# OATML-Markslab/ProteinGym

Hardware: AMD Instinct MI355X
Metric: mutants scored/sec (ESM-1v 650M masked-marginal) (higher is better)
Workload: dtype f16x3 (fp32 operands split into 2 fp16 planes, 3 fp16 MFMAs per product, fp32 accumulate)

## Files before the change

### proteingym_amd/csrc/api_esm.hip

```cpp
#include "model.h"

namespace pgmi {

int create_esm(pgmi_model* m, const pgmi_config* cfg, const float* w, int64_t n_weights) {
    const size_t D = cfg->embed_dim, F = cfg->ffn_dim, V = cfg->vocab, dh = m->dh, Da = m->Da;
    BlobCursor c(m, w, n_weights);
    c.upload(&m->embed_tokens, V * D);
    if (cfg->arch == PGMI_ARCH_ESM1B) c.upload(&m->embed_positions, (size_t)(cfg->max_positions + 2) * D);
    if (cfg->emb_layer_norm_before) {
        c.upload(&m->lnb_w, D);
        c.upload(&m->lnb_b, D);
    }
    auto slot = [&](size_t col) -> size_t { return rotate_half_slot(col, dh); };
    const float qscale = 1.0f / sqrtf((float)dh);
    m->layers.resize(cfg->layers);
    std::vector<float> wq(3 * Da * D, 0.0f), bq(3 * Da, 0.0f), wo_r(D * Da, 0.0f);
    for (int l = 0; l < cfg->layers; ++l) {
        Layer& L = m->layers[l];
        c.upload(&L.ln1_w, D);
        c.upload(&L.ln1_b, D);
        pack_qkv_slots(c.take(3 * (D * D + D)), D, Da, slot, qscale, wq.data(), bq.data());
        c.linear(&L.wqkv, &L.wqkv16, wq.data(), wq.size(), D);
        c.upload(&L.bqkv, bq.data(), bq.size());
        pack_out_cols(c.take(D * D), D, Da, slot, wo_r.data());
        c.linear(&L.wo, &L.wo16, wo_r.data(), wo_r.size(), Da);
        c.upload(&L.bo, D);
        c.upload(&L.ln2_w, D);
        c.upload(&L.ln2_b, D);
        c.linear(&L.w1, &L.w116, F * D, D);
        c.upload(&L.b1, F);
        c.linear(&L.w2, &L.w216, D * F, F);
        c.upload(&L.b2, D);
    }
    c.upload(&m->lna_w, D);
    c.upload(&m->lna_b, D);
    c.linear(&m->hd_w, &m->hd16, D * D, D);
    c.upload(&m->hd_b, D);
    c.upload(&m->hln_w, D);
    c.upload(&m->hln_b, D);
    c.upload(&m->head_b, V);
    m->head_w = m->embed_tokens;
    return c.finish();
}

int ensure_rotary(pgmi_model* m, int T) {
    if ((!esm2_rotary(m->cfg.arch) && !esmc_blocks(m->cfg.arch)) || T <= m->rot_len) return PGMI_OK;
    return upload_rotate_half(m, std::max(T, 1026));
}

int upload_rotate_half(pgmi_model* m, int n) {
    const int rh = m->rot_halves;
    float inv[64];
    const int half = m->dh / 2;
    for (int i = 0; i < half; ++i) inv[i] = 1.0f / powf(10000.0f, (float)(2 * i) / (float)m->dh);
    return upload_rotary(m, n, rh, [&](int t, int g, int i) {
        const int j = (rh == 1) ? i : 32 * g + i;
        return j < half ? (float)t * inv[j] : 0.0f;
    });
}

int run_encoder(pgmi_model* m, int B, int T, const int32_t* keep, int n_keep, bool* compacted) {
    const pgmi_config& c = m->cfg;
    const int M = B * T, D = c.embed_dim, F = c.ffn_dim, N1 = m->fc1_cols, H = c.heads, Da = m->Da;
    hipStream_t s = m->stream;
    if (c.arch == PGMI_ARCH_ESM1B && T > c.max_positions) {
        set_error("Sequence length %d above maximum sequence length of %d", T, c.max_positions);
        return PGMI_EINVAL;
    }
    int rc = ensure_rotary(m, T);
    if (!rc) rc = reset_pad_keys(m, B, T);
    if (rc) return rc;
    {
        ProfScope p(m, PGMI_K_EMBED, 0, (double)M * D * 4);
        launch_seq_stats(m->tokens, B, T, m->embed_gather ? 0 : c.token_dropout, m->denom, m->pos_idx, m->kv_len, s, m->mask_id);
        if (c.arch == PGMI_ARCH_ESM3) { if ((rc = esm3_embed(m, B, T))) return rc; }
        else if (m->embed_gather) launch_gather_rows(m->embed_tokens, m->tokens, M, D, m->x, s);
        else launch_embed(m->tokens, m->denom, m->pos_idx, m->embed_tokens, m->embed_positions, c.token_dropout, M, T, D, m->x, s, m->mask_id);
        if (m->lnb_w) {
            launch_layernorm(m->x, m->lnb_w, m->lnb_b, M, D, 1e-5f, m->x, s);
            launch_zero_pad_rows(m->tokens, M, D, m->x, s);
        }
    }
    const double ln_bytes = 2.0 * M * D * 4;
    const int prec = c.precision;
    const int mode16 = (prec == PGMI_PREC_F16X3) ? 1 : 2;
    for (int l = 0; l < c.layers; ++l) {
        const Layer& L = m->layers[l];
        { ProfScope p(m, PGMI_K_LAYERNORM, 0, ln_bytes);
          if (prec == PGMI_PREC_FP32) launch_layernorm(m->x, L.ln1_w, L.ln1_b, M, D, 1e-5f, m->h, s);
          else launch_layernorm16(m->x, L.ln1_w, L.ln1_b, M, D, 1e-5f, m->h16, mode16, s); }
        const bool fused_qkv = prec != PGMI_PREC_FP32 && !L.q_ln;
        { ProfScope p(m, PGMI_K_GEMM_QKV, 2.0 * M * 3 * D * D, 0);
          if (fused_qkv) {
              GemmLaunch g = qkv_launch(m, L.wqkv16, L.bqkv, M, Da, D, T, m->Hs);
              g.bf = prec == PGMI_PREC_BF16;
              g.qkv.cos_t = m->rot_cos; g.qkv.sin_t = m->rot_sin; g.qkv.rotary = esm2_rotary(c.arch); g.qkv.rot_halves = m->rot_halves;
              rc = launch_gemm16(g);
          } else
              rc = linear(m, m->h, m->h16, L.wqkv, L.wqkv16, L.bqkv, nullptr, m->qkv, nullptr, M, 3 * Da, D, EPI_NONE);
          if (rc) return rc; }
        { ProfScope p(m, PGMI_K_ATTENTION, 4.0 * M * T * D, L.q_ln ? (double)M * D * 20 : 0);
          if (L.q_ln && (rc = launch_qkln_prep(m->qkv, L.q_ln, L.k_ln, 1e-5f, m->rot_cos, m->rot_sin, B, T, H, m->qk16, m->qk16_plane,
                                               m->vt16, m->vt16_plane, s)))
              return rc;
          const bool v2 = prec != PGMI_PREC_FP32;
          if (esm2_rotary(c.arch) && !v2) launch_rotary(m->qkv, m->rot_cos, m->rot_sin, M, T, m->Hs, s, m->rot_halves);
          if (v2) {
              AttLaunch a;
              a.qk16 = m->qk16, a.qk_plane = m->qk16_plane, a.vt16 = m->vt16, a.vt_plane = m->vt16_plane;
              a.B = B, a.T = T, a.H = H, a.head_dim = m->rot_halves * kHeadDim;
              a.kv_len = m->kv_len;
              a.out = prec == PGMI_PREC_F16X3 ? ATT_OUT_SPLIT : ATT_OUT_BF16;
              a.ctx16 = m->h16;
              a.stream = s;
              rc = launch_attention_f16x3_v2(a);
          } else {
              rc = launch_attention_f32(m->qkv, m->kv_len, B, T, H, m->h, s, m->rot_halves * kHeadDim);
          }
          if (rc) return rc; }
        if (keep && m->keep_rows && l == c.layers - 1 && !L.g_norm_w) {
            const int R = n_keep;
            ProfScope p(m, PGMI_K_KEPT_ROWS, 2.0 * R * D * (Da + N1 + F), 0);
            launch_gather_rows(m->x, keep, R, D, m->qkv, s);
            if (prec == PGMI_PREC_FP32) launch_gather_rows(m->h, keep, R, Da, m->g, s);
            else
                launch_gather_rows(reinterpret_cast<const float*>(m->h16), keep, R, prec == PGMI_PREC_F16X3 ? Da : Da / 2,
                                   reinterpret_cast<float*>(m->g16), s);
            rc = linear(m, m->g, m->g16, L.wo, L.wo16, L.bo, m->qkv, m->x, nullptr, R, D, Da, EPI_NONE);
            if (rc) return rc;
            if (prec == PGMI_PREC_FP32) launch_layernorm(m->x, L.ln2_w, L.ln2_b, R, D, 1e-5f, m->h, s);
            else launch_layernorm16(m->x, L.ln2_w, L.ln2_b, R, D, 1e-5f, m->h16, mode16, s);
            rc = linear(m, m->h, m->h16, L.w1, L.w116, L.b1, nullptr,
                        prec == PGMI_PREC_FP32 ? m->g : nullptr, prec == PGMI_PREC_FP32 ? nullptr : m->g16,
                        R, N1, D, m->fc1_epi);
            if (rc) return rc;
            rc = linear(m, m->g, m->g16, L.w2, L.w216, L.b2, m->x, m->x, nullptr, R, D, F, EPI_NONE);
            if (rc) return rc;
            if (compacted) *compacted = true;
            break;
        }
        { ProfScope p(m, PGMI_K_GEMM_OUT, 2.0 * M * D * D, 0);
          rc = linear(m, m->h, m->h16, L.wo, L.wo16, L.bo, m->x, m->x, nullptr, M, D, Da, EPI_NONE);
          if (rc) return rc; }
        if (L.g_norm_w && m->e3_framed && (rc = geom_branch(m, L, B, T))) return rc;
        { ProfScope p(m, PGMI_K_LAYERNORM, 0, ln_bytes);
          if (prec == PGMI_PREC_FP32) launch_layernorm(m->x, L.ln2_w, L.ln2_b, M, D, 1e-5f, m->h, s);
          else launch_layernorm16(m->x, L.ln2_w, L.ln2_b, M, D, 1e-5f, m->h16, mode16, s); }
        { ProfScope p(m, PGMI_K_GEMM_FC1, 2.0 * M * N1 * D, 0);
          rc = linear(m, m->h, m->h16, L.w1, L.w116, L.b1, nullptr,
                      prec == PGMI_PREC_FP32 ? m->g : nullptr, prec == PGMI_PREC_FP32 ? nullptr : m->g16,
                      M, N1, D, m->fc1_epi);
          if (rc) return rc; }
        { ProfScope p(m, PGMI_K_GEMM_FC2, 2.0 * M * F * D, 0);
          rc = linear(m, m->g, m->g16, L.w2, L.w216, L.b2, m->x, m->x, nullptr, M, D, F, EPI_NONE);
          if (rc) return rc; }
    }
    PGMI_HIP(hipGetLastError());
    return PGMI_OK;
}

int run_head(pgmi_model* m, int R, const int32_t* row_idx) {
    const pgmi_config& c = m->cfg;
    ProfScope p(m, PGMI_K_HEAD, 2.0 * R * c.embed_dim * (c.embed_dim + c.vocab), 0);
    int rc = head_hidden(m, R, row_idx);
    if (rc) return rc;
    launch_vocab_logsoftmax(m->g, m->head_w, m->head_b, R, c.embed_dim, c.vocab, m->lp, m->nonfinite, m->stream);
    PGMI_HIP(hipGetLastError());
    return PGMI_OK;
}

int head_hidden(pgmi_model* m, int R, const int32_t* row_idx) {
    const pgmi_config& c = m->cfg;
    const int D = c.embed_dim;
    hipStream_t s = m->stream;
    const int prec = c.precision;
    const float* src = m->x;
    if (row_idx) {
        launch_gather_rows(m->x, row_idx, R, D, m->h, s);
        src = m->h;
    }
    if (prec == PGMI_PREC_FP32) launch_layernorm(src, m->lna_w, m->lna_b, R, D, 1e-5f, m->h, s);
    else launch_layernorm16(src, m->lna_w, m->lna_b, R, D, 1e-5f, m->h16, prec == PGMI_PREC_F16X3 ? 1 : 2, s);
    int rc = linear(m, m->h, m->h16, m->hd_w, m->hd16, m->hd_b, nullptr, m->g, nullptr, R, D, D, EPI_GELU);
    if (rc) return rc;
    launch_layernorm(m->g, m->hln_w, m->hln_b, R, D, 1e-5f, m->g, s);
    return PGMI_OK;
}


int run_rows(pgmi_model* m, int B, int T, int R, const int32_t* row_idx) {
    bool compacted = false;
    int rc = run_encoder(m, B, T, row_idx, R, &compacted);
    if (rc) return rc;
    return run_head(m, R, compacted ? nullptr : row_idx);
}

}

extern "C" {

int pgmi_token_logprobs(pgmi_model* m, const int32_t* tokens, int B, int T, float* out) {
    if (!m || !tokens || !out || B <= 0 || T <= 0) { set_error("bad argument"); return PGMI_EINVAL; }
    if (m->cfg.arch == PGMI_ARCH_SAPROT) { set_error("SaProt models are scored with pgmi_saprot_token_logprobs / pgmi_saprot_group_logprobs"); return PGMI_EINVAL; }
    if (T + 31 > m->max_rows) { set_error("T=%d exceeds workspace rows %d", T, m->max_rows); return PGMI_EINVAL; }
    int rc = check_tokens(tokens, B, T);
    if (rc) return rc;
    PGMI_HIP(hipSetDevice(m->device));
    const int V = m->cfg.vocab;
    rc = for_each_chunk(m, B, T, [&](int b0, int bc) {
        PGMI_HIP(hipMemcpyAsync(m->tokens, tokens + (size_t)b0 * T, (size_t)bc * T * 4, hipMemcpyHostToDevice, m->stream));
        int rc = run_rows(m, bc, T, bc * T, nullptr);
        if (rc) return rc;
        PGMI_HIP(hipMemcpyAsync(out + (size_t)b0 * T * V, m->lp, (size_t)bc * T * V * 4, hipMemcpyDeviceToHost, m->stream));
        return PGMI_OK;
    });
    return rc ? rc : check_nonfinite(m);
}

int pgmi_masked_logprobs(pgmi_model* m, const int32_t* tokens, const int32_t* mask_pos, int B, int T, float* out) {
    if (!m || !tokens || !mask_pos || !out || B <= 0 || T <= 0) { set_error("bad argument"); return PGMI_EINVAL; }
    if (m->cfg.arch == PGMI_ARCH_SAPROT) { set_error("SaProt models are scored with pgmi_saprot_token_logprobs / pgmi_saprot_group_logprobs"); return PGMI_EINVAL; }
    if (esmc_blocks(m->cfg.arch) && T + 31 > m->max_rows) { set_error("T=%d exceeds workspace rows %d", T, m->max_rows); return PGMI_EINVAL; }
    if (T > m->max_rows) { set_error("T=%d exceeds workspace rows %d", T, m->max_rows); return PGMI_EINVAL; }
    int rc = check_tokens(tokens, B, T);
    if (rc) return rc;
    for (int b = 0; b < B; ++b)
        if (mask_pos[b] < 0 || mask_pos[b] >= T) { set_error("mask_pos[%d]=%d out of range", b, mask_pos[b]); return PGMI_EINVAL; }
    PGMI_HIP(hipSetDevice(m->device));
    const int V = m->cfg.vocab;
    std::vector<int32_t> ridx;
    rc = for_each_chunk(m, B, T, [&](int b0, int bc) {
        ridx.resize(bc);
        for (int b = 0; b < bc; ++b) ridx[b] = b * T + mask_pos[b0 + b];
        PGMI_HIP(hipMemcpyAsync(m->tokens, tokens + (size_t)b0 * T, (size_t)bc * T * 4, hipMemcpyHostToDevice, m->stream));
        PGMI_HIP(hipMemcpyAsync(m->aux_i, mask_pos + b0, (size_t)bc * 4, hipMemcpyHostToDevice, m->stream));
        PGMI_HIP(hipMemcpyAsync(m->row_idx, ridx.data(), (size_t)bc * 4, hipMemcpyHostToDevice, m->stream));
        launch_apply_mask(m->tokens, m->aux_i, bc, T, m->stream);
        int rc = run_rows(m, bc, T, bc, m->row_idx);
        if (rc) return rc;
        PGMI_HIP(hipMemcpyAsync(out + (size_t)b0 * V, m->lp, (size_t)bc * V * 4, hipMemcpyDeviceToHost, m->stream));
        return PGMI_OK;
    });
    return rc ? rc : check_nonfinite(m);
}

int pgmi_assay_create(pgmi_model* m, const int32_t* wt_tokens, int n_tok, const int32_t* positions, int P,
                      int window, const int32_t* sub_pos, const int32_t* sub_wt, const int32_t* sub_mt,
                      const int64_t* mut_off, int64_t n_mut, pgmi_assay** out) {
    if (!out) { set_error("null out"); return PGMI_EINVAL; }
    *out = nullptr;
    if (!m || !wt_tokens || n_tok <= 0 || P < 0 || (P > 0 && !positions) || window <= 0 || n_mut < 0) { set_error("bad argument"); return PGMI_EINVAL; }
    if (esmc_blocks(m->cfg.arch)) { set_error("ESM C / ESM3 assays run through pgmi_masked_logprobs (their window rule is not pgmi_optimal_window)"); return PGMI_EINVAL; }
    if (m->cfg.arch == PGMI_ARCH_SAPROT) { set_error("SaProt assays run through pgmi_saprot_group_logprobs (position sets, no window)"); return PGMI_EINVAL; }
    for (int i = 0; i < n_tok; ++i)
        if (wt_tokens[i] < 0 || wt_tokens[i] >= PGMI_VOCAB || wt_tokens[i] == PGMI_TOK_PAD) { set_error("wt token %d invalid at %d", wt_tokens[i], i); return PGMI_EINVAL; }
    const int T = std::min(n_tok, window);
    if (T > m->max_rows) { set_error("T=%d exceeds workspace rows %d", T, m->max_rows); return PGMI_EINVAL; }
    std::vector<int32_t> ws(P), mr(P);
    for (int i = 0; i < P; ++i) {
        if (positions[i] < 0 || positions[i] >= n_tok) { set_error("position %d out of range", positions[i]); return PGMI_EINVAL; }
        int s, e;
        pgmi_optimal_window(positions[i], n_tok, window, &s, &e);
        if (e - s != T) { set_error("internal: window length %d != %d", e - s, T); return PGMI_EINVAL; }
        ws[i] = s;
        mr[i] = positions[i] - s;
    }
    const int64_t n_sub = n_mut ? mut_off[n_mut] : 0;
    for (int64_t k = 0; k < n_sub; ++k)
        if (sub_pos[k] < 0 || sub_pos[k] >= n_tok || sub_wt[k] < 0 || sub_wt[k] >= PGMI_VOCAB || sub_mt[k] < 0 || sub_mt[k] >= PGMI_VOCAB) {
            set_error("substitution %lld out of range", (long long)k);
            return PGMI_EINVAL;
        }
    PGMI_HIP(hipSetDevice(m->device));
    pgmi_assay* a = new pgmi_assay();
    a->m = m; a->n_tok = n_tok; a->P = P; a->T = T; a->n_mut = n_mut; a->n_sub = n_sub;
    int rc = dev_upload(a->allocs, &a->wt, wt_tokens, (size_t)n_tok);
    if (!rc) rc = dev_upload(a->allocs, &a->positions, positions, (size_t)P);
    if (!rc) rc = dev_upload(a->allocs, &a->win_start, ws.data(), (size_t)P);
    if (!rc) rc = dev_upload(a->allocs, &a->mask_rel, mr.data(), (size_t)P);
    if (!rc) rc = dev_upload(a->allocs, &a->sub_pos, sub_pos, (size_t)n_sub);
    if (!rc) rc = dev_upload(a->allocs, &a->sub_wt, sub_wt, (size_t)n_sub);
    if (!rc) rc = dev_upload(a->allocs, &a->sub_mt, sub_mt, (size_t)n_sub);
    if (!rc) rc = dev_upload(a->allocs, &a->mut_off, mut_off, (size_t)(n_mut + 1));
    if (!rc) rc = dev_alloc(a->allocs, &a->table, (size_t)n_tok * PGMI_VOCAB);
    if (!rc) rc = dev_alloc(a->allocs, &a->scores, (size_t)n_mut);
    if (rc) { pgmi_assay_destroy(a); return rc; }
    m->assays.push_back(a);
    *out = a;
    return PGMI_OK;
}

void pgmi_assay_destroy(pgmi_assay* a) {
    if (!a) return;
    if (a->m) {
        hipSetDevice(a->m->device);
        hipStreamSynchronize(a->m->stream);
        auto& v = a->m->assays;
        v.erase(std::remove(v.begin(), v.end(), a), v.end());
    }
    for (void* p : a->allocs) hipFree(p);
    delete a;
}

int pgmi_assay_run(pgmi_model* m, pgmi_assay* a, double* scores_host, float* table_host, double* scores_dev) {
    if (!m || !a || a->m != m) { set_error("bad model/assay handle (assay belongs to another or a destroyed model)"); return PGMI_EINVAL; }
    PGMI_HIP(hipSetDevice(m->device));
    hipStream_t s = m->stream;
    const int T = a->T, V = m->cfg.vocab;
    const int per = rows_per_chunk(m, T);
    launch_fill_f32(a->table, (int64_t)a->n_tok * V, NAN, s);
    for (int p0 = 0; p0 < a->P; p0 += per) {
        const int bc = std::min(per, a->P - p0);
        launch_make_masked_windows(a->wt, a->win_start + p0, a->mask_rel + p0, bc, T, m->tokens, s);
        launch_row_index(a->mask_rel + p0, bc, T, m->row_idx, s);
        int rc = run_rows(m, bc, T, bc, m->row_idx);
        if (rc) return rc;
        launch_scatter_rows(m->lp, a->positions + p0, bc, V, a->table, s);
    }
    {
        ProfScope p(m, PGMI_K_SCORE, 0, (double)a->n_sub * 20);
        launch_score_mutants(a->table, V, a->sub_pos, a->sub_wt, a->sub_mt, a->mut_off, a->n_mut, a->scores, s);
    }
    PGMI_HIP(hipGetLastError());
    if (scores_dev && a->n_mut) PGMI_HIP(hipMemcpyAsync(scores_dev, a->scores, (size_t)a->n_mut * 8, hipMemcpyDeviceToDevice, s));
    if (scores_host && a->n_mut) PGMI_HIP(hipMemcpyAsync(scores_host, a->scores, (size_t)a->n_mut * 8, hipMemcpyDeviceToHost, s));
    if (table_host) PGMI_HIP(hipMemcpyAsync(table_host, a->table, (size_t)a->n_tok * V * 4, hipMemcpyDeviceToHost, s));
    PGMI_HIP(hipStreamSynchronize(s));
    return check_nonfinite(m);
}

int pgmi_pppl_create(pgmi_model* m, const uint8_t* tokens, const int64_t* seq_off, int64_t n_seq, pgmi_pppl** out) {
    if (!out) { set_error("null out"); return PGMI_EINVAL; }
    *out = nullptr;
    if (!m || !tokens || !seq_off || n_seq <= 0 || n_seq > 0x7fffffff) { set_error("bad argument"); return PGMI_EINVAL; }
    if (m->cfg.arch != PGMI_ARCH_ESM1B && m->cfg.arch != PGMI_ARCH_ESM2) { set_error("pseudo-ppl needs an ESM-1b/1v/ESM2 model"); return PGMI_EINVAL; }
    if (seq_off[0] != 0) { set_error("seq_off[0] must be 0"); return PGMI_EINVAL; }
    for (int64_t n = 0; n < n_seq; ++n) {
        const int64_t len = seq_off[n + 1] - seq_off[n];
        if (len < 2 || len > (1 << 24)) { set_error("sequence %lld has %lld tokens", (long long)n, (long long)len); return PGMI_EINVAL; }
        const uint8_t* t = tokens + seq_off[n];
        for (int64_t i = 0; i < len; ++i)
            if (t[i] >= PGMI_VOCAB || t[i] == PGMI_TOK_PAD) { set_error("token id %d invalid at sequence %lld, position %lld", (int)t[i], (long long)n, (long long)i); return PGMI_EINVAL; }
    }
    PGMI_HIP(hipSetDevice(m->device));
    pgmi_pppl* q = new pgmi_pppl();
    q->m = m;
    q->N = n_seq;
    q->off.assign(seq_off, seq_off + n_seq + 1);
    int rc = dev_upload(q->allocs, &q->tok8, tokens, (size_t)seq_off[n_seq]);
    if (!rc) rc = dev_upload(q->allocs, &q->off_dev, seq_off, (size_t)n_seq + 1);
    if (rc) { for (void* p : q->allocs) hipFree(p); delete q; return rc; }
    m->pppls.push_back(q);
    *out = q;
    return PGMI_OK;
}

void pgmi_pppl_destroy(pgmi_pppl* q) {
    if (!q) return;
    if (q->m) {
        hipSetDevice(q->m->device);
        hipStreamSynchronize(q->m->stream);
        auto& v = q->m->pppls;
        v.erase(std::remove(v.begin(), v.end(), q), v.end());
    }
    for (void* p : q->allocs) hipFree(p);
    delete q;
}

int64_t pgmi_pppl_rows(const pgmi_pppl* q, int64_t first, int64_t count) {
    if (!q || first < 0 || count < 0 || first + count > q->N) return -1;
    int64_t r = 0;
    for (int64_t n = first; n < first + count; ++n) r += std::max<int64_t>(0, q->off[n + 1] - q->off[n] - 4);
    return r;
}

int pgmi_pppl_run(pgmi_model* m, pgmi_pppl* q, int64_t first, int64_t count, double* scores_host, float* terms_host,
                  double* scores_dev) {
    if (!m || !q || q->m != m) { set_error("bad model/library handle (library belongs to another or a destroyed model)"); return PGMI_EINVAL; }
    if (first < 0 || count <= 0 || first + count > q->N) { set_error("sequence range [%lld, %lld) outside the library of %lld", (long long)first, (long long)(first + count), (long long)q->N); return PGMI_EINVAL; }
    PGMI_HIP(hipSetDevice(m->device));
    hipStream_t s = m->stream;
    const int J = (int)count, V = m->cfg.vocab;
    std::vector<int32_t> sid(J);
    for (int j = 0; j < J; ++j) sid[j] = (int32_t)(first + j);
    auto len_of = [&](int32_t n) { return q->off[n + 1] - q->off[n]; };
    std::stable_sort(sid.begin(), sid.end(), [&](int32_t a, int32_t b) { return len_of(a) > len_of(b); });
    std::vector<int64_t> rp((size_t)J + 1);
    rp[0] = 0;
    for (int j = 0; j < J; ++j) rp[j + 1] = rp[j] + std::max<int64_t>(0, len_of(sid[j]) - 4);
    const int64_t R = rp[J];
    const int64_t Tmax = len_of(sid[0]);
    if (R > 0 && Tmax + 31 > m->max_rows) { set_error("T=%lld exceeds workspace rows %d", (long long)Tmax, m->max_rows); return PGMI_EINVAL; }
    if (R > 0 && m->cfg.arch == PGMI_ARCH_ESM1B && Tmax > m->cfg.max_positions) {
        set_error("Sequence length %lld above maximum sequence length of %d", (long long)Tmax, m->cfg.max_positions);
        return PGMI_EINVAL;
    }
    std::vector<void*> pool;
    auto cleanup = [&]() { for (void* p : pool) hipFree(p); };
    int32_t* d_sid = nullptr;
    int64_t* d_rp = nullptr;
    float* d_terms = nullptr;
    double* d_out = nullptr;
    int rc = dev_upload(pool, &d_sid, sid.data(), (size_t)J);
    if (!rc) rc = dev_upload(pool, &d_rp, rp.data(), (size_t)J + 1);
    if (!rc) rc = dev_alloc(pool, &d_terms, (size_t)R);
    if (!rc) rc = dev_alloc(pool, &d_out, (size_t)J);
    if (rc) { cleanup(); return rc; }
    q->last_rows = R; q->last_chunks = 0; q->last_tokens = 0; q->last_padded = 0;
    int j0 = 0;
    for (int64_t g0 = 0; g0 < R;) {
        while (rp[j0 + 1] <= g0) ++j0;
        const int T = (int)len_of(sid[j0]);
        const int bc = (int)std::min<int64_t>(rows_per_chunk(m, T), R - g0);
        launch_make_pppl_rows(q->tok8, q->off_dev, d_sid, d_rp, J, g0, bc, T, m->tokens, m->row_idx, m->aux_i, s);
        rc = run_rows(m, bc, T, bc, m->row_idx);
        if (rc) { hipStreamSynchronize(s); cleanup(); return rc; }
        launch_pppl_pick(m->lp, m->aux_i, bc, V, d_terms + g0, s);
        q->last_chunks += 1;
        q->last_padded += (int64_t)bc * T;
        g0 += bc;
        if ((q->last_chunks & 63) == 0 && g0 < R && (rc = check_nonfinite(m)) != PGMI_OK) { cleanup(); return rc; }
    }
    for (int j = 0; j < J; ++j) q->last_tokens += (rp[j + 1] - rp[j]) * len_of(sid[j]);
    {
        ProfScope p(m, PGMI_K_SCORE, 0, (double)R * 4);
        launch_pppl_sum(d_terms, d_rp, d_sid, J, first, d_out, s);
    }
    hipError_t e = hipGetLastError();
    if (e == hipSuccess && scores_dev) e = hipMemcpyAsync(scores_dev, d_out, (size_t)J * 8, hipMemcpyDeviceToDevice, s);
    if (e == hipSuccess && scores_host) e = hipMemcpyAsync(scores_host, d_out, (size_t)J * 8, hipMemcpyDeviceToHost, s);
    std::vector<float> sorted_terms;
    if (e == hipSuccess && terms_host && R > 0) {
        sorted_terms.resize((size_t)R);
        e = hipMemcpyAsync(sorted_terms.data(), d_terms, (size_t)R * 4, hipMemcpyDeviceToHost, s);
    }
    if (e == hipSuccess) e = hipStreamSynchronize(s);
    cleanup();
    if (e != hipSuccess) { set_error("pseudo-ppl run failed: %s", hipGetErrorString(e)); return PGMI_EHIP; }
    if (terms_host && R > 0) {
        std::vector<int64_t> dst((size_t)J + 1, 0);
        for (int k = 0; k < J; ++k) dst[k + 1] = dst[k] + std::max<int64_t>(0, len_of((int32_t)(first + k)) - 4);
        for (int j = 0; j < J; ++j)
            std::copy(sorted_terms.begin() + rp[j], sorted_terms.begin() + rp[j + 1], terms_host + dst[sid[j] - first]);
    }
    return check_nonfinite(m);
}

int pgmi_pppl_stats(const pgmi_pppl* q, int64_t* rows, int64_t* chunks, int64_t* tokens, int64_t* padded_tokens) {
    if (!q) { set_error("null library"); return PGMI_EINVAL; }
    if (rows) *rows = q->last_rows;
    if (chunks) *chunks = q->last_chunks;
    if (tokens) *tokens = q->last_tokens;
    if (padded_tokens) *padded_tokens = q->last_padded;
    return PGMI_OK;
}

}
```

### proteingym_amd/csrc/api_model.hip

```cpp
#include "model.h"

namespace pgmi {

static thread_local char g_err[1024] = "";
void set_error(const char* fmt, ...) {
    va_list ap;
    va_start(ap, fmt);
    vsnprintf(g_err, sizeof(g_err), fmt, ap);
    va_end(ap);
}

int prof_drain(pgmi_model* m) {
    if (m->events_used == 0) return PGMI_OK;
    PGMI_HIP(hipStreamSynchronize(m->stream));
    for (size_t i = 0; i < m->events_used; ++i) {
        float ms = 0.f;
        PGMI_HIP(hipEventElapsedTime(&ms, m->events[i].start, m->events[i].stop));
        m->prof_ms[m->events[i].cls] += ms;
    }
    m->events_used = 0;
    return PGMI_OK;
}

int check_cfg(const pgmi_config* c) {
    if (!c) { set_error("null config"); return PGMI_EINVAL; }
    if (c->abi_version != PGMI_ABI_VERSION) { set_error("ABI version mismatch: got %d, library is %d", c->abi_version, PGMI_ABI_VERSION); return PGMI_EINVAL; }
    if (c->arch != PGMI_ARCH_ESM1B && c->arch != PGMI_ARCH_ESM2 && c->arch != PGMI_ARCH_TRANCEPTION && c->arch != PGMI_ARCH_MSA &&
        c->arch != PGMI_ARCH_PROGEN2 && c->arch != PGMI_ARCH_GPT && c->arch != PGMI_ARCH_ESMC && c->arch != PGMI_ARCH_SAPROT &&
        c->arch != PGMI_ARCH_POET && c->arch != PGMI_ARCH_PROGEN3 && c->arch != PGMI_ARCH_ESM3 && c->arch != PGMI_ARCH_ESMIF1) { set_error("unknown arch %d", c->arch); return PGMI_EINVAL; }
    if (c->layers <= 0 || c->embed_dim <= 0 || c->heads <= 0 || c->ffn_dim <= 0) { set_error("non-positive model dimension"); return PGMI_EINVAL; }
    if (c->arch == PGMI_ARCH_ESMIF1) return if1_check(c, c->embed_dim);
    if (esmc_blocks(c->arch)) {
        if (c->precision != PGMI_PREC_F16X3) { set_error("ESM C is available in precision f16x3 only"); return PGMI_EINVAL; }
        if (c->embed_dim % 32 || c->embed_dim != c->heads * kHeadDim) { set_error("ESM C needs head_dim 64 and d %% 32 == 0 (embed_dim %d, heads %d)", c->embed_dim, c->heads); return PGMI_EINVAL; }
        if (c->embed_dim > 2048) { set_error("ESM C: embed_dim %d above the 2048 this build supports", c->embed_dim); return PGMI_EINVAL; }
        if (c->ffn_dim % 32) { set_error("ESM C: the SwiGLU hidden width %d must be a multiple of 32", c->ffn_dim); return PGMI_EINVAL; }
        if (c->vocab != PGMI_ESMC_VOCAB) { set_error("ESM C vocab must be %d", PGMI_ESMC_VOCAB); return PGMI_EINVAL; }
        return PGMI_OK;
    }
    {
        const int dh = c->embed_dim / c->heads;
        const bool pg2 = c->arch == PGMI_ARCH_PROGEN2;
        const bool esm_layout = c->arch == PGMI_ARCH_ESM1B || c->arch == PGMI_ARCH_ESM2 || c->arch == PGMI_ARCH_GPT || c->arch == PGMI_ARCH_SAPROT;
        const bool pg3 = c->arch == PGMI_ARCH_PROGEN3;
        if (pg3 && (c->embed_dim % c->heads || (dh != 64 && dh != 80 && dh != 96 && dh != 128 && dh != 256))) {
            set_error("unsupported head_dim %d (embed_dim %d / heads %d): ProGen3 runs head dims 64, 80, 96, 128 and 256", dh, c->embed_dim, c->heads);
            return PGMI_EINVAL;
        }
        const bool poet = c->arch == PGMI_ARCH_POET;
        if (poet && c->embed_dim % c->heads == 0 && dh > kHeadDim) {
            set_error("unsupported head_dim %d (embed_dim %d / heads %d): PoET's prefix attention runs even head dims up to 64", dh, c->embed_dim, c->heads);
            return PGMI_EINVAL;
        }
        const bool ok = c->embed_dim % c->heads == 0 &&
                        (dh == kHeadDim || (dh < kHeadDim && dh % 2 == 0 && (esm_layout || poet)) || (dh == 2 * kHeadDim && esm_layout) ||
                         (pg2 && dh % 2 == 0 && dh <= 4 * kHeadDim) || pg3);
        if (pg2 && !ok && c->embed_dim % c->heads == 0 && dh > 4 * kHeadDim) {
            set_error("unsupported head_dim %d (embed_dim %d / heads %d): ProGen2 runs even head dims up to 256", dh, c->embed_dim, c->heads);
            return PGMI_EINVAL;
        }
        if (!ok) { set_error("unsupported head_dim %d (embed_dim %d / heads %d): this build supports head_dim 64, even head dims below 64 and head_dim 128 (ESM)", dh, c->embed_dim, c->heads); return PGMI_EINVAL; }
    }
    if (c->embed_dim % 32 || c->ffn_dim % 32) { set_error("embed_dim and ffn_dim must be multiples of 32"); return PGMI_EINVAL; }
    if (c->arch == PGMI_ARCH_TRANCEPTION) {
        if (c->vocab != 25) { set_error("Tranception vocab must be 25"); return PGMI_EINVAL; }
        if (c->heads % 4) { set_error("Invalid number of heads. Tranception requires the number of heads to be a multiple of 4."); return PGMI_EINVAL; }
        if (c->precision != PGMI_PREC_F16X3) { set_error("Tranception is available in precision f16x3 only"); return PGMI_EINVAL; }
        if (c->max_positions <= 0) { set_error("Tranception needs max_positions = n_ctx"); return PGMI_EINVAL; }
    } else if (c->arch == PGMI_ARCH_PROGEN2) {
        if (c->vocab != PGMI_PG2_VOCAB) { set_error("ProGen2 vocab must be %d", PGMI_PG2_VOCAB); return PGMI_EINVAL; }
        if (c->heads % 8) { set_error("ProGen2 needs the number of heads to be a multiple of 8 (mp_num = 8), got %d", c->heads); return PGMI_EINVAL; }
        if (c->precision != PGMI_PREC_F16X3) { set_error("ProGen2 is available in precision f16x3 only"); return PGMI_EINVAL; }
        if (c->max_positions <= 0) { set_error("ProGen2 needs max_positions = n_positions"); return PGMI_EINVAL; }
    } else if (c->arch == PGMI_ARCH_GPT) {
        if (c->vocab < 2) { set_error("causal decoder vocab must be at least 2, got %d", c->vocab); return PGMI_EINVAL; }
        if (c->precision != PGMI_PREC_F16X3) { set_error("the causal decoder (RITA / ProtGPT2) is available in precision f16x3 only"); return PGMI_EINVAL; }
        if (c->max_positions <= 0) { set_error("the causal decoder needs max_positions = n_positions / max_seq_len"); return PGMI_EINVAL; }
    } else if (c->arch == PGMI_ARCH_SAPROT) {
        if (c->vocab != PGMI_SAPROT_VOCAB) { set_error("SaProt vocab must be %d (5 specials + 21 x 21 residue tokens)", PGMI_SAPROT_VOCAB); return PGMI_EINVAL; }
        if (c->max_positions != 0) { set_error("SaProt has rotary positions: max_positions must be 0"); return PGMI_EINVAL; }
    } else if (c->arch == PGMI_ARCH_POET) {
        if (c->vocab <= PGMI_POET_TOK_MASK || c->vocab > kWave) { set_error("PoET vocab must be in [%d, 64], got %d", PGMI_POET_TOK_MASK + 1, c->vocab); return PGMI_EINVAL; }
        if (c->precision != PGMI_PREC_F16X3) { set_error("PoET is available in precision f16x3 only"); return PGMI_EINVAL; }
        if (c->max_positions < 0) { set_error("PoET: max_positions is the largest prompt in tokens (0: no prompt)"); return PGMI_EINVAL; }
    } else if (c->arch == PGMI_ARCH_PROGEN3) {
        if (c->vocab <= kWave) { set_error("ProGen3 vocab must be above 64 (the wide LM head), got %d", c->vocab); return PGMI_EINVAL; }
        if (c->precision != PGMI_PREC_F16X3) { set_error("ProGen3 is available in precision f16x3 only"); return PGMI_EINVAL; }
        if (c->max_positions <= 0) { set_error("ProGen3 needs max_positions = the rotary table's rows"); return PGMI_EINVAL; }
    } else if (c->vocab != PGMI_VOCAB) { set_error("vocab must be %d", PGMI_VOCAB); return PGMI_EINVAL; }
    if (c->arch == PGMI_ARCH_ESM1B && c->max_positions <= 0) { set_error("ESM-1b arch needs max_positions"); return PGMI_EINVAL; }
    if (c->arch == PGMI_ARCH_MSA) {
        if (c->max_positions <= 0) { set_error("MSA Transformer needs max_positions"); return PGMI_EINVAL; }
        if (c->embed_dim != c->heads * kHeadDim) { set_error("MSA Transformer: head_dim must be 64"); return PGMI_EINVAL; }
        if (c->precision != PGMI_PREC_F16X3) { set_error("MSA Transformer is available in precision f16x3 only"); return PGMI_EINVAL; }
    }
    if (c->precision != PGMI_PREC_FP32 && c->precision != PGMI_PREC_F16X3 && c->precision != PGMI_PREC_BF16) { set_error("unknown precision %d", c->precision); return PGMI_EINVAL; }
    if (c->precision == PGMI_PREC_BF16 && (c->embed_dim % 64 || c->ffn_dim % 64)) { set_error("precision bf16 needs embed_dim and ffn_dim to be multiples of 64"); return PGMI_EINVAL; }
    return PGMI_OK;
}

int check_tokens(const int32_t* tokens, int B, int T, int n_ids) {
    for (int b = 0; b < B; ++b) {
        const int32_t* t = tokens + (size_t)b * T;
        bool seen_pad = false;
        if (t[0] == PGMI_TOK_PAD) { set_error("sequence %d is empty (all <pad>)", b); return PGMI_EINVAL; }
        for (int i = 0; i < T; ++i) {
            if (t[i] < 0 || t[i] >= n_ids) { set_error("token id %d out of range at [%d,%d]", t[i], b, i); return PGMI_EINVAL; }
            if (t[i] == PGMI_TOK_PAD) seen_pad = true;
            else if (seen_pad) { set_error("interior <pad> at [%d,%d]: only trailing padding is supported", b, i); return PGMI_EINVAL; }
        }
    }
    return PGMI_OK;
}

int check_vocab(const int32_t* tokens, int B, int T, int V) {
    for (int b = 0; b < B; ++b)
        for (int t = 0; t < T; ++t) {
            const int tk = tokens[(size_t)b * T + t];
            if (tk < 0 || tk >= V) { set_error("token id %d out of range at [%d,%d]", tk, b, t); return PGMI_EINVAL; }
        }
    return PGMI_OK;
}

int env_int(const char* name, int dflt) {
    const char* v = getenv(name);
    return v ? atoi(v) : dflt;
}

int make_w16(std::vector<void*>& pool, const float* host, size_t n, size_t K, int precision, hipStream_t s, W16* out) {
    float mx = 0.f;
    for (size_t i = 0; i < n; ++i) mx = std::max(mx, fabsf(host[i]));
    float scale = 1.0f;
    const int planes = (precision == PGMI_PREC_F16X3) ? 2 : 1;
    if (precision == PGMI_PREC_F16X3 && mx > 0.f && std::isfinite(mx)) scale = exp2f(floorf(log2f(16384.0f / mx)));
    float* tmp = nullptr;
    hipError_t e = hipMalloc(reinterpret_cast<void**>(&tmp), n * sizeof(float));
    if (e != hipSuccess) { set_error("hipMalloc failed: %s", hipGetErrorString(e)); return PGMI_ENOMEM; }
    int rc = dev_alloc(pool, &out->p, n * planes);
    if (rc) { hipFree(tmp); return rc; }
    e = hipMemcpy(tmp, host, n * sizeof(float), hipMemcpyHostToDevice);
    if (e == hipSuccess) {
        launch_split16(tmp, (int64_t)n, scale, precision == PGMI_PREC_BF16 ? 1 : 0, (int)K, out->p, s);
        e = hipStreamSynchronize(s);
    }
    hipFree(tmp);
    if (e != hipSuccess) { set_error("weight split failed: %s", hipGetErrorString(e)); return PGMI_EHIP; }
    out->out_scale = 1.0f / scale;
    return PGMI_OK;
}

int linear(pgmi_model* m, const float* in32, const unsigned short* in16, const float* W32, const W16& w16, const float* bias,
           const float* residual, float* out32, unsigned short* out16, int M, int N, int K, int epi) {
    if (m->cfg.precision == PGMI_PREC_FP32)
        return launch_gemm_f32(in32, W32, bias, residual, out32, M, N, K, epi, m->stream);
    GemmLaunch g;
    g.A = in16; g.W = w16.p; g.out_scale = w16.out_scale;
    g.bias = bias; g.residual = residual;
    g.out32 = out32; g.out16 = out16;
    g.M = M; g.N = N; g.K = K;
    g.epilogue = epi; g.bf = m->cfg.precision == PGMI_PREC_BF16; g.variant = m->gemm_variant; g.stream = m->stream;
    return launch_gemm16(g);
}

GemmLaunch qkv_launch(pgmi_model* m, const W16& w16, const float* bias, int M, int Da, int K, int T, int H) {
    GemmLaunch g;
    g.A = m->h16; g.W = w16.p; g.out_scale = w16.out_scale;
    g.bias = bias;
    g.out16 = m->qk16;
    g.M = M; g.N = 3 * Da; g.K = K;
    g.variant = m->gemm_variant; g.stream = m->stream;
    g.qkv.vt16 = m->vt16; g.qkv.vt_plane = m->vt16_plane; g.qkv.qk_plane = m->qk16_plane;
    g.qkv.T = T; g.qkv.H = H;
    return g;
}

PrefixAttLaunch prefix_launch(pgmi_model* m, const SegPlan& pl) {
    PrefixAttLaunch a;
    a.seg_off = pl.d_seg_off; a.ent_seg = pl.d_ent_seg; a.ent_tile = pl.d_ent_tile;
    a.n_seg = pl.n_seg(); a.n_ent = pl.n_ent(); a.H = m->cfg.heads;
    a.q16 = m->qk16; a.q_plane = (size_t)m->max_rows * m->Da;
    a.out = ATT_OUT_SPLIT; a.ctx16 = m->h16; a.stream = m->stream;
    return a;
}

int alloc_prefix_cache(pgmi_model* m) {
    PrefixCache& c = m->pfx;
    c.pitch = ((size_t)m->cfg.max_positions + 31) / 32 * 32;
    c.plane = (size_t)m->Da * c.pitch;
    c.cap = (size_t)m->max_rows;
    int rc = PGMI_OK;
    if (c.pitch) {
        const size_t n = (size_t)m->cfg.layers * 4 * c.plane;
        rc = dev_alloc(m->allocs, &c.planes, n);
        if (!rc) PGMI_HIP(hipMemset(c.planes, 0, n * sizeof(unsigned short)));
    }
    if (!rc) rc = dev_alloc(m->allocs, &c.meta, PrefixCache::meta_ints(c.cap));
    if (!rc) rc = dev_alloc(m->allocs, &m->gpt_sum, c.cap);
    return rc;
}

int check_nonfinite(pgmi_model* m) {
    if (m->cfg.precision == PGMI_PREC_FP32) return PGMI_OK;
    int32_t flag = 0;
    PGMI_HIP(hipMemcpyAsync(&flag, m->nonfinite, 4, hipMemcpyDeviceToHost, m->stream));
    PGMI_HIP(hipStreamSynchronize(m->stream));
    if (flag) {
        PGMI_HIP(hipMemsetAsync(m->nonfinite, 0, 4, m->stream));
        set_error("non-finite log-probabilities: an activation left the fp16/bf16 range in precision mode %d; "
                  "re-run with precision fp32", m->cfg.precision);
        return PGMI_EOVERFLOW;
    }
    return PGMI_OK;
}

int reset_pad_keys(pgmi_model* m, int B, int T) {
    if (!m->vt16 || (B == m->last_B && T == m->last_T)) return PGMI_OK;
    PGMI_HIP(hipMemsetAsync(m->vt16, 0, m->vt16_plane * 2 * sizeof(unsigned short), m->stream));
    m->last_B = B;
    m->last_T = T;
    return PGMI_OK;
}

}

extern "C" {

int pgmi_abi_version(void) { return PGMI_ABI_VERSION; }

const char* pgmi_last_error(void) { return g_err; }

int pgmi_device_count(void) {
    int n = 0;
    if (hipGetDeviceCount(&n) != hipSuccess) return 0;
    return n;
}

int64_t pgmi_weight_count(const pgmi_config* c) {
    if (!c || c->layers <= 0 || c->embed_dim <= 0 || c->ffn_dim <= 0) return -1;
    const int64_t D = c->embed_dim, F = c->ffn_dim, V = c->vocab;
    if (c->arch == PGMI_ARCH_TRANCEPTION) {
        const int64_t conv = 3 * ((64 * 3 + 64) + (64 * 5 + 64) + (64 * 7 + 64));
        return V * D + (int64_t)c->layers * (2 * D + (D * 3 * D + 3 * D) + conv + (D * D + D) + 2 * D + (D * F + F) + (F * D + D)) + 2 * D + V * D;
    }
    if (c->arch == PGMI_ARCH_PROGEN2)
        return V * D + (int64_t)c->layers * (2 * D + 3 * D * D + D * D + (F * D + F) + (D * F + D)) + 2 * D + V * D + V;
    if (c->arch == PGMI_ARCH_GPT) return -1;
    if (c->arch == PGMI_ARCH_POET) return -1;
    if (c->arch == PGMI_ARCH_PROGEN3) return -1;
    if (c->arch == PGMI_ARCH_ESM3) return -1;
    if (c->arch == PGMI_ARCH_ESMIF1) return -1;
    if (c->arch == PGMI_ARCH_ESMC) return esmc_weight_count(c);
    if (c->arch == PGMI_ARCH_MSA) {
        const int64_t attn = 2 * D + 4 * (D * D + D);
        return V * D + (int64_t)(c->max_positions + 2) * D + 1024 * D + 2 * D +
               (int64_t)c->layers * (2 * attn + 2 * D + (F * D + F) + (D * F + D)) + 2 * D + (D * D + D) + 2 * D + V;
    }
    int64_t n = V * D;
    if (c->arch == PGMI_ARCH_ESM1B) n += (int64_t)(c->max_positions + 2) * D;
    if (c->emb_layer_norm_before) n += 2 * D;
    n += (int64_t)c->layers * (2 * D + 4 * (D * D + D) + 2 * D + (F * D + F) + (D * F + D));
    n += 2 * D + (D * D + D) + 2 * D + V;
    return n;
}

int pgmi_model_create(const pgmi_config* cfg, const float* w, int64_t n_weights, int device, pgmi_model** out) {
    if (cfg && cfg->arch == PGMI_ARCH_PROGEN2) {
        if (out) *out = nullptr;
        set_error("ProGen2 models are created with pgmi_pg2_model_create (it takes rotary_dim)");
        return PGMI_EINVAL;
    }
    if (cfg && cfg->arch == PGMI_ARCH_GPT) {
        if (out) *out = nullptr;
        set_error("causal decoder models are created with pgmi_gpt_model_create (it takes pos_kind)");
        return PGMI_EINVAL;
    }
    if (cfg && cfg->arch == PGMI_ARCH_SAPROT) {
        if (out) *out = nullptr;
        set_error("SaProt models are created with pgmi_saprot_model_create (it takes the tokenizer's <mask> id)");
        return PGMI_EINVAL;
    }
    if (cfg && cfg->arch == PGMI_ARCH_POET) {
        if (out) *out = nullptr;
        set_error("PoET models are created with pgmi_poet_model_create (it takes final_norm)");
        return PGMI_EINVAL;
    }
    if (cfg && cfg->arch == PGMI_ARCH_PROGEN3) {
        if (out) *out = nullptr;
        set_error("ProGen3 models are created with pgmi_pg3_model_create (it takes pgmi_pg3_params)");
        return PGMI_EINVAL;
    }
    if (cfg && cfg->arch == PGMI_ARCH_ESM3) {
        if (out) *out = nullptr;
        set_error("ESM3 models are created with pgmi_esm3_model_create (it takes v_heads)");
        return PGMI_EINVAL;
    }
    if (cfg && cfg->arch == PGMI_ARCH_ESMIF1) {
        if (out) *out = nullptr;
        set_error("ESM-IF1 decoders are created with pgmi_esmif1_model_create (it takes the encoder width)");
        return PGMI_EINVAL;
    }
    return model_create(cfg, w, n_weights, device, out, 0);
}

}

namespace pgmi {

static int alloc_workspace(pgmi_model* m) {
    const pgmi_config& c = m->cfg;
    const size_t R = m->max_rows, D = c.embed_dim, F = c.ffn_dim, V = c.vocab, Da = m->Da;
    const size_t Dw = std::max(D, Da);
    const bool f32mode = c.precision == PGMI_PREC_FP32;
    int rc = PGMI_OK;
    auto alloc = [&](auto** p, size_t n) { if (!rc) rc = dev_alloc(m->allocs, p, n); };
    alloc(&m->x, R * D);
    alloc(&m->h, R * Dw);
    alloc(&m->qkv, R * 3 * Da);
    alloc(&m->g, R * (f32mode ? std::max(F, D) : D));
    if (!f32mode) {
        const size_t planes = c.precision == PGMI_PREC_F16X3 ? 2 : 1;
        m->h16_plane = R * Dw;
        m->g16_plane = R * F;
        alloc(&m->h16, m->h16_plane * planes);
        alloc(&m->g16, m->g16_plane * planes);
    }
    alloc(&m->nonfinite, (size_t)1);
    if (!f32mode) {
        m->qk16_plane = R * 2 * Da;
        m->vt16_plane = R * Da;
        alloc(&m->qk16, m->qk16_plane * 2);
        alloc(&m->vt16, m->vt16_plane * 2);
    }
    if (c.arch == PGMI_ARCH_MSA) {
        alloc(&m->xt, R * D);
        alloc(&m->msa_kv_len, (size_t)2048);
    }
    alloc(&m->lp, ((c.arch == PGMI_ARCH_GPT || c.arch == PGMI_ARCH_PROGEN3) && V > kWave ? (size_t)m->gpt_head_rows : R) * V);
    alloc(&m->denom, R);
    alloc(&m->tokens, R);
    alloc(&m->pos_idx, R);
    alloc(&m->kv_len, R);
    alloc(&m->row_idx, R);
    alloc(&m->aux_i, R);
    if (rc) return rc;
    PGMI_HIP(hipMemset(m->nonfinite, 0, 4));
    if (m->vt16) PGMI_HIP(hipMemset(m->vt16, 0, m->vt16_plane * 2 * sizeof(unsigned short)));
    return PGMI_OK;
}

int model_create(const pgmi_config* cfg, const float* w, int64_t n_weights, int device, pgmi_model** out, int arch_arg,
                 const pgmi_pg3_params* pg3) {
    if (!out) { set_error("null out"); return PGMI_EINVAL; }
    *out = nullptr;
    int rc = check_cfg(cfg);
    if (rc) return rc;
    if (cfg->arch == PGMI_ARCH_PROGEN3 && (rc = pg3_check(cfg, pg3))) return rc;
    if (cfg->arch == PGMI_ARCH_ESM3 && (rc = esm3_check(cfg, arch_arg))) return rc;
    if (cfg->arch == PGMI_ARCH_ESMIF1 && (rc = if1_check(cfg, arch_arg))) return rc;
    const int64_t need = cfg->arch == PGMI_ARCH_GPT ? gpt_weight_count(cfg, arch_arg)
                         : cfg->arch == PGMI_ARCH_PROGEN3 ? pg3_weight_count(cfg, pg3)
                         : cfg->arch == PGMI_ARCH_POET ? poet_weight_count(cfg, arch_arg)
                         : cfg->arch == PGMI_ARCH_ESM3 ? esm3_weight_count(cfg, arch_arg)
                         : cfg->arch == PGMI_ARCH_ESMIF1 ? if1_weight_count(cfg, arch_arg) : pgmi_weight_count(cfg);
    if (need < 0) { set_error("causal decoder pos_kind %d: must be PGMI_GPT_POS_ROTARY or PGMI_GPT_POS_LEARNED", arch_arg); return PGMI_EINVAL; }
    if (!w || n_weights != need) {
        set_error("weight blob has %lld elements, config needs %lld", (long long)n_weights, (long long)need);
        return PGMI_EINVAL;
    }
    const int ndev = pgmi_device_count();
    if (ndev <= 0) { set_error("no HIP device visible (libpgmi has no CPU fallback)"); return PGMI_ENODEV; }
    if (device < 0 || device >= ndev) { set_error("device %d out of range (%d visible)", device, ndev); return PGMI_EINVAL; }
    PGMI_HIP(hipSetDevice(device));
    pgmi_model* m = new pgmi_model();
    m->cfg = *cfg;
    m->device = device;
    if (hipStreamCreateWithFlags(&m->stream, hipStreamNonBlocking) != hipSuccess) { set_error("hipStreamCreate failed"); delete m; return PGMI_EHIP; }
    m->dh = cfg->embed_dim / cfg->heads;
    m->rot_halves = m->dh > 2 * kHeadDim ? 4 : m->dh > kHeadDim ? 2 : 1;
    m->Hs = cfg->heads * m->rot_halves;
    m->Da = m->Hs * kHeadDim;
    m->ln_eps = cfg->ln_eps > 0.f ? cfg->ln_eps : 1e-5f;
    m->max_rows = std::max(cfg->max_rows > 0 ? cfg->max_rows : 98304, 2048);
    const size_t V = cfg->vocab;
    const std::vector<float> zeros(std::max({3 * (size_t)m->Da, (V + 63) / 64 * 64, (size_t)cfg->embed_dim, V, (size_t)cfg->heads}), 0.0f);
    rc = dev_upload(m->allocs, &m->zeros, zeros.data(), zeros.size());
    m->fc1_cols = cfg->ffn_dim;
    if (!rc) switch (cfg->arch) {
        case PGMI_ARCH_TRANCEPTION: rc = create_tranception(m, cfg, w, n_weights); break;
        case PGMI_ARCH_MSA: rc = create_msa(m, cfg, w, n_weights); break;
        case PGMI_ARCH_PROGEN2: rc = create_progen2(m, cfg, w, n_weights, arch_arg); break;
        case PGMI_ARCH_GPT: rc = create_gpt(m, cfg, w, n_weights, arch_arg); break;
        case PGMI_ARCH_ESMC: rc = create_esmc(m, cfg, w, n_weights); break;
        case PGMI_ARCH_SAPROT: rc = create_saprot(m, cfg, w, n_weights, arch_arg); break;
        case PGMI_ARCH_POET: rc = create_poet(m, cfg, w, n_weights, arch_arg); break;
        case PGMI_ARCH_PROGEN3: rc = create_progen3(m, cfg, w, n_weights, pg3); break;
        case PGMI_ARCH_ESM3: rc = create_esm3(m, cfg, w, n_weights, arch_arg); break;
        case PGMI_ARCH_ESMIF1: rc = create_esmif1(m, cfg, w, n_weights, arch_arg); break;
        default: rc = create_esm(m, cfg, w, n_weights);
    }
    if (!rc) rc = alloc_workspace(m);
    if (rc) { pgmi_model_destroy(m); return rc; }
    m->keep_rows = env_int("PGMI_KEEP_ROWS", 1);
    gemm_options_from_env();
    m->gemm_variant = env_int("PGMI_GEMM_VARIANT", 0);
    *out = m;
    return PGMI_OK;
}

}

extern "C" {

void pgmi_model_destroy(pgmi_model* m) {
    if (!m) return;
    hipSetDevice(m->device);
    if (m->stream) hipStreamSynchronize(m->stream);
    for (pgmi_assay* a : m->assays) {
        for (void* p : a->allocs) hipFree(p);
        a->allocs.clear();
        a->m = nullptr;
    }
    m->assays.clear();
    for (pgmi_pppl* q : m->pppls) {
        for (void* p : q->allocs) hipFree(p);
        q->allocs.clear();
        q->m = nullptr;
    }
    m->pppls.clear();
    for (auto& e : m->events) { hipEventDestroy(e.start); hipEventDestroy(e.stop); }
    if (m->moe.counts_host) hipHostFree(m->moe.counts_host);
    for (void* p : m->allocs) hipFree(p);
    if (m->stream) hipStreamDestroy(m->stream);
    delete m;
}

int pgmi_model_device(const pgmi_model* m) { return m ? m->device : -1; }

int pgmi_set_option(const char* name, int64_t value) {
    if (!name) { set_error("null option name"); return PGMI_EINVAL; }
    int rc = gemm_set_option(name, (long long)value);
    if (rc) rc = att_set_option(name, (long long)value);
    if (rc) rc = eve_set_option(name, (long long)value);
    if (rc) rc = mpnn_set_option(name, (long long)value);
    if (rc) rc = unirep_set_option(name, (long long)value);
    if (rc) rc = s2f_set_option(name, (long long)value);
    if (rc) set_error("unknown option '%s' (gemm_half_tail, gemm_max_rows, att_xcd_local, att_v3, eve_max_rows, eve_fixed_sample, eve_prior_batch, mpnn_max_rows, unirep_max_rows, s2f_max_rows)", name);
    return rc;
}

int pgmi_synchronize(pgmi_model* m) {
    if (!m) { set_error("null model"); return PGMI_EINVAL; }
    PGMI_HIP(hipStreamSynchronize(m->stream));
    return PGMI_OK;
}

int pgmi_profile_enable(pgmi_model* m, int on) {
    if (!m) { set_error("null model"); return PGMI_EINVAL; }
    int rc = prof_drain(m);
    m->prof = on != 0;
    return rc;
}

int pgmi_profile_reset(pgmi_model* m) {
    if (!m) { set_error("null model"); return PGMI_EINVAL; }
    int rc = prof_drain(m);
    for (int i = 0; i < PGMI_K_COUNT; ++i) { m->prof_ms[i] = 0; m->prof_n[i] = 0; m->prof_flops[i] = 0; m->prof_bytes[i] = 0; }
    return rc;
}

int pgmi_profile_get(pgmi_model* m, int k, double* ms, int64_t* launches, double* flops, double* bytes) {
    if (!m || k < 0 || k >= PGMI_K_COUNT) { set_error("bad argument"); return PGMI_EINVAL; }
    int rc = prof_drain(m);
    if (rc) return rc;
    if (ms) *ms = m->prof_ms[k];
    if (launches) *launches = m->prof_n[k];
    if (flops) *flops = m->prof_flops[k];
    if (bytes) *bytes = m->prof_bytes[k];
    return PGMI_OK;
}

}
```

### proteingym_amd/csrc/attention_f16.hip

```cpp
#include <stdlib.h>
#include <string.h>
#include <algorithm>

#include "attention_f16_common.h"

namespace pgmi {

template <int WPB, int OUT, int NSTG, int DH = 64, bool RAG = false, int DO = DH>
__global__ __launch_bounds__(WPB * 64) void attention_f16x3_v2_kernel(
    const unsigned short* __restrict__ qk16, size_t qk_plane, const unsigned short* __restrict__ vt16,
    size_t vt_plane, const int32_t* __restrict__ kv_len, const float* __restrict__ slopes, int T, int H,
    int Tp, float* __restrict__ ctx, unsigned short* __restrict__ ctx16, RagMap rag, int dense_nblk, int nseq) {
    constexpr float defer_thr = kAttDefer;
    constexpr int NT = WPB * 64;
    constexpr int KCPR = DH / 8;
    constexpr int KCH = AKT * KCPR, VCH = DO * 4;
    constexpr int NSL = DH / DO;
    static_assert(NSL == 1 || (OUT == ATT_OUT_SPLIT && !RAG), "sliced context: split-plane output of dense launches only");
    constexpr int STG_CH = 2 * KCH + 2 * VCH;
    constexpr int NWI = STG_CH / 64;
    static_assert(NWI % WPB == 0, "the wave-instructions of a stage divide evenly over the waves");
    constexpr int NDMA = NWI / WPB;
    constexpr int NS = DH / 16, ND = DO / 32;
    extern __shared__ __attribute__((aligned(16))) u32x4 lds[];

    int b, h, qblk_dense, hs;
    if (RAG) {
        b = rag.ent_seq[blockIdx.x];
        hs = blockIdx.y;
        qblk_dense = 0;
    } else if (dense_nblk > 0) {
        const int pair = xcd_local_pair(dense_nblk, qblk_dense);
        if (pair >= nseq * H * NSL) return;
        b = pair / (H * NSL);
        hs = pair - b * (H * NSL);
    } else {
        b = blockIdx.z;
        hs = blockIdx.y;
        qblk_dense = blockIdx.x;
    }
    h = hs / NSL;
    const int d0 = (hs - h * NSL) * DO;
    const int tid = threadIdx.x, lane = tid & 63;
    const int wave = __builtin_amdgcn_readfirstlane(tid >> 6);
    const int r = lane & 31, kh = lane >> 5;
    const int D = H * DH;
    const int Tk = (!RAG && kv_len) ? kv_len[b] : T;
    const int p0 = RAG ? rag.seq_p[b] : 0, a0 = p0 & ~(AKT - 1), kt0 = a0 / AKT;
    const int qblk = RAG ? rag.ent_j[blockIdx.x] : qblk_dense;
    const int row0 = RAG ? rag.seq_q[b] : b * T, rrow0 = RAG ? rag.seq_q[rag.seq_root[b]] : 0;
    const int orow0 = RAG ? rag.seq_off[b] - p0 : b * T;
    const int Tpo = RAG ? (T - a0 + 31) / 32 * 32 : Tp;
    const int q0 = a0 + (qblk * WPB + wave) * 32;
    const bool active = q0 < T;

    constexpr bool q_lds = NSTG >= 3;
    u32x4 qh[NS], ql[NS];
    if (!q_lds) {
        const int qrow = min(q0 + r, T - 1);
        const unsigned short* qp = qk16 + ((size_t)row0 + (qrow - a0)) * (2 * D) + h * DH + kh * 8;
#pragma unroll
        for (int s = 0; s < NS; ++s) {
            qh[s] = *reinterpret_cast<const u32x4*>(qp + s * 16);
            ql[s] = *reinterpret_cast<const u32x4*>(qp + qk_plane + s * 16);
        }
    }

    const size_t seq_halfs = (size_t)T * (2 * D), vt_halfs = (size_t)DH * Tp;
    const unsigned long long qk_bytes = std::min<unsigned long long>(0xFFFFFFFFull, (unsigned long long)qk_plane * 2ull + seq_halfs * 2ull);
    const unsigned long long vt_bytes = std::min<unsigned long long>(0xFFFFFFFFull, (unsigned long long)vt_plane * 2ull + vt_halfs * 2ull);
    const __amdgpu_buffer_rsrc_t rsQK = operand_rsrc(qk16 + (size_t)row0 * (2 * D), qk_bytes);
    const __amdgpu_buffer_rsrc_t rsVT = operand_rsrc(vt16 + (RAG ? (size_t)rag.seq_vt[b] + (size_t)h * DH * Tpo : ((size_t)b * H + h) * vt_halfs), vt_bytes);
    const __amdgpu_buffer_rsrc_t rsQKr = operand_rsrc(qk16 + (size_t)rrow0 * (2 * D), qk_bytes);
    const __amdgpu_buffer_rsrc_t rsVTr = operand_rsrc(vt16 + (RAG ? (size_t)rag.seq_vt[rag.seq_root[b]] + (size_t)h * DH * Tp : (size_t)0), vt_bytes);
    const bool causal = slopes != nullptr;
    const int last_q = min(T, a0 + (qblk * WPB + WPB) * 32);
    const int nkt = causal ? (min(Tk, last_q) + AKT - 1) / AKT : (Tk + AKT - 1) / AKT;
    int voff[NDMA], voff_last[NDMA], voff_root[NDMA], sbase[NDMA], sstep[NDMA], slot0[NDMA];
    bool is_k[NDMA];
#pragma unroll
    for (int i = 0; i < NDMA; ++i) {
        int wi = wave + WPB * i;
        if (wi >= NWI) wi -= NWI;
        slot0[i] = wi * 64;
        is_k[i] = wi < 2 * KCH / 64;
        if (is_k[i]) {
            const int p = wi / (KCH / 64), key = ((wi % (KCH / 64)) * 64 + lane) / KCPR;
            const int c = (lane % KCPR) ^ k_swizzle<DH>(key);
            voff[i] = voff_root[i] = key * (2 * D) * 2 + c * 16;
            voff_last[i] = min(key, T - 1 - (nkt - 1) * AKT) * (2 * D) * 2 + c * 16;
            sbase[i] = (int)((unsigned int)p * (unsigned int)qk_plane * 2u + (unsigned int)(D + h * DH) * 2u);
            sstep[i] = AKT * (2 * D) * 2;
        } else {
            const int wv = wi - 2 * KCH / 64, p = wv / (VCH / 64), g = (wv % (VCH / 64)) * 64 + lane;
            const int d = g >> 2, c = (g & 3) ^ ((d >> 2) & 3);
            voff[i] = voff_last[i] = (d0 + d) * Tpo * 2 + c * 16;
            voff_root[i] = (d0 + d) * Tp * 2 + c * 16;
            sbase[i] = (int)((unsigned int)p * (unsigned int)vt_plane * 2u);
            sstep[i] = (AKT / 8) * 16;
        }
    }
    auto issue_tile = [&](int kt, int buf) {
        u32x4* base = lds + buf * STG_CH;
        const bool from_root = RAG && kt < kt0;
#pragma unroll
        for (int i = 0; i < NDMA; ++i) {
            const int vo = from_root ? voff_root[i] : ((kt == nkt - 1) ? voff_last[i] : voff[i]);
            const int so = sbase[i] + (from_root ? kt : kt - kt0) * sstep[i];
            if (is_k[i]) __builtin_amdgcn_raw_ptr_buffer_load_lds(from_root ? rsQKr : rsQK, (__attribute__((address_space(3))) void*)(base + slot0[i]), 16, vo, so, 0, 0);
            else __builtin_amdgcn_raw_ptr_buffer_load_lds(from_root ? rsVTr : rsVT, (__attribute__((address_space(3))) void*)(base + slot0[i]), 16, vo, so, 0, 0);
        }
    };

    constexpr float kLog2e = 1.4426950408889634f;
    const float slope2 = causal ? slopes[h] * kLog2e : 0.0f;
    if (q_lds) {
        issue_tile(0, 0);
        u32x4* qbase = lds + STG_CH + wave * (2 * KCH);
        if (active) {
            constexpr int NQ = 2 * KCH / 64;
#pragma unroll
            for (int i = 0; i < NQ; ++i) {
                const int f = i * 64 + lane, pq = f / KCH, row = (f % KCH) / KCPR;
                const int c = (f % KCPR) ^ k_swizzle<DH>(row);
                const int vo = (int)(((unsigned int)(min(q0 + row, T - 1) - a0) * (unsigned int)(2 * D) + (unsigned int)(h * DH)) * 2u + (unsigned int)c * 16u);
                const int so = (int)((unsigned int)pq * (unsigned int)qk_plane * 2u);
                __builtin_amdgcn_raw_ptr_buffer_load_lds(rsQK, (__attribute__((address_space(3))) void*)(qbase + i * 64), 16, vo, so, 0, 0);
            }
        }
        asm volatile("s_waitcnt vmcnt(0)" ::: "memory");
        if (active) {
#pragma unroll
            for (int s = 0; s < NS; ++s) {
                const int ci = r * KCPR + ((2 * s + kh) ^ k_swizzle<DH>(r));
                qh[s] = qbase[ci];
                ql[s] = qbase[KCH + ci];
            }
        }
        asm volatile("s_waitcnt lgkmcnt(0)" ::: "memory");
        __builtin_amdgcn_s_barrier();
        asm volatile("" ::: "memory");
#pragma unroll
        for (int t = 1; t < NSTG - 1; ++t)
            if (t < nkt) issue_tile(t, t);
    } else {
#pragma unroll
        for (int t = 0; t < NSTG - 1; ++t)
            if (t < nkt) issue_tile(t, t);
    }

    f32x16 om[ND], oc[ND];
#pragma unroll
    for (int dt = 0; dt < ND; ++dt)
#pragma unroll
        for (int v = 0; v < 16; ++v) { om[dt][v] = 0.f; oc[dt][v] = 0.f; }
    float m_run = -INFINITY, l_run = 0.f;
    constexpr float kInvLo = 1.0f / kLoScale;

    const f32x16 zero16 = {0.f, 0.f, 0.f, 0.f, 0.f, 0.f, 0.f, 0.f, 0.f, 0.f, 0.f, 0.f, 0.f, 0.f, 0.f, 0.f};
    auto wanted = [&](int kt) -> bool { return active && !(causal && kt * AKT > q0 + 31); };
    auto scores = [&](int buf, f32x16& sm, f32x16& sc) {
        const u32x4* Kb = lds + buf * STG_CH;
#pragma unroll
        for (int s = 0; s < NS; ++s) {
            const int ci = r * KCPR + ((2 * s + kh) ^ k_swizzle<DH>(r));
            const u32x4 kfh = Kb[ci], kfl = Kb[KCH + ci];
            sc = mfma_h(kfh, ql[s], s == 0 ? zero16 : sc);
            sc = mfma_h(kfl, qh[s], sc);
            sm = mfma_h(kfh, qh[s], s == 0 ? zero16 : sm);
        }
    };
    auto wait_tile = [&](int younger) {
        if (younger >= 2) asm volatile("s_waitcnt vmcnt(%0)" ::"n"(2 * NDMA) : "memory");
        else if (younger == 1) asm volatile("s_waitcnt vmcnt(%0)" ::"n"(NDMA) : "memory");
        else asm volatile("s_waitcnt vmcnt(0)" ::: "memory");
    };
    int cur = 0;
    for (int kt = 0; kt < nkt; ++kt) {
        wait_tile(min(NSTG - 2, nkt - 1 - kt));
        __builtin_amdgcn_s_barrier();
        asm volatile("" ::: "memory");
        if (kt + NSTG - 1 < nkt) issue_tile(kt + NSTG - 1, (cur == 0) ? NSTG - 1 : cur - 1);
        if (wanted(kt)) {
            const u32x4* Vb = lds + cur * STG_CH + 2 * KCH;
            f32x16 sm, sc;
            scores(cur, sm, sc);
            float st[16];
            if (causal) {
                const float kb = (float)(kt * AKT + 4 * kh);
#pragma unroll
                for (int v = 0; v < 16; ++v)
                    st[v] = fmaf(slope2, kb + (float)((v & 3) + 8 * (v >> 2)), fmaf(sc[v], kInvLo, sm[v]));
                if (kt * AKT + AKT - 1 > q0) {
#pragma unroll
                    for (int v = 0; v < 16; ++v) {
                        const int key = kt * AKT + (v & 3) + 8 * (v >> 2) + 4 * kh;
                        if (key > q0 + r) st[v] = -INFINITY;
                    }
                }
            } else {
#pragma unroll
                for (int v = 0; v < 16; ++v) st[v] = fmaf(sc[v], kInvLo, sm[v]);
            }
            if (kt * AKT + AKT > Tk) {
#pragma unroll
                for (int v = 0; v < 16; ++v) {
                    const int key = kt * AKT + (v & 3) + 8 * (v >> 2) + 4 * kh;
                    if (key >= Tk) st[v] = -INFINITY;
                }
            }
            float mloc = st[0];
#pragma unroll
            for (int v = 1; v < 16; ++v) mloc = fmaxf(mloc, st[v]);
            {
                const unsigned int mu = __builtin_bit_cast(unsigned int, mloc);
                const auto sw = __builtin_amdgcn_permlane32_swap(mu, mu, false, false);
                const unsigned int s0 = sw[0], s1 = sw[1];
                mloc = fmaxf(__builtin_bit_cast(float, s0), __builtin_bit_cast(float, s1));
            }
            const float m_new = fmaxf(m_run, mloc);
            if (!__all(m_new <= m_run + defer_thr)) {
                const bool moved = m_new > m_run + defer_thr;
                const float alpha = moved ? __builtin_amdgcn_exp2f(m_run - m_new) : 1.0f;
                l_run *= alpha;
#pragma unroll
                for (int dt = 0; dt < ND; ++dt)
#pragma unroll
                    for (int v = 0; v < 16; ++v) { om[dt][v] *= alpha; oc[dt][v] *= alpha; }
                if (moved) m_run = m_new;
            }
            const float mb = m_run - 10.0f;
            typedef float f32x2 __attribute__((ext_vector_type(2)));
#pragma unroll
            for (int v = 0; v < 16; v += 2) {
                const f32x2 dlt = f32x2{st[v], st[v + 1]} - f32x2{mb, mb};
                st[v] = __builtin_amdgcn_exp2f(dlt[0]);
                st[v + 1] = __builtin_amdgcn_exp2f(dlt[1]);
            }
            l_run += ((st[0] + st[1]) + (st[2] + st[3])) + ((st[4] + st[5]) + (st[6] + st[7])) +
                     (((st[8] + st[9]) + (st[10] + st[11])) + ((st[12] + st[13]) + (st[14] + st[15])));
#pragma unroll
            for (int m = 0; m < 2; ++m) {
                u32x4 ph, pl;
#pragma unroll
                for (int e = 0; e < 4; ++e) {
                    const u32x2 p = split_p(st[8 * m + 2 * e], st[8 * m + 2 * e + 1]);
                    ph[e] = p[0];
                    pl[e] = p[1];
                }
#pragma unroll
                for (int dt = 0; dt < ND; ++dt) {
                    const int ci = v_chunk(dt * 32 + r, m, kh);
                    const u32x4 vfh = Vb[ci], vfl = Vb[VCH + ci];
                    oc[dt] = mfma_h(vfh, pl, oc[dt]);
                    oc[dt] = mfma_h(vfl, ph, oc[dt]);
                    om[dt] = mfma_h(vfh, ph, om[dt]);
                }
            }
        }
        cur = (cur == NSTG - 1) ? 0 : cur + 1;
    }

    if (active) {
        const float l_tot = l_run + __shfl_xor(l_run, 32);
        const float inv = 1.0f / l_tot;
        const bool row_ok = q0 + r < T && q0 + r >= p0;
        const size_t orow = (size_t)(orow0 + max(min(q0 + r, T - 1), p0));
        if (OUT == ATT_OUT_BF16) store_ctx_bf16<ND>(om, oc, inv, kInvLo, row_ok, ctx16 + orow * (size_t)D + (size_t)h * DH, kh);
        else if (OUT == ATT_OUT_SPLIT) store_ctx_split<ND>(om, oc, inv, kInvLo, row_ok, ctx16 + orow * (size_t)(2 * D) + (size_t)((h * DH + d0) / 32) * 64, kh);
        else if (row_ok) store_ctx_f32<ND>(om, oc, inv, kInvLo, ctx + (size_t)(orow0 + q0 + r) * D + (size_t)h * DH + 4 * kh);
    }
}


using Att16v2Kernel = decltype(&attention_f16x3_v2_kernel<4, ATT_OUT_F32, 3, 64, false, 64>);
struct Att16v2Inst { int wpb, out, head_dim; bool rag; Att16v2Kernel fn; size_t lds_bytes; };
template <int WPB, int OUT, int NSTG, int DH, bool RAG = false, int DO = DH>
static constexpr Att16v2Inst att16v2_inst() {
    return {WPB, OUT, DH, RAG, attention_f16x3_v2_kernel<WPB, OUT, NSTG, DH, RAG, DO>, (size_t)NSTG * (8 * DH + 8 * DO) * 16};
}
static const Att16v2Inst kAtt16v2[] = {
    att16v2_inst<1, ATT_OUT_F32, 3, 64>(),   att16v2_inst<2, ATT_OUT_F32, 3, 64>(),   att16v2_inst<4, ATT_OUT_F32, 3, 64>(),
    att16v2_inst<1, ATT_OUT_SPLIT, 3, 64>(), att16v2_inst<2, ATT_OUT_SPLIT, 3, 64>(), att16v2_inst<4, ATT_OUT_SPLIT, 3, 64>(),
    att16v2_inst<1, ATT_OUT_BF16, 3, 64>(),  att16v2_inst<2, ATT_OUT_BF16, 3, 64>(),  att16v2_inst<4, ATT_OUT_BF16, 3, 64>(),
    att16v2_inst<1, ATT_OUT_SPLIT, 3, 64, true>(), att16v2_inst<2, ATT_OUT_SPLIT, 3, 64, true>(), att16v2_inst<4, ATT_OUT_SPLIT, 3, 64, true>(),
    att16v2_inst<4, ATT_OUT_F32, 3, 128>(),  att16v2_inst<4, ATT_OUT_SPLIT, 3, 128>(), att16v2_inst<4, ATT_OUT_BF16, 3, 128>(),
    att16v2_inst<4, ATT_OUT_SPLIT, 2, 256, false, 128>(),
};

static int launch_att16v2(const AttLaunch& a, int wpb, dim3 grid, const RagMap* rag, int dense_nblk) {
    for (const Att16v2Inst& k : kAtt16v2) {
        if (k.wpb != wpb || k.out != a.out || k.head_dim != a.head_dim || k.rag != (rag != nullptr)) continue;
        if (k.lds_bytes > 65536) {
            hipError_t e = hipFuncSetAttribute(reinterpret_cast<const void*>(k.fn), hipFuncAttributeMaxDynamicSharedMemorySize, (int)k.lds_bytes);
            if (e != hipSuccess) { set_error("hipFuncSetAttribute: %s", hipGetErrorString(e)); return PGMI_EHIP; }
        }
        hipLaunchKernelGGL(k.fn, grid, dim3(wpb * 64), k.lds_bytes, a.stream, a.qk16, a.qk_plane, a.vt16, a.vt_plane, a.kv_len, a.slopes,
                           a.T, a.H, (a.T + 31) / 32 * 32, a.ctx, a.ctx16, rag ? *rag : RagMap{}, dense_nblk, a.B);
        PGMI_HIP(hipGetLastError());
        return PGMI_OK;
    }
    set_error("attention_f16x3_v2: no kernel for %d waves, output %d, head_dim %d%s", wpb, (int)a.out, a.head_dim, rag ? ", ragged" : "");
    return PGMI_EINVAL;
}

static int g_att_xcd_local = -1;
int att_set_option(const char* name, long long value) {
    if (!strcmp(name, "att_xcd_local")) { g_att_xcd_local = (int)value; return PGMI_OK; }
    if (!strcmp(name, "att_v3")) { att_v3_set_option((int)value); return PGMI_OK; }
    return PGMI_EINVAL;
}
static dim3 dense_grid(int nblk, int H, int B, int* dense_nblk) {
    if (g_att_xcd_local == 0 || (g_att_xcd_local < 0 && nblk < 2)) { *dense_nblk = 0; return dim3(nblk, H, B); }
    *dense_nblk = nblk;
    const long long pairs = (long long)H * B, groups = (pairs + 7) / 8;
    return dim3((unsigned)(groups * 8 * nblk), 1, 1);
}

int att16_waves_per_block(int T) {
    const int n32 = (T + 31) / 32, nblk = (n32 + 3) / 4;
    const int wpb = (n32 + nblk - 1) / nblk;
    return wpb == 3 ? 4 : wpb;
}

static int check_operand_range(const char* who, const AttLaunch& a) {
    const unsigned long long Tp = (unsigned long long)(a.T + 31) / 32 * 32;
    const unsigned long long seq_bytes = (unsigned long long)a.T * 2ull * (unsigned long long)a.H * (unsigned long long)a.head_dim * 2ull;
    const unsigned long long vt_bytes = (unsigned long long)a.head_dim * Tp * 2ull;
    if ((unsigned long long)a.qk_plane * 2ull + seq_bytes >= (1ull << 32) || (unsigned long long)a.vt_plane * 2ull + vt_bytes >= (1ull << 32)) {
        set_error("%s: operand planes of %zu / %zu halfs exceed the 32-bit offset range of the K / V^T DMA "
                  "(plane stride + one sequence must stay below 4 GiB: create the model with a smaller max_rows)", who, a.qk_plane, a.vt_plane);
        return PGMI_EINVAL;
    }
    return PGMI_OK;
}

int launch_attention_f16x3_v2(const AttLaunch& a) {
    const int B = a.B, T = a.T, H = a.H, head_dim = a.head_dim;
    if (B <= 0 || T <= 0 || H <= 0 || a.out < ATT_OUT_F32 || a.out > ATT_OUT_BF16 || (head_dim != 64 && head_dim != 128 && head_dim != 256)) {
        set_error("attention_f16x3_v2: bad arguments B=%d T=%d H=%d out=%d head_dim=%d", B, T, H, (int)a.out, head_dim);
        return PGMI_EINVAL;
    }
    const int n32 = (T + 31) / 32, Tp = n32 * 32;
    int rc = check_operand_range("attention_f16x3_v2", a);
    if (rc) return rc;
    int dn = 0;
    if (head_dim == 256) {
        if (a.qkv || a.conv || !a.slopes || a.out != ATT_OUT_SPLIT) { set_error("attention_f16x3_v2: head_dim 256 is the causal, fused-QKV, split-plane-output flavour only"); return PGMI_EINVAL; }
        const dim3 grid = dense_grid((n32 + 3) / 4, 2 * H, B, &dn);
        return launch_att16v2(a, 4, grid, nullptr, dn);
    }
    if (head_dim == 128) {
        if (a.qkv || a.conv) { set_error("attention_f16x3_v2: head_dim 128 needs operands from the fused QKV projection"); return PGMI_EINVAL; }
        const dim3 grid = dense_grid((n32 + 3) / 4, H, B, &dn);
        return launch_att16v2(a, 4, grid, nullptr, dn);
    }
    if (a.qkv && a.conv && a.rotary) { set_error("attention_f16x3_v2: depth-wise convolution and rotary together are not a model this library knows"); return PGMI_EINVAL; }
    if (a.qkv && a.conv && H % 4) { set_error("attention_f16x3_v2: the depth-wise convolution has four head groups, H = %d is not a multiple of 4", H); return PGMI_EINVAL; }
    if (a.qkv && a.conv)
        launch_qkv_prep_conv(dim3(n32, H, B), a.stream, a.qkv, a.conv, T, H, Tp, a.qk16, a.qk_plane, a.vt16, a.vt_plane, nullptr);
    else if (a.qkv)
        launch_qkv_prep(dim3(n32, H, B), a.stream, a.qkv, a.cos_t, a.sin_t, a.rotary, T, H, Tp, a.qk16, a.qk_plane, a.vt16, a.vt_plane);
    const int wpb = att16_waves_per_block(T);
    const dim3 grid = dense_grid((n32 + wpb - 1) / wpb, H, B, &dn);
    return att_v3_serves(a) ? launch_att16v3(a, wpb, grid, dn) : launch_att16v2(a, wpb, grid, nullptr, dn);
}

int launch_attention_tr_ragged(const AttLaunch& a, const AttRagged& rg) {
    const int T = a.T, H = a.H;
    if (T <= 0 || H <= 0 || !a.qkv || !a.conv || !a.slopes || a.head_dim != 64 || a.out != ATT_OUT_SPLIT || rg.n_tiles <= 0 || rg.n_blocks <= 0) {
        set_error("attention_tr_ragged: bad arguments T=%d H=%d tiles=%d blocks=%d", T, H, rg.n_tiles, rg.n_blocks);
        return PGMI_EINVAL;
    }
    const int rc = check_operand_range("attention_tr_ragged", a);
    if (rc) return rc;
    const RagMap tiles{rg.seq_off, rg.seq_p, rg.seq_q, rg.seq_root, rg.seq_vt, rg.tile_seq, rg.tile_j};
    launch_qkv_prep_conv(dim3(rg.n_tiles, H, 1), a.stream, a.qkv, a.conv, T, H, (T + 31) / 32 * 32, a.qk16, a.qk_plane, a.vt16, a.vt_plane, &tiles);
    const RagMap rag{rg.seq_off, rg.seq_p, rg.seq_q, rg.seq_root, rg.seq_vt, rg.blk_seq, rg.blk_j};
    return launch_att16v2(a, att16_waves_per_block(T), dim3(rg.n_blocks, H, 1), &rag, 0);
}

}
```

### proteingym_amd/csrc/attention_f16_v3.hip

```cpp
#include <stdlib.h>
#include <string.h>
#include <algorithm>

#include "attention_f16_common.h"

namespace pgmi {

template <int WPB, int OUT>
__global__ __launch_bounds__(WPB * 64, 2) void attention_f16x3_v3_kernel(
    const unsigned short* __restrict__ qk16, size_t qk_plane, const unsigned short* __restrict__ vt16, size_t vt_plane,
    const int32_t* __restrict__ kv_len, int T, int H, int Tp, float* __restrict__ ctx, unsigned short* __restrict__ ctx16,
    int dense_nblk, int nseq) {
    constexpr float defer_thr = kAttDefer;
    constexpr int DH = 64, NSTG = 3, KCPR = 8, KCH = AKT * KCPR, VCH = DH * 4, STG_CH = 2 * KCH + 2 * VCH;
    constexpr int NWI = STG_CH / 64, NDMA = (NWI + WPB - 1) / WPB, NS = 4, ND = 2;
    extern __shared__ __attribute__((aligned(16))) u32x4 lds[];
    int b, h, qblk;
    if (dense_nblk > 0) {
        const int pair = xcd_local_pair(dense_nblk, qblk);
        if (pair >= nseq * H) return;
        b = pair / H;
        h = pair - b * H;
    } else {
        b = blockIdx.z;
        h = blockIdx.y;
        qblk = blockIdx.x;
    }
    const int tid = threadIdx.x, lane = tid & 63;
    const int wave = __builtin_amdgcn_readfirstlane(tid >> 6);
    const int r = lane & 31, kh = lane >> 5;
    const int D = H * DH;
    const int Tk = kv_len ? kv_len[b] : T;
    const int q0 = (qblk * WPB + wave) * 32;
    const bool active = q0 < T;
    const int nkt = (Tk + AKT - 1) / AKT;
    const size_t seq_halfs = (size_t)T * (2 * D), vt_halfs = (size_t)DH * Tp;
    const unsigned long long qk_bytes = std::min<unsigned long long>(0xFFFFFFFFull, (unsigned long long)qk_plane * 2ull + seq_halfs * 2ull);
    const unsigned long long vt_bytes = std::min<unsigned long long>(0xFFFFFFFFull, (unsigned long long)vt_plane * 2ull + vt_halfs * 2ull);
    const __amdgpu_buffer_rsrc_t rsQK = operand_rsrc(qk16 + (size_t)b * seq_halfs, qk_bytes);
    const __amdgpu_buffer_rsrc_t rsVT = operand_rsrc(vt16 + ((size_t)b * H + h) * vt_halfs, vt_bytes);

    static_assert(WPB == 1 || WPB == 2 || WPB == 4, "the DMA map needs WPB to divide 8");
    constexpr int NK = 8 / WPB;
    int kvoff[NK], krow[NK], vvoff[NDMA - NK];
#pragma unroll
    for (int i = 0; i < NK; ++i) {
        const int q4 = (wave + WPB * i) & 3;
        const int key = q4 * 8 + (lane >> 3);
        krow[i] = key;
        kvoff[i] = ((lane & 7) ^ k_swizzle<DH>(key)) * 16;
    }
#pragma unroll
    for (int i = 0; i < NDMA - NK; ++i) {
        const int q4 = (wave + WPB * (i + NK)) & 3;
        const int g = q4 * 64 + lane, d = g >> 2, c = (g & 3) ^ ((d >> 2) & 3);
        vvoff[i] = d * Tp * 2 + c * 16;
    }
    auto issue_piece = [&](int i, int m, int stage, bool on) {
        u32x4* base = lds + stage * STG_CH;
        const int kk = min(m, nkt - 1), vv = min(max(m - 2, 0), nkt - 1);
        if (i < NK) {
            const int wi = wave + WPB * i, p = (WPB * i) >> 2;
            const int kr = krow[i < NK ? i : 0], ko = kvoff[i < NK ? i : 0];
            const int vo = on ? min(kk * AKT + kr, T - 1) * (2 * D) * 2 + ko : -16;
            const int so = (int)((unsigned int)p * (unsigned int)qk_plane * 2u + (unsigned int)(D + h * DH) * 2u);
            __builtin_amdgcn_raw_ptr_buffer_load_lds(rsQK, (__attribute__((address_space(3))) void*)(base + wi * 64), 16, vo, so, 0, 0);
        } else {
            const int wi = wave + WPB * i, p = (WPB * i - 8) >> 2;
            const int so = (int)((unsigned int)p * (unsigned int)vt_plane * 2u) + vv * ((AKT / 8) * 16);
            const int vv0 = vvoff[i >= NK ? i - NK : 0];
            const int vo = on ? vv0 : -16;
            __builtin_amdgcn_raw_ptr_buffer_load_lds(rsVT, (__attribute__((address_space(3))) void*)(base + wi * 64), 16, vo, so, 0, 0);
        }
    };
    auto issue_bundle = [&](int m, int stage, bool on) {
#pragma unroll
        for (int i = 0; i < NDMA; ++i) issue_piece(i, m, stage, on);
    };
    const int last_bundle = nkt + 1;

    issue_bundle(0, 0, true);
    u32x4 qh[NS], ql[NS];
    {
        u32x4* qbase = lds + STG_CH + wave * (2 * KCH);
        if (active) {
            constexpr int NQ = 2 * KCH / 64;
#pragma unroll
            for (int i = 0; i < NQ; ++i) {
                const int f = i * 64 + lane, pq = f / KCH, row = (f % KCH) / KCPR;
                const int c = (f % KCPR) ^ k_swizzle<DH>(row);
                const int vo = (int)(((unsigned int)min(q0 + row, T - 1) * (unsigned int)(2 * D) + (unsigned int)(h * DH)) * 2u + (unsigned int)c * 16u);
                const int so = (int)((unsigned int)pq * (unsigned int)qk_plane * 2u);
                __builtin_amdgcn_raw_ptr_buffer_load_lds(rsQK, (__attribute__((address_space(3))) void*)(qbase + i * 64), 16, vo, so, 0, 0);
            }
        }
        asm volatile("s_waitcnt vmcnt(0)" ::: "memory");
        if (active) {
#pragma unroll
            for (int s = 0; s < NS; ++s) {
                const int ci = r * KCPR + ((2 * s + kh) ^ k_swizzle<DH>(r));
                qh[s] = qbase[ci];
                ql[s] = qbase[KCH + ci];
            }
        }
        asm volatile("s_waitcnt lgkmcnt(0)" ::: "memory");
        __builtin_amdgcn_s_barrier();
        asm volatile("" ::: "memory");
    }
    issue_bundle(1, 1, true);
    issue_bundle(2, 2, true);

    f32x16 om[ND], oc[ND], sm, sc;
#pragma unroll
    for (int dt = 0; dt < ND; ++dt)
#pragma unroll
        for (int v = 0; v < 16; ++v) { om[dt][v] = 0.f; oc[dt][v] = 0.f; }
#pragma unroll
    for (int v = 0; v < 16; ++v) { sm[v] = 0.f; sc[v] = 0.f; }
    u32x4 ph[2], pl[2];
#pragma unroll
    for (int m = 0; m < 2; ++m)
#pragma unroll
        for (int e = 0; e < 4; ++e) { ph[m][e] = 0u; pl[m][e] = 0u; }
    float m_run = -INFINITY, l_run = 0.f;
    constexpr float kInvLo = 1.0f / kLoScale;
    const f32x16 zero16 = {0.f, 0.f, 0.f, 0.f, 0.f, 0.f, 0.f, 0.f, 0.f, 0.f, 0.f, 0.f, 0.f, 0.f, 0.f, 0.f};
    typedef float f32x2 __attribute__((ext_vector_type(2)));
    typedef _Float16 h4 __attribute__((ext_vector_type(4)));

    auto vfrag = [&](const u32x4* Vb, int m, u32x4 (&fh)[ND], u32x4 (&fl)[ND]) {
#pragma unroll
        for (int dt = 0; dt < ND; ++dt) {
            const int ci = v_chunk(dt * 32 + r, m, kh);
            fh[dt] = Vb[ci];
            fl[dt] = Vb[VCH + ci];
        }
    };
    auto kfrag = [&](const u32x4* Kb, int s, u32x4& kh_, u32x4& kl_) {
        const int ci = r * KCPR + ((2 * s + kh) ^ k_swizzle<DH>(r));
        kh_ = Kb[ci];
        kl_ = Kb[KCH + ci];
    };
    auto pv = [&](int m, const u32x4 (&fh)[ND], const u32x4 (&fl)[ND]) {
#pragma unroll
        for (int dt = 0; dt < ND; ++dt) {
            oc[dt] = mfma_h(fh[dt], pl[m], oc[dt]);
            oc[dt] = mfma_h(fl[dt], ph[m], oc[dt]);
            om[dt] = mfma_h(fh[dt], ph[m], om[dt]);
        }
    };
    auto split_pm = [&](const float (&st)[16], int m, int e) {
        const u32x2 p = split_p(st[8 * m + 2 * e], st[8 * m + 2 * e + 1]);
        ph[m][e] = p[0];
        pl[m][e] = p[1];
    };
    bool pend = false;
    float pend_alpha = 1.0f;
    auto apply_pending = [&]() {
        if (pend) {
#pragma unroll
            for (int dt = 0; dt < ND; ++dt)
#pragma unroll
                for (int v = 0; v < 16; ++v) { om[dt][v] *= pend_alpha; oc[dt][v] *= pend_alpha; }
        }
    };
    auto step = [&](auto MKc, int kt, const u32x4* stage, int dma_stage) {
        constexpr bool MK = decltype(MKc)::value;
        apply_pending();
        const u32x4* Kb = stage;
        const u32x4* Vb = stage + 2 * KCH;
        u32x4 va_h[ND], va_l[ND], vb_h[ND], vb_l[ND];
        u32x4 k0h, k0l, k1h, k1l;
        float st[16];
#define PGMI_SLOT() __builtin_amdgcn_sched_barrier(0)
        vfrag(Vb, 0, va_h, va_l);
        vfrag(Vb, 1, vb_h, vb_l);
#pragma unroll
        for (int v = 0; v < 16; ++v) st[v] = fmaf(sc[v], kInvLo, sm[v]);
        if constexpr (MK) {
#pragma unroll
            for (int v = 0; v < 16; ++v) {
                const int key = kt * AKT + (v & 3) + 8 * (v >> 2) + 4 * kh;
                if (key >= Tk) st[v] = -INFINITY;
            }
        }
        float ma = st[0];
#pragma unroll
        for (int v = 1; v < 8; ++v) ma = fmaxf(ma, st[v]);
        PGMI_SLOT();
        oc[0] = mfma_h(va_h[0], pl[0], oc[0]);
        float mloc = st[8];
#pragma unroll
        for (int v = 9; v < 16; ++v) mloc = fmaxf(mloc, st[v]);
        mloc = fmaxf(mloc, ma);
        PGMI_SLOT();
        oc[0] = mfma_h(va_l[0], ph[0], oc[0]);
        {
            const unsigned int mu = __builtin_bit_cast(unsigned int, mloc);
            const auto sw = __builtin_amdgcn_permlane32_swap(mu, mu, false, false);
            const unsigned int s0 = sw[0], s1 = sw[1];
            mloc = fmaxf(__builtin_bit_cast(float, s0), __builtin_bit_cast(float, s1));
        }
        const float m_new = fmaxf(m_run, mloc);
        PGMI_SLOT();
        om[0] = mfma_h(va_h[0], ph[0], om[0]);
        const bool moved = m_new > m_run + defer_thr;
        pend = !__all(m_new <= m_run + defer_thr);
        pend_alpha = moved ? __builtin_amdgcn_exp2f(m_run - m_new) : 1.0f;
        l_run *= pend_alpha;
        asm volatile("" : "+v"(l_run));
        m_run = moved ? m_new : m_run;
        const float mb = m_run - 10.0f;
        PGMI_SLOT();
        auto exp_pairs = [&](int v0) {
#pragma unroll
            for (int v = v0; v < v0 + 4; v += 2) {
                const f32x2 dlt = f32x2{st[v], st[v + 1]} - f32x2{mb, mb};
                st[v] = __builtin_amdgcn_exp2f(dlt[0]);
                st[v + 1] = __builtin_amdgcn_exp2f(dlt[1]);
            }
        };
        oc[1] = mfma_h(va_h[1], pl[0], oc[1]);
        exp_pairs(0);
        PGMI_SLOT();
        oc[1] = mfma_h(va_l[1], ph[0], oc[1]);
        exp_pairs(4);
        PGMI_SLOT();
        om[1] = mfma_h(va_h[1], ph[0], om[1]);
        exp_pairs(8);
        PGMI_SLOT();
        oc[0] = mfma_h(vb_h[0], pl[1], oc[0]);
        exp_pairs(12);
        PGMI_SLOT();
        oc[0] = mfma_h(vb_l[0], ph[1], oc[0]);
        const float sa = ((st[0] + st[1]) + (st[2] + st[3])) + ((st[4] + st[5]) + (st[6] + st[7]));
        PGMI_SLOT();
        om[0] = mfma_h(vb_h[0], ph[1], om[0]);
        kfrag(Kb, 0, k0h, k0l);
        l_run += sa + (((st[8] + st[9]) + (st[10] + st[11])) + ((st[12] + st[13]) + (st[14] + st[15])));
        PGMI_SLOT();
        oc[1] = mfma_h(vb_h[1], pl[1], oc[1]);
        split_pm(st, 0, 0);
        PGMI_SLOT();
        oc[1] = mfma_h(vb_l[1], ph[1], oc[1]);
        split_pm(st, 0, 1);
        PGMI_SLOT();
        om[1] = mfma_h(vb_h[1], ph[1], om[1]);
        kfrag(Kb, 1, k1h, k1l);
        split_pm(st, 0, 2);
        PGMI_SLOT();
        sc = mfma_h(k0h, ql[0], zero16);
        split_pm(st, 0, 3);
        PGMI_SLOT();
        sc = mfma_h(k0l, qh[0], sc);
        split_pm(st, 1, 0);
        PGMI_SLOT();
        sm = mfma_h(k0h, qh[0], zero16);
        kfrag(Kb, 2, k0h, k0l);
        split_pm(st, 1, 1);
        PGMI_SLOT();
        sc = mfma_h(k1h, ql[1], sc);
        split_pm(st, 1, 2);
        PGMI_SLOT();
        sc = mfma_h(k1l, qh[1], sc);
        split_pm(st, 1, 3);
        PGMI_SLOT();
        sm = mfma_h(k1h, qh[1], sm);
        kfrag(Kb, 3, k1h, k1l);
        PGMI_SLOT();
        const bool dma_on = kt + 3 <= last_bundle;
        auto dma_slot = [&](int j) {
#pragma unroll
            for (int i = j; i < NDMA; i += 6) issue_piece(i, kt + 3, dma_stage, dma_on);
        };
        sc = mfma_h(k0h, ql[2], sc);
        dma_slot(0);
        PGMI_SLOT();
        sc = mfma_h(k0l, qh[2], sc);
        dma_slot(1);
        PGMI_SLOT();
        sm = mfma_h(k0h, qh[2], sm);
        dma_slot(2);
        PGMI_SLOT();
        sc = mfma_h(k1h, ql[3], sc);
        dma_slot(3);
        PGMI_SLOT();
        sc = mfma_h(k1l, qh[3], sc);
        dma_slot(4);
        PGMI_SLOT();
        sm = mfma_h(k1h, qh[3], sm);
        dma_slot(5);
#undef PGMI_SLOT
    };
    auto closing_pv = [&](const u32x4* stage) {
        apply_pending();
        const u32x4* Vb = stage + 2 * KCH;
        u32x4 va_h[ND], va_l[ND], vb_h[ND], vb_l[ND];
        vfrag(Vb, 0, va_h, va_l);
        vfrag(Vb, 1, vb_h, vb_l);
        pv(0, va_h, va_l);
        pv(1, vb_h, vb_l);
    };
    using T1 = std::integral_constant<bool, true>;
    using T0 = std::integral_constant<bool, false>;

    if (active && nkt > 0) {
#pragma unroll
        for (int s = 0; s < NS; ++s) {
            const int ci = r * KCPR + ((2 * s + kh) ^ k_swizzle<DH>(r));
            const u32x4 kfh = lds[ci], kfl = lds[KCH + ci];
            sc = mfma_h(kfh, ql[s], s == 0 ? zero16 : sc);
            sc = mfma_h(kfl, qh[s], sc);
            sm = mfma_h(kfh, qh[s], s == 0 ? zero16 : sm);
        }
    }
    auto wait_bundle = [&](int younger) {
        if (younger >= 1) asm volatile("s_waitcnt vmcnt(%0)" ::"n"(NDMA) : "memory");
        else asm volatile("s_waitcnt vmcnt(0)" ::: "memory");
    };
    int cur = 1;
    auto step_head = [&](int kt) {
        wait_bundle(1);
        __builtin_amdgcn_s_barrier();
        asm volatile("" ::: "memory");
    };
    auto idle_dma = [&](int kt) {
        issue_bundle(kt + 3, cur == 0 ? NSTG - 1 : cur - 1, kt + 3 <= last_bundle);
    };
    for (int kt = 0; kt < nkt - 1; ++kt) {
        step_head(kt);
        if (active) step(T0{}, kt, lds + cur * STG_CH, cur == 0 ? NSTG - 1 : cur - 1);
        else idle_dma(kt);
        cur = (cur == NSTG - 1) ? 0 : cur + 1;
    }
    step_head(nkt - 1);
    if (active) step(T1{}, nkt - 1, lds + cur * STG_CH, cur == 0 ? NSTG - 1 : cur - 1);
    else idle_dma(nkt - 1);
    cur = (cur == NSTG - 1) ? 0 : cur + 1;
    asm volatile("s_waitcnt vmcnt(0)" ::: "memory");
    __builtin_amdgcn_s_barrier();
    asm volatile("" ::: "memory");
    if (active) closing_pv(lds + cur * STG_CH);

    if (active) {
        const float l_tot = l_run + __shfl_xor(l_run, 32);
        const float inv = 1.0f / l_tot;
        const bool row_ok = q0 + r < T;
        const size_t orow = (size_t)(b * T + min(q0 + r, T - 1));
        if (OUT == ATT_OUT_BF16) store_ctx_bf16<ND>(om, oc, inv, kInvLo, row_ok, ctx16 + orow * (size_t)D + (size_t)h * DH, kh);
        else if (OUT == ATT_OUT_SPLIT) store_ctx_split<ND>(om, oc, inv, kInvLo, row_ok, ctx16 + orow * (size_t)(2 * D) + (size_t)(ND * h) * 64, kh);
        else if (row_ok) store_ctx_f32<ND>(om, oc, inv, kInvLo, ctx + (size_t)(b * T + q0 + r) * D + (size_t)h * DH + 4 * kh);
    }
}

static int g_att_v3 = -1;
void att_v3_set_option(int value) { g_att_v3 = value; }
bool att_v3_serves(const AttLaunch& a) {
    if (g_att_v3 == 0 || a.conv || a.slopes || a.head_dim != 64) return false;
    return g_att_v3 > 0 || (a.T + 31) / 32 >= 7;
}

using Att16v3Kernel = decltype(&attention_f16x3_v3_kernel<4, ATT_OUT_F32>);
struct Att16v3Inst { int wpb, out; Att16v3Kernel fn; };
template <int WPB, int OUT>
static constexpr Att16v3Inst att16v3_inst() { return {WPB, OUT, attention_f16x3_v3_kernel<WPB, OUT>}; }
static const Att16v3Inst kAtt16v3[] = {
    att16v3_inst<1, ATT_OUT_F32>(),   att16v3_inst<2, ATT_OUT_F32>(),   att16v3_inst<4, ATT_OUT_F32>(),
    att16v3_inst<1, ATT_OUT_SPLIT>(), att16v3_inst<2, ATT_OUT_SPLIT>(), att16v3_inst<4, ATT_OUT_SPLIT>(),
    att16v3_inst<1, ATT_OUT_BF16>(),  att16v3_inst<2, ATT_OUT_BF16>(),  att16v3_inst<4, ATT_OUT_BF16>(),
};

int launch_att16v3(const AttLaunch& a, int wpb, dim3 grid, int dense_nblk) {
    constexpr size_t lds_bytes = (size_t)3 * (2 * AKT * 8 + 2 * 64 * 4) * 16;
    for (const Att16v3Inst& k : kAtt16v3) {
        if (k.wpb != wpb || k.out != a.out) continue;
        hipLaunchKernelGGL(k.fn, grid, dim3(wpb * 64), lds_bytes, a.stream, a.qk16, a.qk_plane, a.vt16, a.vt_plane, a.kv_len, a.T, a.H, (a.T + 31) / 32 * 32,
                           a.ctx, a.ctx16, dense_nblk, a.B);
        PGMI_HIP(hipGetLastError());
        return PGMI_OK;
    }
    set_error("attention_f16x3_v3: no kernel for %d waves, output %d", wpb, (int)a.out);
    return PGMI_EINVAL;
}

}
```

### proteingym_amd/csrc/common.h

```cpp
#pragma once
#include <hip/hip_runtime.h>
#include <stdint.h>
#include <stddef.h>

#include "../../include/pgmi.h"

namespace pgmi {

void set_error(const char* fmt, ...);

#define PGMI_HIP(expr)                                                                   \
    do {                                                                                 \
        hipError_t _e = (expr);                                                          \
        if (_e != hipSuccess) {                                                          \
            pgmi::set_error("%s failed: %s (%s:%d)", #expr, hipGetErrorString(_e),       \
                            __FILE__, __LINE__);                                         \
            return PGMI_EHIP;                                                            \
        }                                                                                \
    } while (0)

typedef float f32x4 __attribute__((ext_vector_type(4)));
typedef float f32x16 __attribute__((ext_vector_type(16)));

constexpr int kWave = 64;
constexpr int kHeadDim = 64;

enum Epilogue { EPI_NONE = 0, EPI_GELU = 1, EPI_SQRELU = 2, EPI_GELU_TANH = 3,
                EPI_SWIGLU = 4,
                EPI_RELU = 5 };

constexpr float kLoScale = 2048.0f;
constexpr float kQLog2e = 1.4426950408889634f;

__host__ __device__ __forceinline__ size_t ki_off(size_t row, int k, int K) {
    return row * (size_t)(2 * K) + (size_t)(k >> 5) * 64 + (size_t)(k & 31);
}
#if defined(__HIPCC__)
__device__ __forceinline__ void split_act(float x, _Float16& hi, _Float16& lo) {
    hi = (fabsf(x) < 6.103515625e-05f) ? (_Float16)0.0f : (_Float16)x;
    lo = (_Float16)((x - (float)hi) * kLoScale);
}
typedef _Float16 f16x4 __attribute__((ext_vector_type(4)));
__device__ __forceinline__ void split_act4(f32x4 x, f16x4& hi, f16x4& lo) {
    f32x4 xz, lo32;
#pragma unroll
    for (int e = 0; e < 4; ++e) xz[e] = (fabsf(x[e]) < 6.103515625e-05f) ? 0.0f : x[e];
    hi = __builtin_convertvector(xz, f16x4);
    const f32x4 xs = x * f32x4{kLoScale, kLoScale, kLoScale, kLoScale};
#pragma unroll
    for (int e = 0; e < 4; ++e) lo32[e] = __builtin_fmaf((float)hi[e], -kLoScale, xs[e]);
    lo = __builtin_convertvector(lo32, f16x4);
}
__device__ __forceinline__ void split_act4_prod(f32x4 a, f32x4 b, f16x4& hi, f16x4& lo) {
    const f32x4 x = a * b;
    f32x4 xz, lo32;
#pragma unroll
    for (int e = 0; e < 4; ++e) xz[e] = (fabsf(x[e]) < 6.103515625e-05f) ? 0.0f : x[e];
    hi = __builtin_convertvector(xz, f16x4);
#pragma unroll
    for (int e = 0; e < 4; ++e) lo32[e] = __builtin_fmaf(a[e], b[e], -(float)hi[e]);
    lo = __builtin_convertvector(lo32 * f32x4{kLoScale, kLoScale, kLoScale, kLoScale}, f16x4);
}
__device__ __forceinline__ void store_split4(f32x4 o, unsigned short* y16, size_t row, int c, int lane, int D) {
    typedef _Float16 h4 __attribute__((ext_vector_type(4)));
    typedef unsigned int u32x2 __attribute__((ext_vector_type(2)));
    typedef unsigned int u32x4 __attribute__((ext_vector_type(4)));
    h4 hi, lo;
#pragma unroll
    for (int k = 0; k < 4; ++k) {
        _Float16 a, b;
        split_act(o[k], a, b);
        hi[k] = a;
        lo[k] = b;
    }
    const u32x2 H = __builtin_bit_cast(u32x2, hi), L = __builtin_bit_cast(u32x2, lo);
    const bool odd = lane & 1;
    const unsigned int s0 = odd ? H[0] : L[0], s1 = odd ? H[1] : L[1];
    const unsigned int r0 = __shfl_xor(s0, 1), r1 = __shfl_xor(s1, 1);
    const u32x4 out = odd ? u32x4{r0, r1, L[0], L[1]} : u32x4{H[0], H[1], r0, r1};
    *reinterpret_cast<u32x4*>(y16 + ki_off(row, 4 * (c & ~1), D) + (odd ? 32 : 0)) = out;
}
#endif

void launch_make_masked_windows(const int32_t* wt, const int32_t* win_start, const int32_t* mask_rel,
                                int B, int T, int32_t* tokens_out, hipStream_t s);
void launch_apply_mask(int32_t* tokens, const int32_t* mask_pos, int B, int T, hipStream_t s);
void launch_seq_stats(const int32_t* tokens, int B, int T, int token_dropout, float* scale,
                      int32_t* pos_idx, int32_t* kv_len, hipStream_t s, int mask_id = PGMI_TOK_MASK);
void launch_zero_pad_rows(const int32_t* tokens, int rows, int D, float* x, hipStream_t s);
void launch_embed(const int32_t* tokens, const float* scale, const int32_t* pos_idx,
                  const float* embed_tokens, const float* embed_positions, int token_dropout,
                  int rows, int T, int D, float* x, hipStream_t s, int mask_id = PGMI_TOK_MASK);
void launch_layernorm(const float* x, const float* w, const float* b, int rows, int D, float eps,
                      float* y, hipStream_t s);
void launch_gather_rows(const float* x, const int32_t* row_idx, int n, int D, float* y, hipStream_t s);
void launch_strided_index(int first, int stride, int n, int32_t* idx, hipStream_t s);
void launch_vocab_logsoftmax(const float* h, const float* E, const float* bias, int rows, int D,
                             int V, float* out, int32_t* nonfinite, hipStream_t s);
void launch_layernorm16(const float* x, const float* w, const float* b, int rows, int D, float eps,
                        unsigned short* y16, int mode, hipStream_t s);
int launch_rmsnorm16(const float* x, const float* w, int rows, int D, float eps, unsigned short* y16, hipStream_t s);
void launch_scatter_rows(const float* src, const int32_t* dst_row, int n, int V, float* table,
                         hipStream_t s);
void launch_row_index(const int32_t* mask_rel, int B, int T, int32_t* out, hipStream_t s);
void launch_fill_f32(float* p, int64_t n, float v, hipStream_t s);
void launch_seq_loglik(const float* lp, const int32_t* tokens, const int32_t* lens, int B, int T, int V,
                       const float* prior, const int32_t* a0, const int32_t* row0, const int32_t* n,
                       const int32_t* flip, float alpha, const float* eve, float beta, int eve_fallback, float* out, hipStream_t s);
void launch_seq_loglik_ragged(const float* lp, const int32_t* tokens, const int32_t* seq_off, const int32_t* seq_p,
                              const int32_t* seq_root, int B, int T, int V, const float* prior, const int32_t* a0,
                              const int32_t* row0, const int32_t* n, const int32_t* flip, float alpha, const float* eve, float beta,
                              int eve_fallback, float* out, hipStream_t s);
void launch_pg2_seq_loglik(const float* lp, const int32_t* col, const int32_t* n_kept, int B, int T, int V, float* out, hipStream_t s);
void launch_embed_learned(const int32_t* tokens, const float* E, const float* P, int rows, int T, int D, float* x, hipStream_t s);
void launch_embed_scaled_pos(const int32_t* tokens, const int32_t* pos, const float* E, const float* P, float scale, int rows, int D,
                             float* x, hipStream_t s);
void launch_wide_logsoftmax(const float* logits, int ldl, int rows, int V, const int32_t* tgt, float* out, int32_t* nonfinite,
                            hipStream_t s);
void launch_seq_sum(const float* terms, const int32_t* off, int B, double* out, hipStream_t s);
void launch_score_mutants(const float* table, int V, const int32_t* sub_pos, const int32_t* sub_wt,
                          const int32_t* sub_mt, const int64_t* mut_off, int64_t n_mut,
                          double* scores, hipStream_t s);
void launch_rotary(float* qkv, const float* cos_t, const float* sin_t, int rows, int T, int H,
                   hipStream_t s, int rot_halves = 1);
void launch_make_pppl_rows(const uint8_t* tok8, const int64_t* seq_off, const int32_t* sid, const int64_t* rp, int J,
                           int64_t g0, int bc, int T, int32_t* tokens, int32_t* row_idx, int32_t* target, hipStream_t s);
void launch_pppl_pick(const float* lp, const int32_t* target, int bc, int V, float* terms, hipStream_t s);
void launch_pppl_sum(const float* terms, const int64_t* rp, const int32_t* sid, int J, int64_t first, double* out, hipStream_t s);
void launch_saprot_rows(const int32_t* wt, const int32_t* set_off, const int32_t* set_pos, int s0, int bc, int T, int first, int groups,
                        int width, int32_t* tokens, int32_t* keep, hipStream_t s);
int launch_group_logsoftmax(const float* h, const float* E, const float* bias, int rows, int D, int V, int first, int groups, int width,
                            float* full, float* group, int32_t* nonfinite, hipStream_t s);
int group_logsoftmax_check(int D, int V, int first, int groups, int width);

struct MoeRoute {
    const float* gate = nullptr;
    int E = 0, top_k = 0;
    const int32_t* tokens = nullptr;
    int pad_id = 0;
    int32_t* ids = nullptr;
    float* wts = nullptr;
};
int launch_rmsnorm_route(const float* x, const float* w, int rows, int D, float eps, unsigned short* y16, const MoeRoute& r, hipStream_t s);
int moe_perm_blocks(int n_entries);
void launch_moe_permute(const int32_t* ids, int n_entries, int E, int tile, int32_t* blk_cnt, int32_t* blk_base, int32_t* counts_seg,
                        int32_t* slot, hipStream_t s);
void launch_moe_gather(const unsigned short* h16, const int32_t* slot, int n_entries, int top_k, int D, unsigned short* a16, hipStream_t s);
void launch_moe_combine(const float* y, const int32_t* slot, const float* wts, int rows, int top_k, int D, float* x, hipStream_t s);
void launch_silu_split(const float* t, int rows, int F, unsigned short* g16, hipStream_t s);

enum EveTensor { PGMI_EVE_T_Z = 0, PGMI_EVE_T_KEEP = 1, PGMI_EVE_T_W = 16, PGMI_EVE_T_B = 32, PGMI_EVE_T_WOUT = 48, PGMI_EVE_T_BOUT = 49,
                 PGMI_EVE_T_CONV = 50, PGMI_EVE_T_SPARSITY = 51, PGMI_EVE_T_TEMP = 52 };
void launch_eve_gather(const uint8_t* res, const float* W0t, const float* b, int rows, int L, int ld, int act, float* out, hipStream_t s);
void launch_eve_act(float* x, int rows, int n, int ld, int act, uint32_t keep24, float scale, uint64_t seed, uint32_t sample, int tensor,
                    int64_t row_base, const uint8_t* inj, int64_t inj_row0, hipStream_t s);
void launch_eve_latent(const float* mulv, int ldz, int64_t mulv_row0, int rows, int z, int ld, uint32_t keep24, float scale, uint64_t seed,
                       uint32_t sample, int64_t row_base, const float* inj_eps, const uint8_t* inj_keep, int64_t inj_row0, float* h,
                       hipStream_t s);
void launch_eve_sample(const float* mean, const float* sd, int64_t n, int K, int Kp, uint64_t seed, uint32_t sample, int tensor,
                       const float* inj, float* out, hipStream_t s);
void launch_eve_sample_final(const float* w_mean, const float* w_sd, const float* c_mean, const float* c_sd, const float* s_mean,
                             const float* s_sd, int L, int H, int Hp, int C, int Ht, bool conv, uint64_t seed, uint32_t sample,
                             const float* inj_w, const float* inj_c, const float* inj_s, float* out, hipStream_t s);
void launch_eve_elbo(const float* logits, const uint8_t* res, const float* mulv, int ldz, int z, const float* temp, int rows, int L,
                     int64_t loc0, float* elbo, float* bce, float* kld, double* acc, int first, hipStream_t s);
void launch_eve_fill_normal(uint64_t seed, uint32_t sample, int tensor, uint64_t e0, int64_t n, float* out, hipStream_t s);
void launch_eve_fill_keep(uint64_t seed, uint32_t sample, int tensor, uint64_t e0, int64_t n, uint32_t keep24, uint8_t* out, hipStream_t s);
constexpr int EVE_PRIOR_S = 4;
struct EvePriorPtrs { const float* p[EVE_PRIOR_S] = {nullptr, nullptr, nullptr, nullptr}; };
void launch_eve_prior_latent(const float* mulv, int z, int ld, uint64_t seed, uint32_t sample, const EvePriorPtrs& inj, int S, float* h,
                             hipStream_t s);
void launch_eve_prior_hidden(const float* w_mean, const float* w_sd, const float* b_mean, const float* b_sd, int N, int K, uint64_t seed,
                             uint32_t sample, int tw, int tb, const EvePriorPtrs& inj_w, const EvePriorPtrs& inj_b, int S, const float* x,
                             int ldx, int act, float* y, int ldy, hipStream_t s);
int eve_prior_blocks(int L, int H);
int eve_prior_kmax(int H);
int eve_prior_max_samples(int C, bool conv);
void launch_eve_prior_final(const float* w_mean, const float* w_sd, const float* c_mean, const float* c_sd, const float* s_mean,
                            const float* s_sd, int L, int H, int C, int Ht, bool conv, uint64_t seed, uint32_t sample,
                            const EvePriorPtrs& inj_w, const EvePriorPtrs& inj_c, const EvePriorPtrs& inj_s, int S, const float* h, int ldh,
                            float* partial, hipStream_t s);
void launch_eve_prior_finish(const float* partial, int S, const float* b_mean, const float* b_sd, const float* t_mean, const float* t_sd,
                             uint64_t seed, uint32_t sample, const EvePriorPtrs& inj_b, const EvePriorPtrs& inj_t, int L, int H, int sample0,
                             double* acc, hipStream_t s);
int eve_set_option(const char* name, long long value);

void launch_mpnn_graph(const float* X, const float* mask, int L, int K, int32_t* E_idx, float* D_nb, hipStream_t s);
void launch_mpnn_edge_feat(const float* X, const int32_t* ridx, const int32_t* chain, const int32_t* E_idx, const float* D_nb,
                           const float* Wpos, const float* bpos, const float* Wt, const float* ln_w, const float* ln_b, int L, int K, float* E,
                           hipStream_t s);
void launch_mpnn_concat(const float* hV, const float* hE, const int32_t* E_idx, int L, int K, float* out, hipStream_t s);
void launch_mpnn_edge_sum(const float* msg, const float* mask, const int32_t* E_idx, int L, int K, float* out, hipStream_t s);
void launch_mpnn_add_ln(const float* a, int64_t a_rows, const float* b, const float* bias, float kb, float div, const float* ln_w,
                        const float* ln_b, const float* rowmask, int L, int64_t rows, float* out, hipStream_t s);
int launch_mpnn_dec_edge(const float* Ep, const float* T, const float* Penc, const float* AP, int64_t ap_bstride, const float* W2,
                         const float* b2, const int32_t* E_idx, const float* mask, const uint8_t* S, const int32_t* rank, int B, int L, int K,
                         float* out, hipStream_t s);
void launch_mpnn_head(const float* h, const float* W, const float* bias, const uint8_t* S, int64_t rows, float* lp, float* nll,
                      hipStream_t s);
void launch_mpnn_score(const float* nll, const float* mask, int B, int L, double* out, hipStream_t s);
int mpnn_set_option(const char* name, long long value);

struct S2fMsgWeights {
    const float *wv0, *wsv0, *bsv0;
    const float *wh1, *ws1, *bs1, *wv1, *wsv1, *bsv1;
    const float *wh2, *ws2, *bs2, *wv2, *wsv2, *bsv2;
    int ldw;
};
int launch_s2f_message(const float* P, const float* VT, const float* Es, const float* ev, const float* whe, const float* Wnt,
                       const S2fMsgWeights& w, const int32_t* src, const int32_t* off, int L, int64_t nodes, float* ds, float* dv, hipStream_t s);
int launch_s2f_gvp_mid(const float* spre, const float* vh, const float* wv, const float* gpre, const float* nwh, int so,
                       int vo, int h, int h2, int relu, int lda, int64_t rows, float* outA, float* outV, hipStream_t s);
int launch_s2f_node_ln(const float* rs, const float* rv, const float* ds, const float* dv, const float* lnw, const float* lnb, const float* wh, int h, int vn, int lda, int64_t rows, float* os, float* ov,
                       float* outA, float* outV, hipStream_t s);
void launch_s2f_head(const float* x, const float* W, const float* bias, const float* seq, const float* plddt, float thr, int L, int64_t rows,
                     float* lp, hipStream_t s);
void launch_s2f_pick_logits(const float* lp, const int32_t* cols, int L, int T, int V, int64_t rows, float* out, hipStream_t s);
int s2f_set_option(const char* name, long long value);

void launch_mlstm_m(const float* g1, const float* Tmx, const int32_t* tok, int tok_stride, int rows, int Hp, unsigned short* m16,
                    float* m32, hipStream_t s);
struct MlstmGate {
    const float* z = nullptr;
    const float* Tx = nullptr;
    const int32_t* tok = nullptr;
    int tok_stride = 0;
    float* c = nullptr;
    unsigned short* h16 = nullptr;
    float* h32 = nullptr;
    float* hwin = nullptr;
    float* z_out = nullptr;
    int rows = 0, Hp = 0;
};
void launch_mlstm_gate(const MlstmGate& a, hipStream_t s);
void launch_mlstm_init(const float* ctab, const uint32_t* htab, const float* tlp, const int32_t* tgt, const int32_t* join, int rows,
                       int Hp, int Lc, float* c, uint32_t* h, float* terms, hipStream_t s);
void launch_mlstm_head(const float* hwin, size_t slot_stride, int W, const float* Wd, const float* bd, const int32_t* tgt,
                       const int32_t* join, int Lc, int t0, int nw, int rows, int Hp, float* terms, float* lp, hipStream_t s);
void launch_mlstm_score(const float* terms, const int32_t* tgt, int rows, int Lc, double* out, hipStream_t s);
int unirep_set_option(const char* name, long long value);

int launch_dilated_conv16(const unsigned short* A16, const unsigned short* W16, float out_scale, const float* bias, const int32_t* seg_off,
                          int n_seg, int64_t M, int C, int taps, int dilation, float* out32, hipStream_t s);
int launch_dilated_conv32(const float* x, const float* W, const float* bias, const int32_t* seg_off, int n_seg, int64_t M, int C, int taps,
                          int dilation, float* col, float* out32, hipStream_t s);
int launch_ln_gelu16(const float* x, const float* w, const float* b, int rows, int D, float eps, unsigned short* y16, hipStream_t s);
int launch_ln_gelu32(const float* x, const float* w, const float* b, int rows, int D, float eps, float* y, hipStream_t s);

void launch_msa_window_tokens(const int32_t* full, int R, int Tfull, int start, int Tw, int mask_col, int32_t* out, hipStream_t s);
void launch_add_row_embedding(float* x, const float* pe, int R, int C, int D, hipStream_t s);
void launch_permute_rows(const float* src, float* dst, int A, int B, int D, hipStream_t s);
void launch_tied_prep_qk(const float* qkv, int64_t M, int D, unsigned short* q16, unsigned short* k16, hipStream_t s);
void launch_pack_vt16(const float* qkv, int R, int C, int Kp, int H, unsigned short* Vt, hipStream_t s);
int launch_tied_softmax16(const float* part, int H, int S, int C, int Kp, float scale, unsigned short* P, hipStream_t s);
float tied_w_scale();
struct TiedRowLaunch {
    const float* qkv = nullptr;
    int R = 0, C = 0, H = 0;
    int S = 0;
    unsigned short* qctx16 = nullptr;
    unsigned short* k16 = nullptr;
    float* part = nullptr;
    float* p = nullptr;
    float* vt = nullptr;
    hipStream_t stream = nullptr;
};
int tied_row_kp(int C);
int tied_row_splits(int R, int C, int H);
int tied_row_check(int R, int C, int H, int S);
int launch_tied_row_attention(const TiedRowLaunch& t);

int launch_gemm_f32(const float* A, const float* W, const float* bias, const float* residual,
                    float* C, int M, int N, int K, int epilogue, hipStream_t s);

void gemm_options_from_env();
int gemm_set_option(const char* name, long long value);
struct GemmLaunch {
    const unsigned short* A = nullptr;
    const unsigned short* W = nullptr;
    float out_scale = 1.0f;
    const float* bias = nullptr;
    const float* residual = nullptr;
    float* out32 = nullptr;
    unsigned short* out16 = nullptr;
    int M = 0, N = 0, K = 0;
    int epilogue = EPI_NONE;
    bool bf = false;
    int variant = 0;
    hipStream_t stream = nullptr;
    struct Qkv {
        unsigned short* vt16 = nullptr;
        size_t vt_plane = 0, qk_plane = 0;
        const float* cos_t = nullptr;
        const float* sin_t = nullptr;
        int rotary = 0, T = 0, H = 0, rot_halves = 1;
    } qkv;
};
int launch_gemm16(const GemmLaunch& g);
struct XMap;
int launch_gemm16_ex(const unsigned short* A, const unsigned short* W, float* Cf, unsigned short* Ch, int M, int N, int K,
                     float out_scale, XMap xm, int nbatch, hipStream_t s);
void launch_split16(const float* x, int64_t n, float scale, int mode, int K, unsigned short* out, hipStream_t s);

int launch_qkln_prep(const float* qkv, const float* q_w, const float* k_w, float eps, const float* cos_t, const float* sin_t, int B,
                     int T, int H, unsigned short* qk16, size_t qk_plane, unsigned short* vt16, size_t vt_plane, hipStream_t s);

struct GeomAttLaunch {
    const float* proj = nullptr;
    int pitch = 0;
    const float *rot = nullptr, *trans = nullptr;
    const int32_t* mask = nullptr;
    bool per_row_frames = false;
    const float *w_rot = nullptr, *w_dist = nullptr;
    int B = 0, S = 0, H = 0;
    float* out = nullptr;
    int opitch = 0;
    hipStream_t stream = nullptr;
};
int launch_geom_attention(const GeomAttLaunch& g);
int geom_key_tile(int S);
void launch_esm3_embed(const int32_t* tokens, const int32_t* stok, const int32_t* plddt, const float* seq_embed, const float* struct_embed,
                       const float* cst, int rows, int T, int D, float* x, hipStream_t s);

int launch_attention_f32(const float* qkv, const int32_t* kv_len, int B, int T, int H, float* ctx, hipStream_t s,
                         int head_dim = 64);

enum AttOut {
    ATT_OUT_F32 = 0,
    ATT_OUT_SPLIT = 1,
    ATT_OUT_BF16 = 2
};
struct AttLaunch {
    unsigned short* qk16 = nullptr;
    size_t qk_plane = 0;
    unsigned short* vt16 = nullptr;
    size_t vt_plane = 0;
    int B = 1, T = 0, H = 0;
    int head_dim = 64;
    const int32_t* kv_len = nullptr;
    const float* slopes = nullptr;
    AttOut out = ATT_OUT_F32;
    float* ctx = nullptr;
    unsigned short* ctx16 = nullptr;
    hipStream_t stream = nullptr;
    const float* qkv = nullptr;
    const float* conv = nullptr;
    const float* cos_t = nullptr;
    const float* sin_t = nullptr;
    int rotary = 0;
};
int launch_attention_f16x3_v2(const AttLaunch& a);

struct AttRagged {
    const int32_t* seq_off;
    const int32_t* seq_p;
    const int32_t* seq_q;
    const int32_t* seq_root;
    const uint32_t* seq_vt;
    const int32_t* tile_seq;
    const int32_t* tile_j;
    const int32_t* blk_seq;
    const int32_t* blk_j;
    int n_tiles, n_blocks;
};
struct PrefixAttLaunch {
    const float* qkv = nullptr;
    const int32_t* pos = nullptr;
    const float* cos_t = nullptr;
    const float* sin_t = nullptr;
    const int32_t* seg_off = nullptr;
    const int32_t* ent_seg = nullptr;
    const int32_t* ent_tile = nullptr;
    int n_seg = 0, n_ent = 0, H = 0;
    unsigned short* q16 = nullptr;
    size_t q_plane = 0;
    unsigned short* k16 = nullptr;
    unsigned short* vt16 = nullptr;
    size_t pitch = 0;
    const unsigned short* pk16 = nullptr;
    const unsigned short* pvt16 = nullptr;
    size_t ppitch = 0;
    int P = 0;
    AttOut out = ATT_OUT_SPLIT;
    float* ctx = nullptr;
    unsigned short* ctx16 = nullptr;
    hipStream_t stream = nullptr;
};
int launch_prefix_prep(const PrefixAttLaunch& p);
int launch_prefix_attention(const PrefixAttLaunch& p);
int launch_cross_q_prep(const float* q, size_t rows, int H, unsigned short* q16, size_t q_plane, hipStream_t s);
int launch_cross_attention(const PrefixAttLaunch& p);

int att16_waves_per_block(int T);
int att_set_option(const char* name, long long value);
int launch_attention_tr_ragged(const AttLaunch& a, const AttRagged& rg);

}
```

### proteingym_amd/csrc/elementwise.hip

```cpp
#include "common.h"

namespace pgmi {

__device__ __forceinline__ float wave_sum(float v) {
#pragma unroll
    for (int o = 32; o > 0; o >>= 1) v += __shfl_xor(v, o);
    return v;
}
__device__ __forceinline__ float wave_max(float v) {
#pragma unroll
    for (int o = 32; o > 0; o >>= 1) v = fmaxf(v, __shfl_xor(v, o));
    return v;
}
__device__ __forceinline__ double wave_sum_d(double v) {
#pragma unroll
    for (int o = 32; o > 0; o >>= 1) v += __shfl_xor(v, o);
    return v;
}
__device__ __forceinline__ int wave_sum_i(int v) {
#pragma unroll
    for (int o = 32; o > 0; o >>= 1) v += __shfl_xor(v, o);
    return v;
}

__global__ void make_masked_windows_kernel(const int32_t* __restrict__ wt,
                                           const int32_t* __restrict__ win_start,
                                           const int32_t* __restrict__ mask_rel, int B, int T,
                                           int32_t* __restrict__ out) {
    const int64_t i = (int64_t)blockIdx.x * blockDim.x + threadIdx.x;
    if (i >= (int64_t)B * T) return;
    const int b = (int)(i / T), t = (int)(i % T);
    out[i] = (t == mask_rel[b]) ? PGMI_TOK_MASK : wt[win_start[b] + t];
}
void launch_make_masked_windows(const int32_t* wt, const int32_t* win_start, const int32_t* mask_rel,
                                int B, int T, int32_t* out, hipStream_t s) {
    const int64_t n = (int64_t)B * T;
    hipLaunchKernelGGL(make_masked_windows_kernel, dim3((unsigned)((n + 255) / 256)), dim3(256), 0, s,
                       wt, win_start, mask_rel, B, T, out);
}

__global__ void apply_mask_kernel(int32_t* tokens, const int32_t* __restrict__ mask_pos, int B, int T) {
    const int b = blockIdx.x * blockDim.x + threadIdx.x;
    if (b < B) tokens[(int64_t)b * T + mask_pos[b]] = PGMI_TOK_MASK;
}
void launch_apply_mask(int32_t* tokens, const int32_t* mask_pos, int B, int T, hipStream_t s) {
    hipLaunchKernelGGL(apply_mask_kernel, dim3((B + 255) / 256), dim3(256), 0, s, tokens, mask_pos, B, T);
}

__global__ void seq_stats_kernel(const int32_t* __restrict__ tokens, int B, int T, int token_dropout, int mask_id,
                                 float* __restrict__ denom, int32_t* __restrict__ pos_idx,
                                 int32_t* __restrict__ kv_len) {
    const int b = blockIdx.x * (blockDim.x >> 6) + (threadIdx.x >> 6);
    const int lane = threadIdx.x & 63;
    if (b >= B) return;
    const int32_t* tk = tokens + (int64_t)b * T;
    int running = 0, n_mask = 0, last_valid = -1;
    for (int t0 = 0; t0 < T; t0 += 64) {
        const int t = t0 + lane;
        const int tok = (t < T) ? tk[t] : PGMI_TOK_PAD;
        const int valid = (t < T) && (tok != PGMI_TOK_PAD);
        const unsigned long long bal = __ballot(valid);
        const unsigned long long below = bal & ((lane == 63) ? ~0ull : ((1ull << (lane + 1)) - 1ull));
        const int incl = __popcll(below);
        if (t < T) pos_idx[(int64_t)b * T + t] = valid ? (running + incl + PGMI_TOK_PAD) : PGMI_TOK_PAD;
        running += __popcll(bal);
        n_mask += __popcll(__ballot((t < T) && tok == mask_id));
        if (bal) last_valid = t0 + 63 - __clzll(bal);
    }
    if (lane == 0) {
        float d = 1.0f;
        if (token_dropout) d = 1.0f - (float)n_mask / (float)running;
        denom[b] = d;
        kv_len[b] = last_valid + 1;
    }
}
void launch_seq_stats(const int32_t* tokens, int B, int T, int token_dropout, float* denom,
                      int32_t* pos_idx, int32_t* kv_len, hipStream_t s, int mask_id) {
    hipLaunchKernelGGL(seq_stats_kernel, dim3((B + 3) / 4), dim3(256), 0, s, tokens, B, T, token_dropout, mask_id,
                       denom, pos_idx, kv_len);
}

__global__ void embed_kernel(const int32_t* __restrict__ tokens, const float* __restrict__ denom,
                             const int32_t* __restrict__ pos_idx, const float* __restrict__ E,
                             const float* __restrict__ P, int token_dropout, int mask_id, int rows, int T, int D,
                             float* __restrict__ x) {
    const int row = blockIdx.x * (blockDim.x >> 6) + (threadIdx.x >> 6);
    const int lane = threadIdx.x & 63;
    if (row >= rows) return;
    const int tok = tokens[row];
    const int b = row / T;
    const float dn = denom[b];
    const f32x4* e = reinterpret_cast<const f32x4*>(E + (size_t)tok * D);
    const f32x4* p = P ? reinterpret_cast<const f32x4*>(P + (size_t)pos_idx[row] * D) : nullptr;
    f32x4* xo = reinterpret_cast<f32x4*>(x + (size_t)row * D);
    const bool is_pad = tok == PGMI_TOK_PAD;
    const bool zero_emb = token_dropout && tok == mask_id;
    for (int i = lane; i < D / 4; i += 64) {
        f32x4 v = zero_emb ? f32x4{0.f, 0.f, 0.f, 0.f} : e[i];
        if (token_dropout) {
#pragma unroll
            for (int c = 0; c < 4; ++c) v[c] = (v[c] * 0.88f) / dn;
        }
        if (p) {
            const f32x4 pv = p[i];
#pragma unroll
            for (int c = 0; c < 4; ++c) v[c] += pv[c];
        }
        if (is_pad) v = f32x4{0.f, 0.f, 0.f, 0.f};
        xo[i] = v;
    }
}
void launch_embed(const int32_t* tokens, const float* denom, const int32_t* pos_idx, const float* E,
                  const float* P, int token_dropout, int rows, int T, int D, float* x, hipStream_t s, int mask_id) {
    hipLaunchKernelGGL(embed_kernel, dim3((rows + 3) / 4), dim3(256), 0, s, tokens, denom, pos_idx, E, P,
                       token_dropout, mask_id, rows, T, D, x);
}

__global__ void zero_pad_rows_kernel(const int32_t* __restrict__ tokens, int rows, int D, float* __restrict__ x) {
    const int row = blockIdx.x * 4 + (threadIdx.x >> 6);
    const int lane = threadIdx.x & 63;
    if (row >= rows || tokens[row] != PGMI_TOK_PAD) return;
    for (int i = lane; i < D; i += 64) x[(size_t)row * D + i] = 0.f;
}
void launch_zero_pad_rows(const int32_t* tokens, int rows, int D, float* x, hipStream_t s) {
    hipLaunchKernelGGL(zero_pad_rows_kernel, dim3((rows + 3) / 4), dim3(256), 0, s, tokens, rows, D, x);
}

template <int NV, int OUTMODE>
__global__ __launch_bounds__(256) void layernorm_kernel(const float* x,
                                                        const float* __restrict__ w,
                                                        const float* __restrict__ bsh, int rows, int D,
                                                        float eps, float* y, unsigned short* y16) {
    const int row = blockIdx.x * 4 + (threadIdx.x >> 6);
    const int lane = threadIdx.x & 63;
    if (row >= rows) return;
    const int nv = D >> 2;
    const f32x4* xr = reinterpret_cast<const f32x4*>(x + (size_t)row * D);
    f32x4 v[NV];
    float s = 0.f;
#pragma unroll
    for (int i = 0; i < NV; ++i) {
        const int c = lane + 64 * i;
        v[i] = (c < nv) ? xr[c] : f32x4{0.f, 0.f, 0.f, 0.f};
        s += (v[i][0] + v[i][1]) + (v[i][2] + v[i][3]);
    }
    const float mean = wave_sum(s) / (float)D;
    float q = 0.f;
#pragma unroll
    for (int i = 0; i < NV; ++i) {
        const int c = lane + 64 * i;
        if (c < nv) {
#pragma unroll
            for (int k = 0; k < 4; ++k) {
                const float d = v[i][k] - mean;
                q += d * d;
            }
        }
    }
    const float rstd = 1.0f / sqrtf(wave_sum(q) / (float)D + eps);
    const f32x4* wr = reinterpret_cast<const f32x4*>(w);
    const f32x4* br = reinterpret_cast<const f32x4*>(bsh);
#pragma unroll
    for (int i = 0; i < NV; ++i) {
        const int c = lane + 64 * i;
        if (c < nv) {
            const f32x4 wv = wr[c], bv = br[c];
            f32x4 o;
#pragma unroll
            for (int k = 0; k < 4; ++k) o[k] = (v[i][k] - mean) * rstd * wv[k] + bv[k];
            if constexpr (OUTMODE == 0) {
                reinterpret_cast<f32x4*>(y + (size_t)row * D)[c] = o;
            } else if constexpr (OUTMODE == 1) {
                typedef _Float16 h4 __attribute__((ext_vector_type(4)));
                h4 hi, lo;
#pragma unroll
                for (int k = 0; k < 4; ++k) {
                    _Float16 a, b2;
                    split_act(o[k], a, b2);
                    hi[k] = a;
                    lo[k] = b2;
                }
                typedef unsigned int u32x2 __attribute__((ext_vector_type(2)));
                typedef unsigned int u32x4 __attribute__((ext_vector_type(4)));
                const u32x2 H = __builtin_bit_cast(u32x2, hi), L = __builtin_bit_cast(u32x2, lo);
                const bool odd = lane & 1;
                const unsigned int s0 = odd ? H[0] : L[0], s1 = odd ? H[1] : L[1];
                const unsigned int r0 = __shfl_xor(s0, 1), r1 = __shfl_xor(s1, 1);
                const u32x4 out = odd ? u32x4{r0, r1, L[0], L[1]} : u32x4{H[0], H[1], r0, r1};
                unsigned short* dst = y16 + ki_off((size_t)row, 4 * (c & ~1), D) + (odd ? 32 : 0);
                *reinterpret_cast<u32x4*>(dst) = out;
            } else {
                typedef unsigned int u32x2 __attribute__((ext_vector_type(2)));
                unsigned short b[4];
#pragma unroll
                for (int k = 0; k < 4; ++k) {
                    const float ok = o[k];
                    unsigned int u = __builtin_bit_cast(unsigned int, ok);
                    u += 0x7fffu + ((u >> 16) & 1u);
                    b[k] = (unsigned short)(u >> 16);
                }
                u32x2 pk;
                pk[0] = b[0] | ((unsigned)b[1] << 16);
                pk[1] = b[2] | ((unsigned)b[3] << 16);
                reinterpret_cast<u32x2*>(y16 + (size_t)row * D)[c] = pk;
            }
        }
    }
}
template <int OUTMODE>
static void launch_ln_mode(const float* x, const float* w, const float* b, int rows, int D, float eps,
                           float* y, unsigned short* y16, hipStream_t s) {
    const dim3 grid((rows + 3) / 4), block(256);
    const int nv = (D / 4 + 63) / 64;
    if (nv <= 1) hipLaunchKernelGGL((layernorm_kernel<1, OUTMODE>), grid, block, 0, s, x, w, b, rows, D, eps, y, y16);
    else if (nv <= 2) hipLaunchKernelGGL((layernorm_kernel<2, OUTMODE>), grid, block, 0, s, x, w, b, rows, D, eps, y, y16);
    else if (nv <= 5) hipLaunchKernelGGL((layernorm_kernel<5, OUTMODE>), grid, block, 0, s, x, w, b, rows, D, eps, y, y16);
    else if (nv <= 10) hipLaunchKernelGGL((layernorm_kernel<10, OUTMODE>), grid, block, 0, s, x, w, b, rows, D, eps, y, y16);
    else hipLaunchKernelGGL((layernorm_kernel<20, OUTMODE>), grid, block, 0, s, x, w, b, rows, D, eps, y, y16);
}
void launch_layernorm(const float* x, const float* w, const float* b, int rows, int D, float eps,
                      float* y, hipStream_t s) {
    launch_ln_mode<0>(x, w, b, rows, D, eps, y, nullptr, s);
}
void launch_layernorm16(const float* x, const float* w, const float* b, int rows, int D, float eps,
                        unsigned short* y16, int mode, hipStream_t s) {
    if (mode == 1) launch_ln_mode<1>(x, w, b, rows, D, eps, nullptr, y16, s);
    else launch_ln_mode<2>(x, w, b, rows, D, eps, nullptr, y16, s);
}

template <int NV>
__global__ __launch_bounds__(256) void rmsnorm16_kernel(const float* __restrict__ x, const float* __restrict__ w, int rows, int D,
                                                        float eps, unsigned short* __restrict__ y16) {
    const int row = blockIdx.x * 4 + (threadIdx.x >> 6);
    const int lane = threadIdx.x & 63;
    if (row >= rows) return;
    const int nv = D >> 2;
    const f32x4* xr = reinterpret_cast<const f32x4*>(x + (size_t)row * D);
    f32x4 v[NV];
    float q = 0.f;
#pragma unroll
    for (int i = 0; i < NV; ++i) {
        const int c = lane + 64 * i;
        v[i] = (c < nv) ? xr[c] : f32x4{0.f, 0.f, 0.f, 0.f};
        q += (v[i][0] * v[i][0] + v[i][1] * v[i][1]) + (v[i][2] * v[i][2] + v[i][3] * v[i][3]);
    }
    const float rstd = 1.0f / sqrtf(wave_sum(q) / (float)D + eps);
    const f32x4* wr = reinterpret_cast<const f32x4*>(w);
#pragma unroll
    for (int i = 0; i < NV; ++i) {
        const int c = lane + 64 * i;
        if (c < nv) {
            const f32x4 wv = wr[c];
            f32x4 o;
#pragma unroll
            for (int k = 0; k < 4; ++k) o[k] = v[i][k] * rstd * wv[k];
            store_split4(o, y16, (size_t)row, c, lane, D);
        }
    }
}
int launch_rmsnorm16(const float* x, const float* w, int rows, int D, float eps, unsigned short* y16, hipStream_t s) {
    if (rows <= 0 || D <= 0 || D % 32 || D > 5120) { set_error("rmsnorm: D = %d must be a multiple of 32, at most 5120", D); return PGMI_EINVAL; }
    const dim3 grid((rows + 3) / 4), block(256);
    const int nv = (D / 4 + 63) / 64;
    if (nv <= 1) hipLaunchKernelGGL((rmsnorm16_kernel<1>), grid, block, 0, s, x, w, rows, D, eps, y16);
    else if (nv <= 2) hipLaunchKernelGGL((rmsnorm16_kernel<2>), grid, block, 0, s, x, w, rows, D, eps, y16);
    else if (nv <= 5) hipLaunchKernelGGL((rmsnorm16_kernel<5>), grid, block, 0, s, x, w, rows, D, eps, y16);
    else if (nv <= 10) hipLaunchKernelGGL((rmsnorm16_kernel<10>), grid, block, 0, s, x, w, rows, D, eps, y16);
    else hipLaunchKernelGGL((rmsnorm16_kernel<20>), grid, block, 0, s, x, w, rows, D, eps, y16);
    return PGMI_OK;
}

__global__ void rotary_kernel(float* __restrict__ qkv, const float* __restrict__ cos_t,
                              const float* __restrict__ sin_t, int64_t n, int T, int H, int rh) {
    const int64_t i = (int64_t)blockIdx.x * blockDim.x + threadIdx.x;
    if (i >= n) return;
    const int d = (int)(i & 31);
    const int64_t j = i >> 5;
    const int h = (int)(j % H);
    const int64_t k2 = j / H;
    const int which = (int)(k2 & 1);
    const int64_t row = k2 >> 1;
    const int t = (int)(row % T);
    float* p = qkv + row * (size_t)(3 * H * 64) + (size_t)which * H * 64 + h * 64 + d;
    const float x1 = p[0], x2 = p[32];
    const int tr = (t * rh + (h % rh)) * 64;
    const float c1 = cos_t[tr + d], s1 = sin_t[tr + d];
    const float c2 = cos_t[tr + d + 32], s2 = sin_t[tr + d + 32];
    p[0] = x1 * c1 + (-x2) * s1;
    p[32] = x2 * c2 + x1 * s2;
}
void launch_rotary(float* qkv, const float* cos_t, const float* sin_t, int rows, int T, int H, hipStream_t s, int rot_halves) {
    const int64_t n = (int64_t)rows * 2 * H * 32;
    hipLaunchKernelGGL(rotary_kernel, dim3((unsigned)((n + 255) / 256)), dim3(256), 0, s, qkv, cos_t, sin_t, n, T, H, rot_halves);
}

__global__ void gather_rows_kernel(const float* __restrict__ x, const int32_t* __restrict__ idx, int n,
                                   int D, float* __restrict__ y) {
    const int row = blockIdx.x * 4 + (threadIdx.x >> 6);
    const int lane = threadIdx.x & 63;
    if (row >= n) return;
    const f32x4* src = reinterpret_cast<const f32x4*>(x + (size_t)idx[row] * D);
    f32x4* dst = reinterpret_cast<f32x4*>(y + (size_t)row * D);
    for (int i = lane; i < D / 4; i += 64) dst[i] = src[i];
}
void launch_gather_rows(const float* x, const int32_t* idx, int n, int D, float* y, hipStream_t s) {
    hipLaunchKernelGGL(gather_rows_kernel, dim3((n + 3) / 4), dim3(256), 0, s, x, idx, n, D, y);
}

__global__ void esm3_embed_kernel(const int32_t* __restrict__ tokens, const int32_t* __restrict__ stok, const int32_t* __restrict__ plddt,
                                  const float* __restrict__ seq_embed, const float* __restrict__ struct_embed, const float* __restrict__ cst,
                                  int n, int T, int D, float* __restrict__ x) {
    const int row = blockIdx.x * 4 + (threadIdx.x >> 6);
    const int lane = threadIdx.x & 63;
    if (row >= n) return;
    const int t = row % T;
    const f32x4* a = reinterpret_cast<const f32x4*>(seq_embed + (size_t)tokens[row] * D);
    const f32x4* b = reinterpret_cast<const f32x4*>(struct_embed + (size_t)stok[t] * D);
    const f32x4* c = reinterpret_cast<const f32x4*>(cst + (size_t)(plddt[t] != 0) * D);
    f32x4* dst = reinterpret_cast<f32x4*>(x + (size_t)row * D);
    for (int i = lane; i < D / 4; i += 64) dst[i] = (a[i] + b[i]) + c[i];
}
void launch_esm3_embed(const int32_t* tokens, const int32_t* stok, const int32_t* plddt, const float* seq_embed, const float* struct_embed,
                       const float* cst, int rows, int T, int D, float* x, hipStream_t s) {
    hipLaunchKernelGGL(esm3_embed_kernel, dim3((rows + 3) / 4), dim3(256), 0, s, tokens, stok, plddt, seq_embed, struct_embed, cst, rows, T, D, x);
}

__global__ void strided_index_kernel(int first, int stride, int n, int32_t* __restrict__ idx) {
    const int i = blockIdx.x * blockDim.x + threadIdx.x;
    if (i < n) idx[i] = first + i * stride;
}
void launch_strided_index(int first, int stride, int n, int32_t* idx, hipStream_t s) {
    hipLaunchKernelGGL(strided_index_kernel, dim3((n + 255) / 256), dim3(256), 0, s, first, stride, n, idx);
}

__global__ void scatter_rows_kernel(const float* __restrict__ src, const int32_t* __restrict__ dst_row,
                                    int n, int V, float* __restrict__ table) {
    const int i = blockIdx.x * blockDim.x + threadIdx.x;
    if (i >= n * V) return;
    const int rI = i / V, c = i % V;
    table[(size_t)dst_row[rI] * V + c] = src[i];
}
void launch_scatter_rows(const float* src, const int32_t* dst_row, int n, int V, float* table, hipStream_t s) {
    hipLaunchKernelGGL(scatter_rows_kernel, dim3((n * V + 255) / 256), dim3(256), 0, s, src, dst_row, n, V, table);
}

__global__ void row_index_kernel(const int32_t* __restrict__ mask_rel, int B, int T, int32_t* __restrict__ out) {
    const int b = blockIdx.x * blockDim.x + threadIdx.x;
    if (b < B) out[b] = b * T + mask_rel[b];
}
void launch_row_index(const int32_t* mask_rel, int B, int T, int32_t* out, hipStream_t s) {
    hipLaunchKernelGGL(row_index_kernel, dim3((B + 255) / 256), dim3(256), 0, s, mask_rel, B, T, out);
}

__global__ void fill_f32_kernel(float* p, int64_t n, float v) {
    const int64_t i = (int64_t)blockIdx.x * blockDim.x + threadIdx.x;
    if (i < n) p[i] = v;
}
void launch_fill_f32(float* p, int64_t n, float v, hipStream_t s) {
    hipLaunchKernelGGL(fill_f32_kernel, dim3((unsigned)((n + 255) / 256)), dim3(256), 0, s, p, n, v);
}

__global__ __launch_bounds__(256) void vocab_logsoftmax_kernel(const float* __restrict__ h,
                                                               const float* __restrict__ E,
                                                               const float* __restrict__ bias, int rows,
                                                               int D, int V, float* __restrict__ out,
                                                               int32_t* __restrict__ nonfinite) {
    const int row = blockIdx.x * 4 + (threadIdx.x >> 6);
    const int lane = threadIdx.x & 63;
    if (row >= rows) return;
    const float* hr = h + (size_t)row * D;
    double my_logit = -INFINITY;
    for (int v = 0; v < V; ++v) {
        const float* ev = E + (size_t)v * D;
        double acc = 0.0;
        for (int i = lane; i < D; i += 64) acc = fma((double)hr[i], (double)ev[i], acc);
        acc = wave_sum_d(acc);
        if (lane == v) my_logit = acc + (double)bias[v];
    }
    const float mx = wave_max((float)my_logit);
    const double ex = (lane < V) ? exp(my_logit - (double)mx) : 0.0;
    const double lse = log(wave_sum_d(ex));
    const float res = (float)((my_logit - (double)mx) - lse);
    if (lane < V) {
        out[(size_t)row * V + lane] = res;
        if (nonfinite && !(fabsf(res) <= 3.0e38f)) atomicOr(nonfinite, 1);
    }
}
void launch_vocab_logsoftmax(const float* h, const float* E, const float* bias, int rows, int D, int V,
                             float* out, int32_t* nonfinite, hipStream_t s) {
    hipLaunchKernelGGL(vocab_logsoftmax_kernel, dim3((rows + 3) / 4), dim3(256), 0, s, h, E, bias, rows, D, V, out, nonfinite);
}

__device__ __forceinline__ float fuse_eve(float two, float e, float beta, int eve_fallback) {
    if (eve_fallback && e == -INFINITY) return two;
    return (1.0f - beta) * two + beta * e;
}
__global__ __launch_bounds__(256) void seq_loglik_kernel(const float* __restrict__ lp, const int32_t* __restrict__ tokens,
                                                         const int32_t* __restrict__ lens, int B, int T, int V,
                                                         const float* __restrict__ prior, const int32_t* __restrict__ a0,
                                                         const int32_t* __restrict__ row0, const int32_t* __restrict__ n,
                                                         const int32_t* __restrict__ flip, float alpha,
                                                         const float* __restrict__ eve, float beta, int eve_fallback,
                                                         float* __restrict__ out) {
    const int b = blockIdx.x * 4 + (threadIdx.x >> 6);
    const int lane = threadIdx.x & 63;
    if (b >= B) return;
    const int len = lens[b];
    float acc = 0.f;
    for (int t = lane; t < len - 1; t += 64) {
        const int tgt = tokens[(size_t)b * T + t + 1];
        float v = lp[((size_t)b * T + t) * V + tgt];
        if (prior && n[b] > 0 && t >= a0[b] && t < a0[b] + n[b]) {
            const int i = t - a0[b];
            const int row = flip[b] ? row0[b] + (n[b] - 1 - i) : row0[b] + i;
            v = (1.0f - alpha) * v + alpha * prior[(size_t)row * V + tgt];
            if (eve) v = fuse_eve(v, eve[(size_t)row * V + tgt], beta, eve_fallback);
        }
        acc += v;
    }
    acc = wave_sum(acc);
    if (lane == 0) out[b] = acc;
}
__global__ __launch_bounds__(256) void seq_loglik_ragged_kernel(const float* __restrict__ lp, const int32_t* __restrict__ tokens,
                                                                const int32_t* __restrict__ seq_off, const int32_t* __restrict__ seq_p,
                                                                const int32_t* __restrict__ seq_root, int B, int T, int V,
                                                                const float* __restrict__ prior, const int32_t* __restrict__ a0,
                                                                const int32_t* __restrict__ row0, const int32_t* __restrict__ n,
                                                                const int32_t* __restrict__ flip, float alpha,
                                                                const float* __restrict__ eve, float beta, int eve_fallback,
                                                                float* __restrict__ out) {
    const int b = blockIdx.x * 4 + (threadIdx.x >> 6);
    const int lane = threadIdx.x & 63;
    if (b >= B) return;
    const int a = seq_p[b], own0 = seq_off[b] - a, root0 = seq_off[seq_root[b]];
    float acc = 0.f;
    for (int t = lane; t < T - 1; t += 64) {
        const int tgt = tokens[(t + 1 < a) ? root0 + t + 1 : own0 + t + 1];
        float v = lp[(size_t)((t < a) ? root0 + t : own0 + t) * V + tgt];
        if (prior && n[b] > 0 && t >= a0[b] && t < a0[b] + n[b]) {
            const int i = t - a0[b];
            const int row = flip[b] ? row0[b] + (n[b] - 1 - i) : row0[b] + i;
            v = (1.0f - alpha) * v + alpha * prior[(size_t)row * V + tgt];
            if (eve) v = fuse_eve(v, eve[(size_t)row * V + tgt], beta, eve_fallback);
        }
        acc += v;
    }
    acc = wave_sum(acc);
    if (lane == 0) out[b] = acc;
}
void launch_seq_loglik_ragged(const float* lp, const int32_t* tokens, const int32_t* seq_off, const int32_t* seq_p,
                              const int32_t* seq_root, int B, int T, int V, const float* prior, const int32_t* a0,
                              const int32_t* row0, const int32_t* n, const int32_t* flip, float alpha, const float* eve, float beta,
                              int eve_fallback, float* out, hipStream_t s) {
    hipLaunchKernelGGL(seq_loglik_ragged_kernel, dim3((B + 3) / 4), dim3(256), 0, s, lp, tokens, seq_off, seq_p, seq_root, B, T, V,
                       prior, a0, row0, n, flip, alpha, eve, beta, eve_fallback, out);
}
void launch_seq_loglik(const float* lp, const int32_t* tokens, const int32_t* lens, int B, int T, int V,
                       const float* prior, const int32_t* a0, const int32_t* row0, const int32_t* n,
                       const int32_t* flip, float alpha, const float* eve, float beta, int eve_fallback, float* out, hipStream_t s) {
    hipLaunchKernelGGL(seq_loglik_kernel, dim3((B + 3) / 4), dim3(256), 0, s, lp, tokens, lens, B, T, V, prior, a0, row0, n,
                       flip, alpha, eve, beta, eve_fallback, out);
}

__global__ __launch_bounds__(256) void pg2_seq_loglik_kernel(const float* __restrict__ lp, const int32_t* __restrict__ col,
                                                             const int32_t* __restrict__ n_kept, int B, int T, int V,
                                                             float* __restrict__ out) {
    const int b = blockIdx.x * 4 + (threadIdx.x >> 6);
    const int lane = threadIdx.x & 63;
    if (b >= B) return;
    const int n = n_kept[b];
    double acc = 0.0;
    for (int t = lane; t < n; t += 64) acc += (double)lp[((size_t)b * T + t) * V + col[(size_t)b * T + t]];
    acc = wave_sum_d(acc);
    if (lane == 0) out[b] = (float)acc;
}
void launch_pg2_seq_loglik(const float* lp, const int32_t* col, const int32_t* n_kept, int B, int T, int V, float* out, hipStream_t s) {
    hipLaunchKernelGGL(pg2_seq_loglik_kernel, dim3((B + 3) / 4), dim3(256), 0, s, lp, col, n_kept, B, T, V, out);
}

__global__ void score_mutants_kernel(const float* __restrict__ table, int V,
                                     const int32_t* __restrict__ sub_pos,
                                     const int32_t* __restrict__ sub_wt,
                                     const int32_t* __restrict__ sub_mt,
                                     const int64_t* __restrict__ mut_off, int64_t n_mut,
                                     double* __restrict__ scores) {
    const int64_t i = (int64_t)blockIdx.x * blockDim.x + threadIdx.x;
    if (i >= n_mut) return;
    double sc = 0.0;
    for (int64_t k = mut_off[i]; k < mut_off[i + 1]; ++k) {
        const float* rowp = table + (size_t)sub_pos[k] * V;
        const float d = rowp[sub_mt[k]] - rowp[sub_wt[k]];
        sc += (double)d;
    }
    scores[i] = sc;
}
void launch_score_mutants(const float* table, int V, const int32_t* sub_pos, const int32_t* sub_wt,
                          const int32_t* sub_mt, const int64_t* mut_off, int64_t n_mut, double* scores,
                          hipStream_t s) {
    if (n_mut <= 0) return;
    hipLaunchKernelGGL(score_mutants_kernel, dim3((unsigned)((n_mut + 255) / 256)), dim3(256), 0, s, table, V,
                       sub_pos, sub_wt, sub_mt, mut_off, n_mut, scores);
}


__global__ __launch_bounds__(256) void make_pppl_rows_kernel(const uint8_t* __restrict__ tok8, const int64_t* __restrict__ seq_off,
                                                             const int32_t* __restrict__ sid, const int64_t* __restrict__ rp, int J,
                                                             int64_t g0, int bc, int T, int32_t* __restrict__ tokens,
                                                             int32_t* __restrict__ row_idx, int32_t* __restrict__ target) {
    const int b = blockIdx.x * 4 + (threadIdx.x >> 6);
    const int lane = threadIdx.x & 63;
    if (b >= bc) return;
    const int64_t g = g0 + b;
    int lo = 0, hi = J;
    while (hi - lo > 1) {
        const int mid = (lo + hi) >> 1;
        if (rp[mid] <= g) lo = mid; else hi = mid;
    }
    const int n = sid[lo];
    const int i = 1 + (int)(g - rp[lo]);
    const int64_t o = seq_off[n];
    const int len = (int)(seq_off[n + 1] - o);
    int32_t* out = tokens + (int64_t)b * T;
    for (int t = lane; t < T; t += 64) out[t] = (t == i) ? PGMI_TOK_MASK : (t < len ? (int32_t)tok8[o + t] : PGMI_TOK_PAD);
    if (lane == 0) {
        row_idx[b] = b * T + i;
        target[b] = (int32_t)tok8[o + i + 1];
    }
}
void launch_make_pppl_rows(const uint8_t* tok8, const int64_t* seq_off, const int32_t* sid, const int64_t* rp, int J,
                           int64_t g0, int bc, int T, int32_t* tokens, int32_t* row_idx, int32_t* target, hipStream_t s) {
    hipLaunchKernelGGL(make_pppl_rows_kernel, dim3((bc + 3) / 4), dim3(256), 0, s, tok8, seq_off, sid, rp, J, g0, bc, T,
                       tokens, row_idx, target);
}

__global__ void pppl_pick_kernel(const float* __restrict__ lp, const int32_t* __restrict__ target, int bc, int V,
                                 float* __restrict__ terms) {
    const int b = blockIdx.x * blockDim.x + threadIdx.x;
    if (b < bc) terms[b] = lp[(size_t)b * V + target[b]];
}
void launch_pppl_pick(const float* lp, const int32_t* target, int bc, int V, float* terms, hipStream_t s) {
    hipLaunchKernelGGL(pppl_pick_kernel, dim3((bc + 255) / 256), dim3(256), 0, s, lp, target, bc, V, terms);
}

__global__ void pppl_sum_kernel(const float* __restrict__ terms, const int64_t* __restrict__ rp, const int32_t* __restrict__ sid,
                                int J, int64_t first, double* __restrict__ out) {
    const int j = blockIdx.x * blockDim.x + threadIdx.x;
    if (j >= J) return;
    double acc = 0.0;
    for (int64_t g = rp[j]; g < rp[j + 1]; ++g) acc += (double)terms[g];
    out[sid[j] - first] = acc;
}
void launch_pppl_sum(const float* terms, const int64_t* rp, const int32_t* sid, int J, int64_t first, double* out, hipStream_t s) {
    if (J <= 0) return;
    hipLaunchKernelGGL(pppl_sum_kernel, dim3((J + 127) / 128), dim3(128), 0, s, terms, rp, sid, J, first, out);
}


__global__ __launch_bounds__(256) void embed_learned_kernel(const int32_t* __restrict__ tokens, const float* __restrict__ E,
                                                            const float* __restrict__ P, int rows, int T, int D, float* __restrict__ x) {
    const int row = blockIdx.x * 4 + (threadIdx.x >> 6);
    const int lane = threadIdx.x & 63;
    if (row >= rows) return;
    const f32x4* e = reinterpret_cast<const f32x4*>(E + (size_t)tokens[row] * D);
    const f32x4* p = reinterpret_cast<const f32x4*>(P + (size_t)(row % T) * D);
    f32x4* xo = reinterpret_cast<f32x4*>(x + (size_t)row * D);
    for (int i = lane; i < D / 4; i += 64) xo[i] = e[i] + p[i];
}
void launch_embed_learned(const int32_t* tokens, const float* E, const float* P, int rows, int T, int D, float* x, hipStream_t s) {
    hipLaunchKernelGGL(embed_learned_kernel, dim3((rows + 3) / 4), dim3(256), 0, s, tokens, E, P, rows, T, D, x);
}

__global__ __launch_bounds__(256) void embed_scaled_pos_kernel(const int32_t* __restrict__ tokens, const int32_t* __restrict__ pos,
                                                               const float* __restrict__ E, const float* __restrict__ P, float scale,
                                                               int rows, int D, float* __restrict__ x) {
    const int row = blockIdx.x * 4 + (threadIdx.x >> 6);
    const int lane = threadIdx.x & 63;
    if (row >= rows) return;
    const f32x4* e = reinterpret_cast<const f32x4*>(E + (size_t)tokens[row] * D);
    const f32x4* p = reinterpret_cast<const f32x4*>(P + (size_t)pos[row] * D);
    f32x4* xo = reinterpret_cast<f32x4*>(x + (size_t)row * D);
    for (int i = lane; i < D / 4; i += 64) {
        const f32x4 ev = e[i], pv = p[i];
        f32x4 o;
#pragma unroll
        for (int k = 0; k < 4; ++k) o[k] = fmaf(scale, ev[k], pv[k]);
        xo[i] = o;
    }
}
void launch_embed_scaled_pos(const int32_t* tokens, const int32_t* pos, const float* E, const float* P, float scale, int rows, int D,
                             float* x, hipStream_t s) {
    hipLaunchKernelGGL(embed_scaled_pos_kernel, dim3((rows + 3) / 4), dim3(256), 0, s, tokens, pos, E, P, scale, rows, D, x);
}

__device__ __forceinline__ void lse_merge(float& m, double& s, float m2, double s2) {
    const float M = fmaxf(m, m2);
    const double a = s == 0.0 ? 0.0 : s * exp((double)m - (double)M);
    const double b = s2 == 0.0 ? 0.0 : s2 * exp((double)m2 - (double)M);
    m = M;
    s = a + b;
}
__global__ __launch_bounds__(256) void wide_logsoftmax_kernel(const float* __restrict__ logits, int ldl, int V,
                                                              const int32_t* __restrict__ tgt, float* __restrict__ out,
                                                              int32_t* __restrict__ nonfinite) {
    __shared__ float sm[256];
    __shared__ double ss[256];
    const int r = blockIdx.x, tid = threadIdx.x;
    const float* row = logits + (size_t)r * ldl;
    const f32x4* row4 = reinterpret_cast<const f32x4*>(row);
    float m = -INFINITY;
    double s = 0.0;
    for (int i = tid; i < (V + 3) / 4; i += 256) {
        const f32x4 v = row4[i];
        const int c0 = 4 * i;
        float mx = m;
#pragma unroll
        for (int k = 0; k < 4; ++k)
            if (c0 + k < V) mx = fmaxf(mx, v[k]);
        if (mx > m) {
            s = s == 0.0 ? 0.0 : s * (double)__expf(m - mx);
            m = mx;
        }
        float e = 0.0f;
#pragma unroll
        for (int k = 0; k < 4; ++k)
            if (c0 + k < V) e += v[k] == -INFINITY ? 0.0f : __expf(v[k] - m);
        s += (double)e;
    }
    sm[tid] = m;
    ss[tid] = s;
    __syncthreads();
    for (int o = 128; o > 0; o >>= 1) {
        if (tid < o) {
            float a = sm[tid];
            double b = ss[tid];
            lse_merge(a, b, sm[tid + o], ss[tid + o]);
            sm[tid] = a;
            ss[tid] = b;
        }
        __syncthreads();
    }
    const double lse = (double)sm[0] + log(ss[0]);
    bool bad = false;
    if (tgt) {
        if (tid == 0) {
            const float res = (float)((double)row[tgt[r]] - lse);
            out[r] = res;
            bad = !(fabsf(res) <= 3.0e38f);
        }
    } else {
        for (int c = tid; c < V; c += 256) {
            const float res = (float)((double)row[c] - lse);
            out[(size_t)r * V + c] = res;
            bad |= !(fabsf(res) <= 3.0e38f);
        }
    }
    if (nonfinite && bad) atomicOr(nonfinite, 1);
}
void launch_wide_logsoftmax(const float* logits, int ldl, int rows, int V, const int32_t* tgt, float* out, int32_t* nonfinite,
                            hipStream_t s) {
    if (rows <= 0) return;
    hipLaunchKernelGGL(wide_logsoftmax_kernel, dim3(rows), dim3(256), 0, s, logits, ldl, V, tgt, out, nonfinite);
}

__global__ void seq_sum_kernel(const float* __restrict__ terms, const int32_t* __restrict__ off, int B, double* __restrict__ out) {
    const int b = blockIdx.x * blockDim.x + threadIdx.x;
    if (b >= B) return;
    double acc = 0.0;
    for (int i = off[b]; i < off[b + 1]; ++i) acc += (double)terms[i];
    out[b] = acc;
}
void launch_seq_sum(const float* terms, const int32_t* off, int B, double* out, hipStream_t s) {
    hipLaunchKernelGGL(seq_sum_kernel, dim3((B + 127) / 128), dim3(128), 0, s, terms, off, B, out);
}

__global__ __launch_bounds__(256) void saprot_rows_kernel(const int32_t* __restrict__ wt, const int32_t* __restrict__ set_off,
                                                          const int32_t* __restrict__ set_pos, int s0, int bc, int T, int first,
                                                          int groups, int width, int32_t* __restrict__ tokens,
                                                          int32_t* __restrict__ keep) {
    const int b = blockIdx.x * 4 + (threadIdx.x >> 6);
    const int lane = threadIdx.x & 63;
    if (b >= bc) return;
    const int e0 = set_off[s0], lo0 = set_off[s0 + b], hi0 = set_off[s0 + b + 1];
    int32_t* out = tokens + (int64_t)b * T;
    for (int t = lane; t < T; t += 64) {
        int lo = lo0, hi = hi0;
        while (lo < hi) {
            const int mid = (lo + hi) >> 1;
            if (set_pos[mid] < t) lo = mid + 1; else hi = mid;
        }
        const int id = wt[t];
        const bool masked = lo < hi0 && set_pos[lo] == t && id >= first;
        out[t] = masked ? first + (groups - 1) * width + (id - first) % width : id;
    }
    for (int e = lo0 + lane; e < hi0; e += 64) keep[e - e0] = b * T + set_pos[e];
}
void launch_saprot_rows(const int32_t* wt, const int32_t* set_off, const int32_t* set_pos, int s0, int bc, int T, int first, int groups,
                        int width, int32_t* tokens, int32_t* keep, hipStream_t s) {
    hipLaunchKernelGGL(saprot_rows_kernel, dim3((bc + 3) / 4), dim3(256), 0, s, wt, set_off, set_pos, s0, bc, T, first, groups, width,
                       tokens, keep);
}

constexpr int kGroupSlots = 8;
template <int NV>
__global__ __launch_bounds__(256) void group_logsoftmax_kernel(const float* __restrict__ h, const float* __restrict__ E,
                                                               const float* __restrict__ bias, int rows, int D, int V, int first,
                                                               int groups, int width, float* __restrict__ full,
                                                               float* __restrict__ group, int32_t* __restrict__ nonfinite) {
    const int row = blockIdx.x * 4 + (threadIdx.x >> 6);
    const int lane = threadIdx.x & 63;
    if (row >= rows) return;
    const int nv = D >> 2;
    const f32x4* hr = reinterpret_cast<const f32x4*>(h + (size_t)row * D);
    f32x4 x[NV];
#pragma unroll
    for (int i = 0; i < NV; ++i) {
        const int c = lane + 64 * i;
        x[i] = (c < nv) ? hr[c] : f32x4{0.f, 0.f, 0.f, 0.f};
    }
    double lg[kGroupSlots];
#pragma unroll
    for (int j = 0; j < kGroupSlots; ++j) {
        lg[j] = -INFINITY;
        for (int l = 0; l < 64; ++l) {
            const int v = 64 * j + l;
            if (v >= V) break;
            const f32x4* ev = reinterpret_cast<const f32x4*>(E + (size_t)v * D);
            double acc = 0.0;
#pragma unroll
            for (int i = 0; i < NV; ++i) {
                const int c = lane + 64 * i;
                if (c < nv) {
                    const f32x4 e = ev[c];
#pragma unroll
                    for (int k = 0; k < 4; ++k) acc = fma((double)x[i][k], (double)e[k], acc);
                }
            }
            acc = wave_sum_d(acc);
            if (lane == l) lg[j] = acc + (double)bias[v];
        }
    }
    float mx = -INFINITY;
#pragma unroll
    for (int j = 0; j < kGroupSlots; ++j) mx = fmaxf(mx, (float)lg[j]);
    mx = wave_max(mx);
    double ex = 0.0;
#pragma unroll
    for (int j = 0; j < kGroupSlots; ++j) ex += (64 * j + lane < V) ? exp(lg[j] - (double)mx) : 0.0;
    const double lse = (double)mx + log(wave_sum_d(ex));
    bool bad = false;
    if (full) {
#pragma unroll
        for (int j = 0; j < kGroupSlots; ++j) {
            const int v = 64 * j + lane;
            if (v < V) {
                const float res = (float)(lg[j] - lse);
                full[(size_t)row * V + v] = res;
                bad |= !(fabsf(res) <= 3.0e38f);
            }
        }
    }
    if (group) {
        float mine = 0.f;
        for (int g = 0; g < groups; ++g) {
            const int c0 = first + g * width;
            double val = -INFINITY;
#pragma unroll
            for (int j = 0; j < kGroupSlots; ++j) {
                const int v = 64 * j + lane;
                if (v >= c0 && v < c0 + width && v < V) val = lg[j];
            }
            const float gm = wave_max((float)val);
            const double gs = wave_sum_d(val == -INFINITY ? 0.0 : exp(val - (double)gm));
            const float res = (float)(((double)gm + log(gs)) - lse);
            if (lane == g) mine = res;
        }
        if (lane < groups) {
            group[(size_t)row * groups + lane] = mine;
            bad |= !(fabsf(mine) <= 3.0e38f);
        }
    }
    if (nonfinite && bad) atomicOr(nonfinite, 1);
}
int group_logsoftmax_check(int D, int V, int first, int groups, int width) {
    const int nv = (D / 4 + 63) / 64;
    if (D % 4 || nv > 10 || V > 64 * kGroupSlots || groups > 64 || width > 64 || first + groups * width > V) {
        set_error("grouped log-softmax: unsupported shape (D %d, V %d, %d groups of %d from column %d)", D, V, groups, width, first);
        return PGMI_EINVAL;
    }
    return PGMI_OK;
}
int launch_group_logsoftmax(const float* h, const float* E, const float* bias, int rows, int D, int V, int first, int groups, int width,
                            float* full, float* group, int32_t* nonfinite, hipStream_t s) {
    if (rows <= 0) return PGMI_OK;
    const int nv = (D / 4 + 63) / 64;
    if (int rc = group_logsoftmax_check(D, V, first, groups, width)) return rc;
    const dim3 grid((rows + 3) / 4), block(256);
#define PGMI_GLS(N) hipLaunchKernelGGL((group_logsoftmax_kernel<N>), grid, block, 0, s, h, E, bias, rows, D, V, first, groups, width, full, group, nonfinite)
    if (nv <= 1) PGMI_GLS(1); else if (nv <= 2) PGMI_GLS(2); else if (nv <= 5) PGMI_GLS(5); else PGMI_GLS(10);
#undef PGMI_GLS
    return PGMI_OK;
}

}
```

### proteingym_amd/csrc/model.h

```cpp
#pragma once
#include <math.h>
#include <stdlib.h>
#include <cmath>
#include <algorithm>
#include <stdarg.h>
#include <stdio.h>
#include <string.h>

#include <string>
#include <vector>

#include "common.h"
#include "gemm16x_kernel.h"
#include "packed_chunks.h"

namespace pgmi {

struct W16 {
    unsigned short* p = nullptr;
    float out_scale = 1.0f;
};

struct Layer {
    float *ln1_w, *ln1_b, *wqkv, *bqkv, *wo, *bo, *ln2_w, *ln2_b, *w1, *b1, *w2, *b2;
    W16 wqkv16, wo16, w116, w216;
    float* conv = nullptr;
    float *c_ln_w = nullptr, *c_ln_b = nullptr, *c_bqkv = nullptr, *c_bo = nullptr;
    W16 c_wqkv16, c_wo16;
    float* c_bq = nullptr;
    W16 c_wq16;
    float *q_ln = nullptr, *k_ln = nullptr;
    float* gate = nullptr;
    std::vector<W16> ew1, ew2;
    float *g_norm_w = nullptr, *g_wrot = nullptr, *g_wdist = nullptr;
    W16 g_proj16, g_out16;
};

struct ProfEvent {
    hipEvent_t start, stop;
    int cls;
};

struct PrefixCache {
    unsigned short* planes = nullptr;
    size_t pitch = 0, plane = 0, cap = 0;
    int rows = 0;
    int32_t* meta = nullptr;
    static size_t plan_ints(size_t cap) { return 3 * cap + 2; }
    static size_t meta_ints(size_t cap) { return 2 * plan_ints(cap) + cap + 4; }
    unsigned short* k(int l) const { return planes ? planes + (size_t)l * 4 * plane : nullptr; }
    unsigned short* vt(int l) const { return planes ? k(l) + 2 * plane : nullptr; }
    int32_t* plan(int slot) const { return meta + (size_t)slot * plan_ints(cap); }
    int32_t* seq_off() const { return plan(2); }
};

}

using namespace pgmi;

struct pgmi_assay;
struct pgmi_pppl;

struct pgmi_model {
    pgmi_config cfg;
    int device = 0;
    hipStream_t stream = nullptr;
    std::vector<void*> allocs;
    std::vector<pgmi_assay*> assays;
    std::vector<pgmi_pppl*> pppls;
    float *embed_tokens = nullptr, *embed_positions = nullptr;
    float *lnb_w = nullptr, *lnb_b = nullptr, *lna_w = nullptr, *lna_b = nullptr;
    float *hd_w = nullptr, *hd_b = nullptr, *hln_w = nullptr, *hln_b = nullptr;
    float *head_w = nullptr, *head_b = nullptr;
    std::vector<Layer> layers;
    W16 hd16;
    int fc1_epi = EPI_GELU, fc1_cols = 0;
    bool embed_gather = false;
    int mask_id = PGMI_TOK_MASK, n_token_ids = PGMI_VOCAB;
    float* slopes = nullptr;
    float* tr_prior = nullptr;
    size_t tr_prior_cap = 0;
    int32_t* tr_meta = nullptr;
    size_t tr_meta_cap = 0;
    int pg2_rotary = 0;
    float *pg2_aa_w = nullptr, *pg2_aa_b = nullptr;
    int gpt_Vp = 0, gpt_head_rows = 0;
    bool parallel_residual = false;
    float* gpt_logits = nullptr;
    W16 gpt_head16;
    double* gpt_sum = nullptr;
    bool rms_norm = false;
    int pg3_E = 0, pg3_k = 0, pg3_gated = 0;
    struct MoeWs {
        int32_t *ids = nullptr, *slot = nullptr, *blk_cnt = nullptr, *blk_base = nullptr, *counts_seg = nullptr;
        float *wts = nullptr, *y = nullptr, *t32 = nullptr;
        unsigned short *a16 = nullptr, *g16 = nullptr;
        int32_t* counts_host = nullptr;
        size_t layer_stride = 0;
    } moe;
    float* msa_pe = nullptr;
    float* xt = nullptr;
    int32_t *msa_full = nullptr, *msa_kv_len = nullptr;
    size_t msa_full_cap = 0;
    float *tied_part = nullptr, *tied_p = nullptr, *tied_vt = nullptr;
    size_t tied_part_cap = 0, tied_p_cap = 0, tied_vt_cap = 0;
    int msa_kv_R = 0, msa_kv_C = 0;
    float ln_eps = 1e-5f;
    bool final_norm = false;
    PrefixCache pfx;
    std::vector<float> poet_prompt_lp;
    int if1_enc = 0, if1_pos_len = 0;
    float *if1_mem = nullptr, *if1_pos = nullptr;
    unsigned short* if1_mem16 = nullptr;
    int e3_vheads = 0, e3_Kp = 0;
    float *e3_struct_embed = nullptr, *e3_const = nullptr;
    int32_t *e3_stok = nullptr, *e3_plddt = nullptr, *e3_mask = nullptr;
    float *e3_rot = nullptr, *e3_trans = nullptr;
    size_t e3_cap = 0;
    int e3_T = 0;
    bool e3_framed = false;
    unsigned short *h16 = nullptr, *g16 = nullptr;
    size_t h16_plane = 0, g16_plane = 0;
    unsigned short *qk16 = nullptr, *vt16 = nullptr;
    size_t qk16_plane = 0, vt16_plane = 0;
    int32_t* nonfinite = nullptr;
    int gemm_variant = 0;
    int keep_rows = 1;
    int last_B = 0, last_T = 0;
    int dh = kHeadDim;
    int rot_halves = 1;
    int Hs = 0;
    int Da = 0;
    float *rot_cos = nullptr, *rot_sin = nullptr;
    int rot_len = 0;
    float* zeros = nullptr;
    int max_rows = 0;
    float *x = nullptr, *h = nullptr, *qkv = nullptr, *g = nullptr, *lp = nullptr, *denom = nullptr;
    int32_t *tokens = nullptr, *pos_idx = nullptr, *kv_len = nullptr, *row_idx = nullptr, *aux_i = nullptr;
    bool prof = false;
    std::vector<ProfEvent> events;
    size_t events_used = 0;
    double prof_ms[PGMI_K_COUNT] = {0};
    int64_t prof_n[PGMI_K_COUNT] = {0};
    double prof_flops[PGMI_K_COUNT] = {0};
    double prof_bytes[PGMI_K_COUNT] = {0};
};

struct pgmi_assay {
    pgmi_model* m = nullptr;
    int n_tok = 0, P = 0, T = 0;
    int64_t n_mut = 0, n_sub = 0;
    std::vector<void*> allocs;
    int32_t *wt = nullptr, *positions = nullptr, *win_start = nullptr, *mask_rel = nullptr;
    int32_t *sub_pos = nullptr, *sub_wt = nullptr, *sub_mt = nullptr;
    int64_t* mut_off = nullptr;
    float* table = nullptr;
    double* scores = nullptr;
};

struct pgmi_pppl {
    pgmi_model* m = nullptr;
    int64_t N = 0;
    std::vector<int64_t> off;
    std::vector<void*> allocs;
    uint8_t* tok8 = nullptr;
    int64_t* off_dev = nullptr;
    int64_t last_rows = 0, last_chunks = 0, last_tokens = 0, last_padded = 0;
};

namespace pgmi {

template <typename T>
int dev_alloc(std::vector<void*>& pool, T** p, size_t n) {
    void* q = nullptr;
    if (n == 0) n = 1;
    hipError_t e = hipMalloc(&q, n * sizeof(T));
    if (e != hipSuccess) {
        set_error("hipMalloc(%zu bytes) failed: %s", n * sizeof(T), hipGetErrorString(e));
        return PGMI_ENOMEM;
    }
    pool.push_back(q);
    *p = static_cast<T*>(q);
    return PGMI_OK;
}

template <typename T>
int dev_upload(std::vector<void*>& pool, T** p, const T* host, size_t n) {
    int rc = dev_alloc(pool, p, n);
    if (rc) return rc;
    if (n) PGMI_HIP(hipMemcpy(*p, host, n * sizeof(T), hipMemcpyHostToDevice));
    return PGMI_OK;
}

struct ProfScope {
    pgmi_model* m;
    ProfEvent* ev = nullptr;
    ProfScope(pgmi_model* m_, int cls, double flops, double bytes) : m(m_) {
        if (!m->prof) return;
        if (m->events_used == m->events.size()) {
            ProfEvent e;
            if (hipEventCreate(&e.start) != hipSuccess || hipEventCreate(&e.stop) != hipSuccess) return;
            m->events.push_back(e);
        }
        ev = &m->events[m->events_used++];
        ev->cls = cls;
        m->prof_n[cls] += 1;
        m->prof_flops[cls] += flops;
        m->prof_bytes[cls] += bytes;
        hipEventRecord(ev->start, m->stream);
    }
    ~ProfScope() {
        if (ev) hipEventRecord(ev->stop, m->stream);
    }
};

template <typename T>
int ensure_cap(pgmi_model* m, T** p, size_t* cap, size_t need) {
    if (need <= *cap) return PGMI_OK;
    T* q = nullptr;
    int rc = dev_alloc(m->allocs, &q, need);
    if (rc) return rc;
    *p = q;
    *cap = need;
    return PGMI_OK;
}

int prof_drain(pgmi_model* m);
int check_cfg(const pgmi_config* c);
int check_tokens(const int32_t* tokens, int B, int T, int n_ids = PGMI_VOCAB);
int check_vocab(const int32_t* tokens, int B, int T, int V);
int env_int(const char* name, int dflt);
int make_w16(std::vector<void*>& pool, const float* host, size_t n, size_t K, int precision, hipStream_t s, W16* out);
int linear(pgmi_model* m, const float* in32, const unsigned short* in16, const float* W32, const W16& w16, const float* bias,
           const float* residual, float* out32, unsigned short* out16, int M, int N, int K, int epi);
GemmLaunch qkv_launch(pgmi_model* m, const W16& w16, const float* bias, int M, int Da, int K, int T, int H);
PrefixAttLaunch prefix_launch(pgmi_model* m, const SegPlan& pl);
int alloc_prefix_cache(pgmi_model* m);
int check_nonfinite(pgmi_model* m);
int reset_pad_keys(pgmi_model* m, int B, int T);
int model_create(const pgmi_config* cfg, const float* w, int64_t n_weights, int device, pgmi_model** out, int arch_arg,
                 const pgmi_pg3_params* pg3 = nullptr);
int create_esm(pgmi_model* m, const pgmi_config* cfg, const float* w, int64_t n_weights);
int ensure_rotary(pgmi_model* m, int T);
int upload_rotate_half(pgmi_model* m, int n);
int run_encoder(pgmi_model* m, int B, int T, const int32_t* keep = nullptr, int n_keep = 0, bool* compacted = nullptr);
int head_hidden(pgmi_model* m, int R, const int32_t* row_idx);
int run_head(pgmi_model* m, int R, const int32_t* row_idx);
int run_rows(pgmi_model* m, int B, int T, int R, const int32_t* row_idx);
int create_tranception(pgmi_model* m, const pgmi_config* cfg, const float* w, int64_t n_weights);
int create_progen2(pgmi_model* m, const pgmi_config* cfg, const float* w, int64_t n_weights, int rotary_dim);
int create_gpt(pgmi_model* m, const pgmi_config* cfg, const float* w, int64_t n_weights, int pos_kind);
int64_t gpt_weight_count(const pgmi_config* c, int pos_kind);
int decoder_check(pgmi_model* m, int arch, int T);
int run_decoder(pgmi_model* m, int B, int T, const AttRagged* rg = nullptr, int rows = 0, double att_flops = 0);
int self_attention(pgmi_model* m, const Layer& L, int B, int T, const AttRagged* rg = nullptr, int rows = 0, double att_flops = 0);
int out_proj(pgmi_model* m, const W16& wo16, const float* bo, int M);
int ffn(pgmi_model* m, const Layer& L, int M);
int narrow_head(pgmi_model* m, const float* src, int n);
int loglik_tail(pgmi_model* m, const int32_t* row_idx, int R, const int32_t* d_off, int bc, double* sum);
int decoder_token_logprobs(pgmi_model* m, int arch, const int32_t* tokens, int B, int T, float* out);
int decoder_sequence_loglik(pgmi_model* m, int arch, const int32_t* tokens, const int32_t* lens, int B, int T, double* sum, int32_t* n_targets);
int pg3_check(const pgmi_config* c, const pgmi_pg3_params* p);
int64_t pg3_weight_count(const pgmi_config* c, const pgmi_pg3_params* p);
int create_progen3(pgmi_model* m, const pgmi_config* cfg, const float* w, int64_t n_weights, const pgmi_pg3_params* p);
void pack_swiglu(const float* w1, const float* w3, size_t F, size_t D, float* dst);
int moe_ws_alloc(std::vector<void*>& pool, pgmi_model::MoeWs* ws, size_t rows, size_t layers, int D, int F, int E, int top_k, int gated);
int dense_ffn(pgmi_model* m, const pgmi_model::MoeWs& ws, const W16& w1, const W16& w2, const unsigned short* h16, unsigned short* g16,
              int M, int D, int F, int gated, float* x);
int pg3_ffn(pgmi_model* m, const Layer& L, int layer, int M);
int moe_ffn(pgmi_model* m, const pgmi_model::MoeWs& ws, const std::vector<W16>& ew1, const std::vector<W16>& ew2,
            const unsigned short* h16, const int32_t* ids, const float* wts, int M, int D, int F, int E, int top_k, int gated, float* x);
int64_t poet_weight_count(const pgmi_config* c, int final_norm);
int create_poet(pgmi_model* m, const pgmi_config* cfg, const float* w, int64_t n_weights, int final_norm);
struct PackedScorer {
    int (*forward)(pgmi_model* m, int bc, int R, const SegPlan& pl);
    int pos_len;
    const char* pos_what;
    const char* not_ready;
    bool same_length;
    bool vocab_per_row;
    int skip_target;
    bool mean;
};
int score_packed(pgmi_model* m, const PackedScorer& e, const int32_t* tokens, const int32_t* lens, int B, int T, bool loglik, float* out,
                 double* sum);
int if1_check(const pgmi_config* c, int enc_dim);
int64_t if1_weight_count(const pgmi_config* c, int enc_dim);
int create_esmif1(pgmi_model* m, const pgmi_config* cfg, const float* w, int64_t n_weights, int enc_dim);
int64_t esmc_weight_count(const pgmi_config* c);
int create_esmc(pgmi_model* m, const pgmi_config* cfg, const float* w, int64_t n_weights);
int esm3_check(const pgmi_config* c, int v_heads);
int64_t esm3_weight_count(const pgmi_config* c, int v_heads);
int create_esm3(pgmi_model* m, const pgmi_config* cfg, const float* w, int64_t n_weights, int v_heads);
int esm3_embed(pgmi_model* m, int B, int T);
int geom_branch(pgmi_model* m, const Layer& L, int B, int T);
int create_saprot(pgmi_model* m, const pgmi_config* cfg, const float* w, int64_t n_weights, int mask_id);
int create_msa(pgmi_model* m, const pgmi_config* cfg, const float* w, int64_t n_weights);
int run_msa(pgmi_model* m, int R, int C, int keep_col = -1, bool* compacted = nullptr);

inline bool esm2_rotary(int arch) { return arch == PGMI_ARCH_ESM2 || arch == PGMI_ARCH_SAPROT; }
inline bool esmc_blocks(int arch) { return arch == PGMI_ARCH_ESMC || arch == PGMI_ARCH_ESM3; }

struct BlobCursor {
    pgmi_model* m;
    const float *p, *end;
    int rc = PGMI_OK;
    BlobCursor(pgmi_model* m_, const float* w, int64_t n_weights) : m(m_), p(w), end(w + n_weights) {}
    const float* take(size_t n) { p += n; return p - n; }
    void upload(float** dst, const float* host, size_t n) { if (!rc) rc = dev_upload(m->allocs, dst, host, n); }
    void upload(float** dst, size_t n) { upload(dst, take(n), n); }
    void w16(W16* dst, const float* host, size_t n, size_t K) { if (!rc) rc = make_w16(m->allocs, host, n, K, m->cfg.precision, m->stream, dst); }
    void w16(W16* dst, size_t n, size_t K) { w16(dst, take(n), n, K); }
    void linear(float** w32, W16* w16_, const float* host, size_t n, size_t K) {
        if (m->cfg.precision == PGMI_PREC_FP32) upload(w32, host, n); else w16(w16_, host, n, K);
    }
    void linear(float** w32, W16* w16_, size_t n, size_t K) { linear(w32, w16_, take(n), n, K); }
    int finish() {
        if (!rc && p != end) { set_error("internal: blob walk mismatch"); rc = PGMI_EINVAL; }
        return rc;
    }
};

inline size_t rotate_half_slot(size_t col, size_t dh) {
    const size_t h = col / dh, j = col % dh;
    if (dh > 64) return (2 * h + ((j >> 5) & 1)) * 64 + ((j >> 6) << 5) + (j & 31);
    return h * 64 + (j < dh / 2 ? j : 32 + (j - dh / 2));
}

template <typename Slot>
void pack_qkv_slots(const float* src, size_t D, size_t Da, Slot slot, float qscale, float* wq, float* bq = nullptr) {
    for (size_t k = 0; k < 3; ++k) {
        const float sc = (k == 0) ? qscale : 1.0f;
        for (size_t o = 0; o < D; ++o) {
            float* dst = &wq[(k * Da + slot(o)) * D];
            for (size_t i = 0; i < D; ++i) dst[i] = src[o * D + i] * sc;
        }
        src += D * D;
        if (!bq) continue;
        for (size_t o = 0; o < D; ++o) bq[k * Da + slot(o)] = src[o] * sc;
        src += D;
    }
}

template <typename Slot>
void pack_out_cols(const float* src, size_t D, size_t Da, Slot slot, float* wo) {
    for (size_t o = 0; o < D; ++o)
        for (size_t i = 0; i < D; ++i) wo[o * Da + slot(i)] = src[o * D + i];
}

template <typename Angle>
int upload_rotary(pgmi_model* m, int n, int groups, Angle angle) {
    std::vector<float> c((size_t)n * groups * 64), s((size_t)n * groups * 64);
    for (int t = 0; t < n; ++t)
        for (int g = 0; g < groups; ++g)
            for (int i = 0; i < 32; ++i) {
                const float f = angle(t, g, i);
                const size_t o = ((size_t)t * groups + g) * 64;
                c[o + i] = c[o + 32 + i] = cosf(f);
                s[o + i] = s[o + 32 + i] = sinf(f);
            }
    int rc = dev_upload(m->allocs, &m->rot_cos, c.data(), c.size());
    if (!rc) rc = dev_upload(m->allocs, &m->rot_sin, s.data(), s.size());
    if (!rc) m->rot_len = n;
    return rc;
}

inline size_t own_pitch(const pgmi_model* m) { return own_pitch(m->max_rows); }

inline int upload_plan(pgmi_model* m, SegPlan& p, int slot) {
    p.d_seg_off = m->pfx.plan(slot);
    p.d_ent_seg = p.d_seg_off + m->pfx.cap + 2;
    p.d_ent_tile = p.d_ent_seg + m->pfx.cap;
    PGMI_HIP(hipMemcpyAsync(p.d_seg_off, p.seg_off.data(), p.seg_off.size() * 4, hipMemcpyHostToDevice, m->stream));
    PGMI_HIP(hipMemcpyAsync(p.d_ent_seg, p.ent_seg.data(), p.ent_seg.size() * 4, hipMemcpyHostToDevice, m->stream));
    PGMI_HIP(hipMemcpyAsync(p.d_ent_tile, p.ent_tile.data(), p.ent_tile.size() * 4, hipMemcpyHostToDevice, m->stream));
    return PGMI_OK;
}

inline int rows_per_chunk(const pgmi_model* m, int T) { return std::max(1, m->max_rows / ((T + 31) / 32 * 32)); }

template <typename Fn>
int for_each_chunk(pgmi_model* m, int B, int T, Fn fn) {
    const int per = rows_per_chunk(m, T);
    for (int b0 = 0; b0 < B; b0 += per) {
        int rc = fn(b0, std::min(per, B - b0));
        if (rc) return rc;
        PGMI_HIP(hipStreamSynchronize(m->stream));
    }
    return PGMI_OK;
}

}
```

Baseline: 18660.

## Share layer-0 QKV across masked windows and restrict last-layer attention to kept tiles

```diff
diff --git a/proteingym_amd/csrc/api_esm.hip b/proteingym_amd/csrc/api_esm.hip
--- a/proteingym_amd/csrc/api_esm.hip
+++ b/proteingym_amd/csrc/api_esm.hip
@@ -59,10 +59,22 @@
     });
 }
 
-int run_encoder(pgmi_model* m, int B, int T, const int32_t* keep, int n_keep, bool* compacted) {
+static struct { int on = 1; bool set = false; } g_mm_share;
+void mm_share_from_env() {
+    if (!g_mm_share.set) g_mm_share.on = env_int("PGMI_MM_SHARE", 1);
+}
+int esm_set_option(const char* name, long long value) {
+    if (strcmp(name, "mm_share")) return PGMI_EINVAL;
+    g_mm_share.set = value >= 0;
+    if (value >= 0) g_mm_share.on = (int)value; else mm_share_from_env();
+    return PGMI_OK;
+}
+
+int run_encoder(pgmi_model* m, int B, int T, const int32_t* keep, int n_keep, bool* compacted, const MaskedWindows* mw) {
     const pgmi_config& c = m->cfg;
     const int M = B * T, D = c.embed_dim, F = c.ffn_dim, N1 = m->fc1_cols, H = c.heads, Da = m->Da;
     hipStream_t s = m->stream;
+    if (!g_mm_share.on) mw = nullptr;
     if (c.arch == PGMI_ARCH_ESM1B && T > c.max_positions) {
         set_error("Sequence length %d above maximum sequence length of %d", T, c.max_positions);
         return PGMI_EINVAL;
@@ -86,20 +98,33 @@
     const int mode16 = (prec == PGMI_PREC_F16X3) ? 1 : 2;
     for (int l = 0; l < c.layers; ++l) {
         const Layer& L = m->layers[l];
-        { ProfScope p(m, PGMI_K_LAYERNORM, 0, ln_bytes);
+        const bool fused_qkv = prec != PGMI_PREC_FP32 && !L.q_ln;
+        const bool share = l == 0 && mw && mw->same_window && fused_qkv && (c.arch == PGMI_ARCH_ESM1B || c.arch == PGMI_ARCH_ESM2) &&
+                           B >= 2 && c.layers > 1 && !L.g_norm_w && (size_t)B * ((T + 31) / 32 * 32) <= (size_t)m->max_rows;
+        const int Mq = share ? 2 * T : M, Tp = (T + 31) / 32 * 32;
+        unsigned short* const cqk = reinterpret_cast<unsigned short*>(m->qkv);
+        unsigned short* const cvt = cqk + (size_t)2 * Mq * 2 * Da;
+        { ProfScope p(m, PGMI_K_LAYERNORM, 0, share ? 2.0 * Mq * D * 4 * 2 : ln_bytes);
+          if (share) launch_mm_share_gather(m->x, mw->mask_rel, B, T, D, m->h, s);
           if (prec == PGMI_PREC_FP32) launch_layernorm(m->x, L.ln1_w, L.ln1_b, M, D, 1e-5f, m->h, s);
-          else launch_layernorm16(m->x, L.ln1_w, L.ln1_b, M, D, 1e-5f, m->h16, mode16, s); }
-        const bool fused_qkv = prec != PGMI_PREC_FP32 && !L.q_ln;
-        { ProfScope p(m, PGMI_K_GEMM_QKV, 2.0 * M * 3 * D * D, 0);
+          else launch_layernorm16(share ? m->h : m->x, L.ln1_w, L.ln1_b, Mq, D, 1e-5f, m->h16, mode16, s); }
+        { ProfScope p(m, PGMI_K_GEMM_QKV, 2.0 * Mq * 3 * D * D, share ? ((double)M * 2 * Da + (double)B * Da * Tp) * 4 : 0);
           if (fused_qkv) {
-              GemmLaunch g = qkv_launch(m, L.wqkv16, L.bqkv, M, Da, D, T, m->Hs);
+              GemmLaunch g = qkv_launch(m, L.wqkv16, L.bqkv, Mq, Da, D, T, m->Hs);
               g.bf = prec == PGMI_PREC_BF16;
               g.qkv.cos_t = m->rot_cos; g.qkv.sin_t = m->rot_sin; g.qkv.rotary = esm2_rotary(c.arch); g.qkv.rot_halves = m->rot_halves;
+              if (share) {
+                  g.out16 = cqk; g.qkv.qk_plane = (size_t)Mq * 2 * Da;
+                  g.qkv.vt16 = cvt; g.qkv.vt_plane = (size_t)2 * Da * Tp;
+              }
               rc = launch_gemm16(g);
+              if (!rc && share)
+                  launch_mm_share_broadcast(cqk, cvt, mw->mask_rel, B, T, Da, m->qk16, m->qk16_plane, m->vt16, m->vt16_plane, s);
           } else
               rc = linear(m, m->h, m->h16, L.wqkv, L.wqkv16, L.bqkv, nullptr, m->qkv, nullptr, M, 3 * Da, D, EPI_NONE);
           if (rc) return rc; }
-        { ProfScope p(m, PGMI_K_ATTENTION, 4.0 * M * T * D, L.q_ln ? (double)M * D * 20 : 0);
+        const bool kept_tile = mw && keep && m->keep_rows && l == c.layers - 1 && !L.g_norm_w && prec != PGMI_PREC_FP32 && m->rot_halves == 1;
+        { ProfScope p(m, PGMI_K_ATTENTION, 4.0 * (kept_tile ? B * 32 : M) * T * D, L.q_ln ? (double)M * D * 20 : 0);
           if (L.q_ln && (rc = launch_qkln_prep(m->qkv, L.q_ln, L.k_ln, 1e-5f, m->rot_cos, m->rot_sin, B, T, H, m->qk16, m->qk16_plane,
                                                m->vt16, m->vt16_plane, s)))
               return rc;
@@ -110,6 +135,7 @@
               a.qk16 = m->qk16, a.qk_plane = m->qk16_plane, a.vt16 = m->vt16, a.vt_plane = m->vt16_plane;
               a.B = B, a.T = T, a.H = H, a.head_dim = m->rot_halves * kHeadDim;
               a.kv_len = m->kv_len;
+              if (kept_tile) a.kept_q = mw->mask_rel;
               a.out = prec == PGMI_PREC_F16X3 ? ATT_OUT_SPLIT : ATT_OUT_BF16;
               a.ctx16 = m->h16;
               a.stream = s;
@@ -188,9 +214,9 @@
 }
 
 
-int run_rows(pgmi_model* m, int B, int T, int R, const int32_t* row_idx) {
+int run_rows(pgmi_model* m, int B, int T, int R, const int32_t* row_idx, const MaskedWindows* mw) {
     bool compacted = false;
-    int rc = run_encoder(m, B, T, row_idx, R, &compacted);
+    int rc = run_encoder(m, B, T, row_idx, R, &compacted, mw);
     if (rc) return rc;
     return run_head(m, R, compacted ? nullptr : row_idx);
 }
@@ -274,6 +300,8 @@
     PGMI_HIP(hipSetDevice(m->device));
     pgmi_assay* a = new pgmi_assay();
     a->m = m; a->n_tok = n_tok; a->P = P; a->T = T; a->n_mut = n_mut; a->n_sub = n_sub;
+    a->win_start_host = ws; a->mask_rel_host = mr;
+    a->wt_has_mask = std::find(wt_tokens, wt_tokens + n_tok, m->mask_id) != wt_tokens + n_tok;
     int rc = dev_upload(a->allocs, &a->wt, wt_tokens, (size_t)n_tok);
     if (!rc) rc = dev_upload(a->allocs, &a->positions, positions, (size_t)P);
     if (!rc) rc = dev_upload(a->allocs, &a->win_start, ws.data(), (size_t)P);
@@ -309,11 +337,21 @@
     const int T = a->T, V = m->cfg.vocab;
     const int per = rows_per_chunk(m, T);
     launch_fill_f32(a->table, (int64_t)a->n_tok * V, NAN, s);
+    std::vector<char> seen;
     for (int p0 = 0; p0 < a->P; p0 += per) {
         const int bc = std::min(per, a->P - p0);
+        MaskedWindows mw;
+        mw.mask_rel = a->mask_rel + p0;
+        mw.same_window = !a->wt_has_mask;
+        seen.assign((size_t)T, 0);
+        for (int b = 0; b < bc && mw.same_window; ++b) {
+            char& hit = seen[(size_t)a->mask_rel_host[p0 + b]];
+            mw.same_window = a->win_start_host[p0 + b] == a->win_start_host[p0] && !hit;
+            hit = 1;
+        }
         launch_make_masked_windows(a->wt, a->win_start + p0, a->mask_rel + p0, bc, T, m->tokens, s);
         launch_row_index(a->mask_rel + p0, bc, T, m->row_idx, s);
-        int rc = run_rows(m, bc, T, bc, m->row_idx);
+        int rc = run_rows(m, bc, T, bc, m->row_idx, &mw);
         if (rc) return rc;
         launch_scatter_rows(m->lp, a->positions + p0, bc, V, a->table, s);
     }
diff --git a/proteingym_amd/csrc/api_model.hip b/proteingym_amd/csrc/api_model.hip
--- a/proteingym_amd/csrc/api_model.hip
+++ b/proteingym_amd/csrc/api_model.hip
@@ -402,6 +402,7 @@
     if (rc) { pgmi_model_destroy(m); return rc; }
     m->keep_rows = env_int("PGMI_KEEP_ROWS", 1);
     gemm_options_from_env();
+    mm_share_from_env();
     m->gemm_variant = env_int("PGMI_GEMM_VARIANT", 0);
     *out = m;
     return PGMI_OK;
@@ -440,11 +441,12 @@
     if (!name) { set_error("null option name"); return PGMI_EINVAL; }
     int rc = gemm_set_option(name, (long long)value);
     if (rc) rc = att_set_option(name, (long long)value);
+    if (rc) rc = esm_set_option(name, (long long)value);
     if (rc) rc = eve_set_option(name, (long long)value);
     if (rc) rc = mpnn_set_option(name, (long long)value);
     if (rc) rc = unirep_set_option(name, (long long)value);
     if (rc) rc = s2f_set_option(name, (long long)value);
-    if (rc) set_error("unknown option '%s' (gemm_half_tail, gemm_max_rows, att_xcd_local, att_v3, eve_max_rows, eve_fixed_sample, eve_prior_batch, mpnn_max_rows, unirep_max_rows, s2f_max_rows)", name);
+    if (rc) set_error("unknown option '%s' (gemm_half_tail, gemm_max_rows, att_xcd_local, att_v3, mm_share, eve_max_rows, eve_fixed_sample, eve_prior_batch, mpnn_max_rows, unirep_max_rows, s2f_max_rows)", name);
     return rc;
 }
 
diff --git a/proteingym_amd/csrc/attention_f16.hip b/proteingym_amd/csrc/attention_f16.hip
--- a/proteingym_amd/csrc/attention_f16.hip
+++ b/proteingym_amd/csrc/attention_f16.hip
@@ -6,11 +6,13 @@
 
 namespace pgmi {
 
-template <int WPB, int OUT, int NSTG, int DH = 64, bool RAG = false, int DO = DH>
+template <int WPB, int OUT, int NSTG, int DH = 64, bool RAG = false, int DO = DH, bool KEPT = false>
 __global__ __launch_bounds__(WPB * 64) void attention_f16x3_v2_kernel(
     const unsigned short* __restrict__ qk16, size_t qk_plane, const unsigned short* __restrict__ vt16,
     size_t vt_plane, const int32_t* __restrict__ kv_len, const float* __restrict__ slopes, int T, int H,
-    int Tp, float* __restrict__ ctx, unsigned short* __restrict__ ctx16, RagMap rag, int dense_nblk, int nseq) {
+    int Tp, float* __restrict__ ctx, unsigned short* __restrict__ ctx16, RagMap rag, int dense_nblk, int nseq,
+    const int32_t* __restrict__ kept_q) {
+    static_assert(!KEPT || (!RAG && DH == 64 && DO == 64), "kept tiles: the dense head_dim-64 launch only");
     constexpr float defer_thr = kAttDefer;
     constexpr int NT = WPB * 64;
     constexpr int KCPR = DH / 8;
@@ -39,6 +41,11 @@
         hs = blockIdx.y;
         qblk_dense = blockIdx.x;
     }
+    int kept_tile = 0;
+    if constexpr (KEPT) {
+        kept_tile = kept_q[b] >> 5;
+        if ((unsigned)(kept_tile - qblk_dense * WPB) >= (unsigned)WPB) return;
+    }
     h = hs / NSL;
     const int d0 = (hs - h * NSL) * DO;
     const int tid = threadIdx.x, lane = tid & 63;
@@ -52,7 +59,7 @@
     const int orow0 = RAG ? rag.seq_off[b] - p0 : b * T;
     const int Tpo = RAG ? (T - a0 + 31) / 32 * 32 : Tp;
     const int q0 = a0 + (qblk * WPB + wave) * 32;
-    const bool active = q0 < T;
+    const bool active = KEPT ? qblk * WPB + wave == kept_tile : q0 < T;
 
     constexpr bool q_lds = NSTG >= 3;
     u32x4 qh[NS], ql[NS];
@@ -274,10 +281,10 @@
 
 
 using Att16v2Kernel = decltype(&attention_f16x3_v2_kernel<4, ATT_OUT_F32, 3, 64, false, 64>);
-struct Att16v2Inst { int wpb, out, head_dim; bool rag; Att16v2Kernel fn; size_t lds_bytes; };
-template <int WPB, int OUT, int NSTG, int DH, bool RAG = false, int DO = DH>
+struct Att16v2Inst { int wpb, out, head_dim; bool rag, kept; Att16v2Kernel fn; size_t lds_bytes; };
+template <int WPB, int OUT, int NSTG, int DH, bool RAG = false, int DO = DH, bool KEPT = false>
 static constexpr Att16v2Inst att16v2_inst() {
-    return {WPB, OUT, DH, RAG, attention_f16x3_v2_kernel<WPB, OUT, NSTG, DH, RAG, DO>, (size_t)NSTG * (8 * DH + 8 * DO) * 16};
+    return {WPB, OUT, DH, RAG, KEPT, attention_f16x3_v2_kernel<WPB, OUT, NSTG, DH, RAG, DO, KEPT>, (size_t)NSTG * (8 * DH + 8 * DO) * 16};
 }
 static const Att16v2Inst kAtt16v2[] = {
     att16v2_inst<1, ATT_OUT_F32, 3, 64>(),   att16v2_inst<2, ATT_OUT_F32, 3, 64>(),   att16v2_inst<4, ATT_OUT_F32, 3, 64>(),
@@ -286,21 +293,26 @@
     att16v2_inst<1, ATT_OUT_SPLIT, 3, 64, true>(), att16v2_inst<2, ATT_OUT_SPLIT, 3, 64, true>(), att16v2_inst<4, ATT_OUT_SPLIT, 3, 64, true>(),
     att16v2_inst<4, ATT_OUT_F32, 3, 128>(),  att16v2_inst<4, ATT_OUT_SPLIT, 3, 128>(), att16v2_inst<4, ATT_OUT_BF16, 3, 128>(),
     att16v2_inst<4, ATT_OUT_SPLIT, 2, 256, false, 128>(),
+    att16v2_inst<1, ATT_OUT_SPLIT, 3, 64, false, 64, true>(), att16v2_inst<2, ATT_OUT_SPLIT, 3, 64, false, 64, true>(),
+    att16v2_inst<4, ATT_OUT_SPLIT, 3, 64, false, 64, true>(),
+    att16v2_inst<1, ATT_OUT_BF16, 3, 64, false, 64, true>(),  att16v2_inst<2, ATT_OUT_BF16, 3, 64, false, 64, true>(),
+    att16v2_inst<4, ATT_OUT_BF16, 3, 64, false, 64, true>(),
 };
 
 static int launch_att16v2(const AttLaunch& a, int wpb, dim3 grid, const RagMap* rag, int dense_nblk) {
     for (const Att16v2Inst& k : kAtt16v2) {
-        if (k.wpb != wpb || k.out != a.out || k.head_dim != a.head_dim || k.rag != (rag != nullptr)) continue;
+        if (k.wpb != wpb || k.out != a.out || k.head_dim != a.head_dim || k.rag != (rag != nullptr) || k.kept != (a.kept_q != nullptr)) continue;
         if (k.lds_bytes > 65536) {
             hipError_t e = hipFuncSetAttribute(reinterpret_cast<const void*>(k.fn), hipFuncAttributeMaxDynamicSharedMemorySize, (int)k.lds_bytes);
             if (e != hipSuccess) { set_error("hipFuncSetAttribute: %s", hipGetErrorString(e)); return PGMI_EHIP; }
         }
         hipLaunchKernelGGL(k.fn, grid, dim3(wpb * 64), k.lds_bytes, a.stream, a.qk16, a.qk_plane, a.vt16, a.vt_plane, a.kv_len, a.slopes,
-                           a.T, a.H, (a.T + 31) / 32 * 32, a.ctx, a.ctx16, rag ? *rag : RagMap{}, dense_nblk, a.B);
+                           a.T, a.H, (a.T + 31) / 32 * 32, a.ctx, a.ctx16, rag ? *rag : RagMap{}, dense_nblk, a.B, a.kept_q);
         PGMI_HIP(hipGetLastError());
         return PGMI_OK;
     }
-    set_error("attention_f16x3_v2: no kernel for %d waves, output %d, head_dim %d%s", wpb, (int)a.out, a.head_dim, rag ? ", ragged" : "");
+    set_error("attention_f16x3_v2: no kernel for %d waves, output %d, head_dim %d%s%s", wpb, (int)a.out, a.head_dim, rag ? ", ragged" : "",
+              a.kept_q ? ", kept tiles" : "");
     return PGMI_EINVAL;
 }
 
@@ -355,6 +367,7 @@
         const dim3 grid = dense_grid((n32 + 3) / 4, H, B, &dn);
         return launch_att16v2(a, 4, grid, nullptr, dn);
     }
+    if (a.kept_q && (a.qkv || a.slopes || a.out == ATT_OUT_F32)) { set_error("attention_f16x3_v2: kept tiles are for the fused-QKV, non-causal launch with 16-bit context rows"); return PGMI_EINVAL; }
     if (a.qkv && a.conv && a.rotary) { set_error("attention_f16x3_v2: depth-wise convolution and rotary together are not a model this library knows"); return PGMI_EINVAL; }
     if (a.qkv && a.conv && H % 4) { set_error("attention_f16x3_v2: the depth-wise convolution has four head groups, H = %d is not a multiple of 4", H); return PGMI_EINVAL; }
     if (a.qkv && a.conv)
diff --git a/proteingym_amd/csrc/attention_f16_v3.hip b/proteingym_amd/csrc/attention_f16_v3.hip
--- a/proteingym_amd/csrc/attention_f16_v3.hip
+++ b/proteingym_amd/csrc/attention_f16_v3.hip
@@ -6,11 +6,11 @@
 
 namespace pgmi {
 
-template <int WPB, int OUT>
+template <int WPB, int OUT, bool KEPT = false>
 __global__ __launch_bounds__(WPB * 64, 2) void attention_f16x3_v3_kernel(
     const unsigned short* __restrict__ qk16, size_t qk_plane, const unsigned short* __restrict__ vt16, size_t vt_plane,
     const int32_t* __restrict__ kv_len, int T, int H, int Tp, float* __restrict__ ctx, unsigned short* __restrict__ ctx16,
-    int dense_nblk, int nseq) {
+    int dense_nblk, int nseq, const int32_t* __restrict__ kept_q) {
     constexpr float defer_thr = kAttDefer;
     constexpr int DH = 64, NSTG = 3, KCPR = 8, KCH = AKT * KCPR, VCH = DH * 4, STG_CH = 2 * KCH + 2 * VCH;
     constexpr int NWI = STG_CH / 64, NDMA = (NWI + WPB - 1) / WPB, NS = 4, ND = 2;
@@ -26,13 +26,18 @@
         h = blockIdx.y;
         qblk = blockIdx.x;
     }
+    int kept_tile = 0;
+    if constexpr (KEPT) {
+        kept_tile = kept_q[b] >> 5;
+        if ((unsigned)(kept_tile - qblk * WPB) >= (unsigned)WPB) return;
+    }
     const int tid = threadIdx.x, lane = tid & 63;
     const int wave = __builtin_amdgcn_readfirstlane(tid >> 6);
     const int r = lane & 31, kh = lane >> 5;
     const int D = H * DH;
     const int Tk = kv_len ? kv_len[b] : T;
     const int q0 = (qblk * WPB + wave) * 32;
-    const bool active = q0 < T;
+    const bool active = KEPT ? qblk * WPB + wave == kept_tile : q0 < T;
     const int nkt = (Tk + AKT - 1) / AKT;
     const size_t seq_halfs = (size_t)T * (2 * D), vt_halfs = (size_t)DH * Tp;
     const unsigned long long qk_bytes = std::min<unsigned long long>(0xFFFFFFFFull, (unsigned long long)qk_plane * 2ull + seq_halfs * 2ull);
@@ -361,25 +366,27 @@
 }
 
 using Att16v3Kernel = decltype(&attention_f16x3_v3_kernel<4, ATT_OUT_F32>);
-struct Att16v3Inst { int wpb, out; Att16v3Kernel fn; };
-template <int WPB, int OUT>
-static constexpr Att16v3Inst att16v3_inst() { return {WPB, OUT, attention_f16x3_v3_kernel<WPB, OUT>}; }
+struct Att16v3Inst { int wpb, out; bool kept; Att16v3Kernel fn; };
+template <int WPB, int OUT, bool KEPT = false>
+static constexpr Att16v3Inst att16v3_inst() { return {WPB, OUT, KEPT, attention_f16x3_v3_kernel<WPB, OUT, KEPT>}; }
 static const Att16v3Inst kAtt16v3[] = {
     att16v3_inst<1, ATT_OUT_F32>(),   att16v3_inst<2, ATT_OUT_F32>(),   att16v3_inst<4, ATT_OUT_F32>(),
     att16v3_inst<1, ATT_OUT_SPLIT>(), att16v3_inst<2, ATT_OUT_SPLIT>(), att16v3_inst<4, ATT_OUT_SPLIT>(),
     att16v3_inst<1, ATT_OUT_BF16>(),  att16v3_inst<2, ATT_OUT_BF16>(),  att16v3_inst<4, ATT_OUT_BF16>(),
+    att16v3_inst<1, ATT_OUT_SPLIT, true>(), att16v3_inst<2, ATT_OUT_SPLIT, true>(), att16v3_inst<4, ATT_OUT_SPLIT, true>(),
+    att16v3_inst<1, ATT_OUT_BF16, true>(),  att16v3_inst<2, ATT_OUT_BF16, true>(),  att16v3_inst<4, ATT_OUT_BF16, true>(),
 };
 
 int launch_att16v3(const AttLaunch& a, int wpb, dim3 grid, int dense_nblk) {
     constexpr size_t lds_bytes = (size_t)3 * (2 * AKT * 8 + 2 * 64 * 4) * 16;
     for (const Att16v3Inst& k : kAtt16v3) {
-        if (k.wpb != wpb || k.out != a.out) continue;
+        if (k.wpb != wpb || k.out != a.out || k.kept != (a.kept_q != nullptr)) continue;
         hipLaunchKernelGGL(k.fn, grid, dim3(wpb * 64), lds_bytes, a.stream, a.qk16, a.qk_plane, a.vt16, a.vt_plane, a.kv_len, a.T, a.H, (a.T + 31) / 32 * 32,
-                           a.ctx, a.ctx16, dense_nblk, a.B);
+                           a.ctx, a.ctx16, dense_nblk, a.B, a.kept_q);
         PGMI_HIP(hipGetLastError());
         return PGMI_OK;
     }
-    set_error("attention_f16x3_v3: no kernel for %d waves, output %d", wpb, (int)a.out);
+    set_error("attention_f16x3_v3: no kernel for %d waves, output %d%s", wpb, (int)a.out, a.kept_q ? ", kept tiles" : "");
     return PGMI_EINVAL;
 }
 
diff --git a/proteingym_amd/csrc/common.h b/proteingym_amd/csrc/common.h
--- a/proteingym_amd/csrc/common.h
+++ b/proteingym_amd/csrc/common.h
@@ -103,6 +103,9 @@
 void launch_scatter_rows(const float* src, const int32_t* dst_row, int n, int V, float* table,
                          hipStream_t s);
 void launch_row_index(const int32_t* mask_rel, int B, int T, int32_t* out, hipStream_t s);
+void launch_mm_share_gather(const float* x, const int32_t* mask_rel, int B, int T, int D, float* y, hipStream_t s);
+void launch_mm_share_broadcast(const unsigned short* cqk, const unsigned short* cvt, const int32_t* mask_rel, int B, int T, int Da,
+                               unsigned short* qk16, size_t qk_plane, unsigned short* vt16, size_t vt_plane, hipStream_t s);
 void launch_fill_f32(float* p, int64_t n, float v, hipStream_t s);
 void launch_seq_loglik(const float* lp, const int32_t* tokens, const int32_t* lens, int B, int T, int V,
                        const float* prior, const int32_t* a0, const int32_t* row0, const int32_t* n,
@@ -338,6 +341,7 @@
     int B = 1, T = 0, H = 0;
     int head_dim = 64;
     const int32_t* kv_len = nullptr;
+    const int32_t* kept_q = nullptr;
     const float* slopes = nullptr;
     AttOut out = ATT_OUT_F32;
     float* ctx = nullptr;
diff --git a/proteingym_amd/csrc/elementwise.hip b/proteingym_amd/csrc/elementwise.hip
--- a/proteingym_amd/csrc/elementwise.hip
+++ b/proteingym_amd/csrc/elementwise.hip
@@ -352,6 +352,70 @@
     hipLaunchKernelGGL(row_index_kernel, dim3((B + 255) / 256), dim3(256), 0, s, mask_rel, B, T, out);
 }
 
+__global__ void mm_share_gather_kernel(const float* __restrict__ x, const int32_t* __restrict__ mask_rel, int B, int T, int D,
+                                       float* __restrict__ y) {
+    __shared__ int src_b;
+    const int r = blockIdx.x, ps = r / T, t = r - ps * T;
+    if (threadIdx.x == 0) src_b = (mask_rel[0] == t) ? 1 : 0;
+    __syncthreads();
+    if (ps == 1) {
+        for (int b = threadIdx.x; b < B; b += blockDim.x)
+            if (mask_rel[b] == t) src_b = b;
+        __syncthreads();
+    }
+    const f32x4* src = reinterpret_cast<const f32x4*>(x + ((size_t)src_b * T + t) * D);
+    f32x4* dst = reinterpret_cast<f32x4*>(y + (size_t)r * D);
+    for (int i = threadIdx.x; i < D / 4; i += blockDim.x) dst[i] = src[i];
+}
+void launch_mm_share_gather(const float* x, const int32_t* mask_rel, int B, int T, int D, float* y, hipStream_t s) {
+    hipLaunchKernelGGL(mm_share_gather_kernel, dim3(2 * T), dim3(256), 0, s, x, mask_rel, B, T, D, y);
+}
+
+typedef unsigned short u16x8 __attribute__((ext_vector_type(8)));
+__device__ __forceinline__ int vt_key_swap(int k) { return (k & ~12) | ((k & 4) << 1) | ((k & 8) >> 1); }
+__global__ void mm_share_broadcast_kernel(const unsigned short* __restrict__ cqk, const unsigned short* __restrict__ cvt,
+                                          const int32_t* __restrict__ mask_rel, int B, int T, int Tp, int Da, int nq_blocks,
+                                          unsigned short* __restrict__ qk16, size_t qk_plane, unsigned short* __restrict__ vt16,
+                                          size_t vt_plane) {
+    if ((int)blockIdx.x < nq_blocks) {
+        const int m = blockIdx.x * 4 + (threadIdx.x >> 6), lane = threadIdx.x & 63;
+        if (m >= B * T) return;
+        const int b = m / T, t = m - b * T;
+        const size_t cplane = (size_t)2 * T * 2 * Da;
+        const u16x8* src = reinterpret_cast<const u16x8*>(cqk + (size_t)(t == mask_rel[b] ? T + t : t) * (2 * Da));
+        u16x8* dst = reinterpret_cast<u16x8*>(qk16 + (size_t)m * (2 * Da));
+        for (int i = lane; i < Da / 4; i += 64) {
+            dst[i] = src[i];
+            dst[qk_plane / 8 + i] = src[cplane / 8 + i];
+        }
+        return;
+    }
+    const int cpr = Tp / 8;
+    const int64_t per_plane = (int64_t)B * Da * cpr;
+    const int64_t i = (int64_t)((int)blockIdx.x - nq_blocks) * 256 + threadIdx.x;
+    if (i >= 2 * per_plane) return;
+    const int p = i >= per_plane;
+    const int64_t j = i - p * per_plane, row = j / cpr;
+    const int c = (int)(j - row * cpr), b = (int)(row / Da), hd = (int)(row - (int64_t)b * Da);
+    const unsigned short* s0 = cvt + (size_t)p * ((size_t)2 * Da * Tp) + (size_t)hd * Tp + 8 * c;
+    u16x8 v = *reinterpret_cast<const u16x8*>(s0);
+    const int mr = mask_rel[b], pm = vt_key_swap(mr);
+    if ((pm >> 3) == c) v[pm & 7] = s0[(size_t)Da * Tp + (pm & 7)];
+    if (8 * c + 8 > (T & ~31)) {
+#pragma unroll
+        for (int e = 0; e < 8; ++e)
+            if (vt_key_swap(8 * c + e) >= T) v[e] = 0;
+    }
+    *reinterpret_cast<u16x8*>(vt16 + (size_t)p * vt_plane + (size_t)row * Tp + 8 * c) = v;
+}
+void launch_mm_share_broadcast(const unsigned short* cqk, const unsigned short* cvt, const int32_t* mask_rel, int B, int T, int Da,
+                               unsigned short* qk16, size_t qk_plane, unsigned short* vt16, size_t vt_plane, hipStream_t s) {
+    const int Tp = (T + 31) / 32 * 32, nq = (B * T + 3) / 4;
+    const int64_t nv = ((int64_t)2 * B * Da * (Tp / 8) + 255) / 256;
+    hipLaunchKernelGGL(mm_share_broadcast_kernel, dim3((unsigned)(nq + nv)), dim3(256), 0, s, cqk, cvt, mask_rel, B, T, Tp, Da, nq, qk16,
+                       qk_plane, vt16, vt_plane);
+}
+
 __global__ void fill_f32_kernel(float* p, int64_t n, float v) {
     const int64_t i = (int64_t)blockIdx.x * blockDim.x + threadIdx.x;
     if (i < n) p[i] = v;
diff --git a/proteingym_amd/csrc/model.h b/proteingym_amd/csrc/model.h
--- a/proteingym_amd/csrc/model.h
+++ b/proteingym_amd/csrc/model.h
@@ -52,6 +52,11 @@
     unsigned short* vt(int l) const { return planes ? k(l) + 2 * plane : nullptr; }
     int32_t* plan(int slot) const { return meta + (size_t)slot * plan_ints(cap); }
     int32_t* seq_off() const { return plan(2); }
+};
+
+struct MaskedWindows {
+    const int32_t* mask_rel = nullptr;
+    bool same_window = false;
 };
 
 }
@@ -152,6 +157,8 @@
     int64_t n_mut = 0, n_sub = 0;
     std::vector<void*> allocs;
     int32_t *wt = nullptr, *positions = nullptr, *win_start = nullptr, *mask_rel = nullptr;
+    std::vector<int32_t> win_start_host, mask_rel_host;
+    bool wt_has_mask = false;
     int32_t *sub_pos = nullptr, *sub_wt = nullptr, *sub_mt = nullptr;
     int64_t* mut_off = nullptr;
     float* table = nullptr;
@@ -243,10 +250,13 @@
 int create_esm(pgmi_model* m, const pgmi_config* cfg, const float* w, int64_t n_weights);
 int ensure_rotary(pgmi_model* m, int T);
 int upload_rotate_half(pgmi_model* m, int n);
-int run_encoder(pgmi_model* m, int B, int T, const int32_t* keep = nullptr, int n_keep = 0, bool* compacted = nullptr);
+int run_encoder(pgmi_model* m, int B, int T, const int32_t* keep = nullptr, int n_keep = 0, bool* compacted = nullptr,
+                const MaskedWindows* mw = nullptr);
+void mm_share_from_env();
+int esm_set_option(const char* name, long long value);
 int head_hidden(pgmi_model* m, int R, const int32_t* row_idx);
 int run_head(pgmi_model* m, int R, const int32_t* row_idx);
-int run_rows(pgmi_model* m, int B, int T, int R, const int32_t* row_idx);
+int run_rows(pgmi_model* m, int B, int T, int R, const int32_t* row_idx, const MaskedWindows* mw = nullptr);
 int create_tranception(pgmi_model* m, const pgmi_config* cfg, const float* w, int64_t n_weights);
 int create_progen2(pgmi_model* m, const pgmi_config* cfg, const float* w, int64_t n_weights, int rotary_dim);
 int create_gpt(pgmi_model* m, const pgmi_config* cfg, const float* w, int64_t n_weights, int pos_kind);
```

Result: no change. 18800, median of 6 (+0.7%).
